# JunyiPeng00/wespeaker_hubert

Hardware: AMD Instinct MI355X
Metric: embeddings/sec on 5s 16kHz utts (higher is better)
Workload: dtype f32 (bf16x3 split MFMA, fp32 accumulate)

## Files before the change

include/wespeaker_amd.h:

```cpp
#ifndef WESPEAKER_AMD_H_
#define WESPEAKER_AMD_H_

#include <stddef.h>
#include <stdint.h>

#ifdef __cplusplus
extern "C" {
#endif

#define WSP_OK 0
#define WSP_E_INVALID (-1)
#define WSP_E_HIP (-2)
#define WSP_E_STATE (-3)
#define WSP_E_UNSUPPORTED (-4)

#define WSP_DTYPE_F32 0
#define WSP_DTYPE_S16 1

#define WSP_WINDOW_HAMMING 0
#define WSP_WINDOW_POVEY 1
#define WSP_WINDOW_HANNING 2
#define WSP_WINDOW_RECTANGULAR 3
#define WSP_WINDOW_BLACKMAN 4

typedef struct wsp_model wsp_model;

int wsp_abi_version(void);
const char* wsp_last_error(void);

int wsp_fbank_num_frames(int num_samples, int frame_len, int frame_shift);

typedef struct wsp_fbank_opts {
  int num_mel_bins;
  int sample_rate;
  double frame_length_ms;
  double frame_shift_ms;
  int window_type;
  double low_freq;
  double high_freq;
} wsp_fbank_opts;

int wsp_fbank_opts_default(wsp_fbank_opts* o);
int wsp_fbank_geometry(const wsp_fbank_opts* o, int* frame_len, int* frame_shift, int* padded);
int wsp_fbank_mel_banks(const wsp_fbank_opts* o, float* banks);

int wsp_fbank_ex(const void* wav, int wav_dtype, int B, int num_samples, int ld, float scale,
                 float* feats, const wsp_fbank_opts* opts, int cmn, void* stream);
int wsp_fbank(const void* wav, int wav_dtype, int B, int num_samples, int ld, float scale,
              float* feats, int num_bins, int sample_rate, int window_type, int cmn,
              void* stream);

int wsp_fbank_segments_ex(const void* wav, int wav_dtype, int B, const int32_t* sample_offsets,
                          const int32_t* frame_offsets, int max_frames, float scale, float* feats,
                          const wsp_fbank_opts* opts, int cmn, void* stream);
int wsp_fbank_segments(const void* wav, int wav_dtype, int B, const int32_t* sample_offsets,
                       const int32_t* frame_offsets, int max_frames, float scale, float* feats,
                       int num_bins, int sample_rate, int window_type, int cmn, void* stream);

int wsp_model_create(const char* arch, int feat_dim, int embed_dim, int emb_bn,
                     int two_emb_layer, wsp_model** out);
int wsp_model_destroy(wsp_model* m);
int wsp_model_num_params(const wsp_model* m);
int wsp_model_param_info(const wsp_model* m, int index, const char** name, int* ndim,
                         int64_t shape[4]);
int wsp_model_set_param(wsp_model* m, int index, const float* host_data, int64_t numel);
int wsp_model_finalize(wsp_model* m);
int wsp_model_embed_dim(const wsp_model* m);
int wsp_model_feat_dim(const wsp_model* m);
int wsp_model_workspace_bytes(const wsp_model* m, int B, int T, size_t* bytes);
int wsp_model_forward(wsp_model* m, const float* feats, int B, int T, float* embed,
                      void* workspace, size_t workspace_bytes, void* stream);

int wsp_model_workspace_bytes_segments(const wsp_model* m, int B, int total_frames, size_t* bytes);
int wsp_model_forward_segments(wsp_model* m, const float* feats, int B, const int32_t* frame_offsets,
                               int total_frames, float* embed, void* workspace, size_t workspace_bytes,
                               void* stream);

int wsp_model_set_option(wsp_model* m, const char* key, int value);
int wsp_model_get_option(const wsp_model* m, const char* key, int* value);

int wsp_model_profile(wsp_model* m, int enable);
int wsp_model_profile_query(wsp_model* m, const char* kernel_class, int* launches,
                            double* total_ms, double* flops_per_launch);

int wsp_frontend_out_frames(const wsp_model* m, int num_samples, int* frames);
int wsp_frontend_workspace_bytes(const wsp_model* m, int B, int num_samples, size_t* bytes);
int wsp_frontend_forward(wsp_model* m, const float* wav, int B, int num_samples, float* feats, int cmn,
                         void* workspace, size_t workspace_bytes, void* stream);

int wsp_frontend_workspace_bytes_segments(const wsp_model* m, int B, const int32_t* num_samples, size_t* bytes);
int wsp_frontend_forward_segments(wsp_model* m, const float* wav, int B, const int32_t* num_samples, float* feats,
                                  int32_t* frame_offsets, int cmn, void* workspace, size_t workspace_bytes,
                                  void* stream);

int wsp_cmn(float* x, int B, int T, int D, void* stream);
int wsp_cmvn(float* x, int B, int T, int D, const int32_t* frame_offsets, int norm_mean, int norm_var,
             void* stream);

typedef struct wsp_resampler wsp_resampler;
int wsp_resampler_create(int orig_freq, int new_freq, int lowpass_filter_width, float rolloff,
                         wsp_resampler** out);
int wsp_resampler_destroy(wsp_resampler* r);
int wsp_resampler_out_len(const wsp_resampler* r, int num_samples, int* out_len);
int wsp_resample(const wsp_resampler* r, const float* x, int B, int num_samples, int ld, float* y, int ldy,
                 void* stream);
int wsp_resampler_kernel(const wsp_resampler* r, int* reduced_orig, int* reduced_new, int* width, int* taps,
                         float* kernel);

int wsp_l2_normalize(const float* x, const float* sub, float* y, int R, int D, void* stream);
int wsp_cosine_pairs(const float* E, int D, const int32_t* idx_a, const int32_t* idx_b,
                     int P, double* score, void* stream);
int wsp_asnorm_stats(const float* E, int Ne, const float* C, int Nc, int D, int top_n,
                     double* mu, double* sd, void* workspace, size_t workspace_bytes,
                     void* stream);
int wsp_asnorm_workspace_bytes(int Ne, int Nc, int D, size_t* bytes);
int wsp_row_mean_accum(const float* x, const int32_t* group, int R, int D, double* acc,
                       double* cnt, void* stream);

#ifdef __cplusplus
}
#endif
#endif
```

wespeaker_hubert_amd/_lib.py:

```python
from __future__ import annotations

import ctypes
import os
from ctypes import POINTER, c_char_p, c_double, c_float, c_int, c_int64, c_size_t, c_void_p

_HERE = os.path.dirname(os.path.abspath(__file__))
LIB_PATH = os.path.join(_HERE, "libwsp_hip.so")

WSP_DTYPE_F32 = 0
WSP_DTYPE_S16 = 1
WSP_WINDOW_HAMMING = 0
WSP_WINDOW_POVEY = 1
WSP_WINDOW_HANNING = 2
WSP_WINDOW_RECTANGULAR = 3
WSP_WINDOW_BLACKMAN = 4
WINDOW_TYPES = {"hamming": WSP_WINDOW_HAMMING, "povey": WSP_WINDOW_POVEY, "hanning": WSP_WINDOW_HANNING,
                "rectangular": WSP_WINDOW_RECTANGULAR, "blackman": WSP_WINDOW_BLACKMAN}


class FbankOpts(ctypes.Structure):
    _fields_ = [("num_mel_bins", c_int), ("sample_rate", c_int), ("frame_length_ms", c_double),
                ("frame_shift_ms", c_double), ("window_type", c_int), ("low_freq", c_double),
                ("high_freq", c_double)]

SIGNATURES = {
    "wsp_abi_version": (c_int, []),
    "wsp_last_error": (c_char_p, []),
    "wsp_fbank_num_frames": (c_int, [c_int, c_int, c_int]),
    "wsp_fbank": (c_int, [c_void_p, c_int, c_int, c_int, c_int, c_float, c_void_p, c_int, c_int,
                          c_int, c_int, c_void_p]),
    "wsp_fbank_segments": (c_int, [c_void_p, c_int, c_int, c_void_p, c_void_p, c_int, c_float, c_void_p, c_int,
                                   c_int, c_int, c_int, c_void_p]),
    "wsp_fbank_opts_default": (c_int, [c_void_p]),
    "wsp_fbank_geometry": (c_int, [c_void_p, POINTER(c_int), POINTER(c_int), POINTER(c_int)]),
    "wsp_fbank_mel_banks": (c_int, [c_void_p, c_void_p]),
    "wsp_fbank_ex": (c_int, [c_void_p, c_int, c_int, c_int, c_int, c_float, c_void_p, c_void_p, c_int, c_void_p]),
    "wsp_fbank_segments_ex": (c_int, [c_void_p, c_int, c_int, c_void_p, c_void_p, c_int, c_float, c_void_p,
                                      c_void_p, c_int, c_void_p]),
    "wsp_model_create": (c_int, [c_char_p, c_int, c_int, c_int, c_int, POINTER(c_void_p)]),
    "wsp_model_destroy": (c_int, [c_void_p]),
    "wsp_model_num_params": (c_int, [c_void_p]),
    "wsp_model_param_info": (c_int, [c_void_p, c_int, POINTER(c_char_p), POINTER(c_int),
                                     POINTER(c_int64)]),
    "wsp_model_set_param": (c_int, [c_void_p, c_int, c_void_p, c_int64]),
    "wsp_model_finalize": (c_int, [c_void_p]),
    "wsp_model_embed_dim": (c_int, [c_void_p]),
    "wsp_model_feat_dim": (c_int, [c_void_p]),
    "wsp_model_workspace_bytes": (c_int, [c_void_p, c_int, c_int, POINTER(c_size_t)]),
    "wsp_model_forward": (c_int, [c_void_p, c_void_p, c_int, c_int, c_void_p, c_void_p, c_size_t,
                                  c_void_p]),
    "wsp_model_workspace_bytes_segments": (c_int, [c_void_p, c_int, c_int, POINTER(c_size_t)]),
    "wsp_model_forward_segments": (c_int, [c_void_p, c_void_p, c_int, c_void_p, c_int, c_void_p, c_void_p,
                                           c_size_t, c_void_p]),
    "wsp_model_set_option": (c_int, [c_void_p, c_char_p, c_int]),
    "wsp_model_get_option": (c_int, [c_void_p, c_char_p, POINTER(c_int)]),
    "wsp_frontend_out_frames": (c_int, [c_void_p, c_int, POINTER(c_int)]),
    "wsp_frontend_workspace_bytes": (c_int, [c_void_p, c_int, c_int, POINTER(c_size_t)]),
    "wsp_frontend_forward": (c_int, [c_void_p, c_void_p, c_int, c_int, c_void_p, c_int, c_void_p, c_size_t,
                                     c_void_p]),
    "wsp_frontend_workspace_bytes_segments": (c_int, [c_void_p, c_int, c_void_p, POINTER(c_size_t)]),
    "wsp_frontend_forward_segments": (c_int, [c_void_p, c_void_p, c_int, c_void_p, c_void_p, c_void_p, c_int,
                                              c_void_p, c_size_t, c_void_p]),
    "wsp_model_profile": (c_int, [c_void_p, c_int]),
    "wsp_model_profile_query": (c_int, [c_void_p, c_char_p, POINTER(c_int), POINTER(c_double),
                                        POINTER(c_double)]),
    "wsp_cmn": (c_int, [c_void_p, c_int, c_int, c_int, c_void_p]),
    "wsp_cmvn": (c_int, [c_void_p, c_int, c_int, c_int, c_void_p, c_int, c_int, c_void_p]),
    "wsp_resampler_create": (c_int, [c_int, c_int, c_int, c_float, c_void_p]),
    "wsp_resampler_destroy": (c_int, [c_void_p]),
    "wsp_resampler_out_len": (c_int, [c_void_p, c_int, c_void_p]),
    "wsp_resample": (c_int, [c_void_p, c_void_p, c_int, c_int, c_int, c_void_p, c_int, c_void_p]),
    "wsp_resampler_kernel": (c_int, [c_void_p, c_void_p, c_void_p, c_void_p, c_void_p, c_void_p]),
    "wsp_l2_normalize": (c_int, [c_void_p, c_void_p, c_void_p, c_int, c_int, c_void_p]),
    "wsp_cosine_pairs": (c_int, [c_void_p, c_int, c_void_p, c_void_p, c_int, c_void_p, c_void_p]),
    "wsp_asnorm_stats": (c_int, [c_void_p, c_int, c_void_p, c_int, c_int, c_int, c_void_p, c_void_p,
                                 c_void_p, c_size_t, c_void_p]),
    "wsp_asnorm_workspace_bytes": (c_int, [c_int, c_int, c_int, POINTER(c_size_t)]),
    "wsp_row_mean_accum": (c_int, [c_void_p, c_void_p, c_int, c_int, c_void_p, c_void_p, c_void_p]),
}

_lib = None


class WspError(RuntimeError):
    pass


def load() -> ctypes.CDLL:
    global _lib
    if _lib is not None:
        return _lib
    if not os.path.exists(LIB_PATH):
        raise WspError(f"HIP library not built: {LIB_PATH} is missing "
                       "(run `python -c 'import __graft_entry__ as g; g.build()'`)")
    lib = ctypes.CDLL(LIB_PATH)
    for name, (res, args) in SIGNATURES.items():
        fn = getattr(lib, name)
        fn.restype = res
        fn.argtypes = args
    _lib = lib
    return lib


def check(status: int, what: str = "") -> None:
    if status != 0:
        msg = load().wsp_last_error().decode("utf-8", "replace")
        raise WspError(f"{what} failed (status {status}): {msg}")


def call(name: str, *args) -> int:
    st = getattr(load(), name)(*args)
    check(st, name)
    return st
```

wespeaker_hubert_amd/csrc/capi.cpp:

```cpp
#include "../../include/wespeaker_amd.h"

#include <hip/hip_runtime.h>

#include <algorithm>
#include <memory>
#include <mutex>
#include <string>
#include <vector>

#include "kernels.h"
#include "model.h"

namespace wsp {
static thread_local std::string g_err;
void set_error(const std::string& m) { g_err = m; }
const std::string& get_error() { return g_err; }

static const FbankPlan& fbank_plan_dev(const FbankConfig& c) {
  static std::mutex mu;
  static std::vector<std::unique_ptr<FbankPlan>> plans;
  static std::vector<int> devs;
  int dev = 0;
  WSP_HIP(hipGetDevice(&dev));
  std::lock_guard<std::mutex> lk(mu);
  for (size_t i = 0; i < plans.size(); ++i) {
    const FbankConfig& q = plans[i]->cfg;
    if (devs[i] == dev && q.num_bins == c.num_bins && q.sample_rate == c.sample_rate && q.window == c.window &&
        q.frame_length_ms == c.frame_length_ms && q.frame_shift_ms == c.frame_shift_ms &&
        q.low_freq == c.low_freq && q.high_freq == c.high_freq)
      return *plans[i];
  }
  auto p = std::make_unique<FbankPlan>();
  fbank_plan(c, *p);
  double* d = nullptr;
  WSP_HIP(hipMalloc(&d, p->host_tab.size() * sizeof(double)));
  WSP_HIP(hipMemcpy(d, p->host_tab.data(), p->host_tab.size() * sizeof(double), hipMemcpyHostToDevice));
  p->tab = d;
  plans.push_back(std::move(p));
  devs.push_back(dev);
  return *plans.back();
}

static FbankConfig fbank_config(const wsp_fbank_opts* o) {
  WSP_CHECK(o != nullptr, "fbank: null options");
  FbankConfig c;
  c.num_bins = o->num_mel_bins;
  c.sample_rate = o->sample_rate;
  c.frame_length_ms = o->frame_length_ms;
  c.frame_shift_ms = o->frame_shift_ms;
  c.window = o->window_type;
  c.low_freq = o->low_freq;
  c.high_freq = o->high_freq;
  fbank_config_resolve(c);
  return c;
}
}

struct wsp_model {
  wsp::Model m;
};

#define WSP_GUARD(...)                                                           \
  try {                                                                          \
    __VA_ARGS__;                                                                      \
    return WSP_OK;                                                               \
  } catch (const wsp::InvalidArg& e) {                                           \
    wsp::set_error(e.msg);                                                       \
    return WSP_E_INVALID;                                                        \
  } catch (const wsp::HipError& e) {                                             \
    wsp::set_error(std::string("HIP error ") + hipGetErrorString(e.err) + " at " + e.where); \
    return WSP_E_HIP;                                                            \
  } catch (const std::exception& e) {                                            \
    wsp::set_error(e.what());                                                    \
    return WSP_E_STATE;                                                          \
  }

static hipStream_t S(void* s) { return reinterpret_cast<hipStream_t>(s); }

extern "C" {

int wsp_abi_version(void) { return 1; }
const char* wsp_last_error(void) { return wsp::get_error().c_str(); }

int wsp_fbank_num_frames(int num_samples, int frame_len, int frame_shift) {
  if (frame_len <= 0 || frame_shift <= 0 || num_samples < frame_len) return 0;
  return 1 + (num_samples - frame_len) / frame_shift;
}

int wsp_fbank_opts_default(wsp_fbank_opts* o) {
  if (!o) return WSP_E_INVALID;
  o->num_mel_bins = 80;
  o->sample_rate = 16000;
  o->frame_length_ms = 25.0;
  o->frame_shift_ms = 10.0;
  o->window_type = WSP_WINDOW_HAMMING;
  o->low_freq = 20.0;
  o->high_freq = 0.0;
  return WSP_OK;
}

int wsp_fbank_geometry(const wsp_fbank_opts* o, int* frame_len, int* frame_shift, int* padded) {
  WSP_GUARD({
    const wsp::FbankConfig c = wsp::fbank_config(o);
    wsp::FbankPlan p;
    wsp::fbank_plan(c, p);
    if (frame_len) *frame_len = c.frame_len;
    if (frame_shift) *frame_shift = c.frame_shift;
    if (padded) *padded = c.padded;
  });
}

int wsp_fbank_mel_banks(const wsp_fbank_opts* o, float* banks) {
  WSP_GUARD({
    WSP_CHECK(banks != nullptr, "fbank: null output");
    std::vector<float> w;
    wsp::fbank_mel_banks(wsp::fbank_config(o), w);
    std::copy(w.begin(), w.end(), banks);
  });
}

int wsp_fbank_ex(const void* wav, int wav_dtype, int B, int num_samples, int ld, float scale, float* feats,
                 const wsp_fbank_opts* opts, int cmn, void* stream) {
  WSP_GUARD({
    const wsp::FbankConfig c = wsp::fbank_config(opts);
    WSP_CHECK(wav_dtype == WSP_DTYPE_F32 || wav_dtype == WSP_DTYPE_S16, "fbank: bad dtype");
    WSP_CHECK(B >= 0 && num_samples >= 0 && ld >= num_samples, "fbank: bad shape");
    const int T = wsp_fbank_num_frames(num_samples, c.frame_len, c.frame_shift);
    if (B > 0 && T > 0) {
      WSP_CHECK(wav && feats, "fbank: null pointer");
      wsp::launch_fbank(wav, wav_dtype, B, num_samples, ld, scale, feats, T, cmn, wsp::fbank_plan_dev(c), S(stream));
    }
  });
}

int wsp_fbank(const void* wav, int wav_dtype, int B, int num_samples, int ld, float scale,
              float* feats, int num_bins, int sample_rate, int window_type, int cmn,
              void* stream) {
  wsp_fbank_opts o;
  wsp_fbank_opts_default(&o);
  o.num_mel_bins = num_bins;
  o.sample_rate = sample_rate;
  o.window_type = window_type;
  return wsp_fbank_ex(wav, wav_dtype, B, num_samples, ld, scale, feats, &o, cmn, stream);
}

int wsp_fbank_segments_ex(const void* wav, int wav_dtype, int B, const int32_t* sample_offsets,
                          const int32_t* frame_offsets, int max_frames, float scale, float* feats,
                          const wsp_fbank_opts* opts, int cmn, void* stream) {
  WSP_GUARD({
    const wsp::FbankConfig c = wsp::fbank_config(opts);
    WSP_CHECK(wav_dtype == WSP_DTYPE_F32 || wav_dtype == WSP_DTYPE_S16, "fbank: bad dtype");
    WSP_CHECK(B >= 0 && max_frames >= 0, "fbank: bad shape");
    if (B > 0 && max_frames > 0) {
      WSP_CHECK(wav && feats && sample_offsets && frame_offsets, "fbank: null pointer");
      wsp::launch_fbank(wav, wav_dtype, B, 0, 0, scale, feats, max_frames, cmn, wsp::fbank_plan_dev(c), S(stream),
                        sample_offsets, frame_offsets);
    }
  });
}

int wsp_fbank_segments(const void* wav, int wav_dtype, int B, const int32_t* sample_offsets,
                       const int32_t* frame_offsets, int max_frames, float scale, float* feats, int num_bins,
                       int sample_rate, int window_type, int cmn, void* stream) {
  wsp_fbank_opts o;
  wsp_fbank_opts_default(&o);
  o.num_mel_bins = num_bins;
  o.sample_rate = sample_rate;
  o.window_type = window_type;
  return wsp_fbank_segments_ex(wav, wav_dtype, B, sample_offsets, frame_offsets, max_frames, scale, feats, &o, cmn,
                               stream);
}

int wsp_model_create(const char* arch, int feat_dim, int embed_dim, int emb_bn, int two_emb_layer,
                     wsp_model** out) {
  WSP_GUARD({
    WSP_CHECK(arch && out, "null argument");
    auto* h = new wsp_model();
    try {
      h->m.create(arch, feat_dim, embed_dim, emb_bn != 0, two_emb_layer != 0);
    } catch (...) {
      delete h;
      throw;
    }
    *out = h;
  });
}

int wsp_model_destroy(wsp_model* m) {
  delete m;
  return WSP_OK;
}

int wsp_model_num_params(const wsp_model* m) { return m ? m->m.num_params() : WSP_E_INVALID; }

int wsp_model_param_info(const wsp_model* m, int index, const char** name, int* ndim,
                         int64_t shape[4]) {
  WSP_GUARD({
    WSP_CHECK(m && name && ndim && shape, "null argument");
    m->m.param_info(index, name, ndim, shape);
  });
}

int wsp_model_set_param(wsp_model* m, int index, const float* host_data, int64_t numel) {
  WSP_GUARD({
    WSP_CHECK(m && (host_data || numel == 0), "null argument");
    m->m.set_param(index, host_data, numel);
  });
}

int wsp_model_finalize(wsp_model* m) {
  WSP_GUARD({
    WSP_CHECK(m, "null model");
    m->m.finalize();
  });
}

int wsp_model_embed_dim(const wsp_model* m) { return m ? m->m.embed_dim() : WSP_E_INVALID; }
int wsp_model_feat_dim(const wsp_model* m) { return m ? m->m.feat_dim() : WSP_E_INVALID; }

int wsp_model_workspace_bytes(const wsp_model* m, int B, int T, size_t* bytes) {
  WSP_GUARD({
    WSP_CHECK(m && bytes && B >= 0 && T >= 0, "bad argument");
    *bytes = m->m.workspace_bytes(B, T);
  });
}

int wsp_model_forward(wsp_model* m, const float* feats, int B, int T, float* embed, void* workspace,
                      size_t workspace_bytes, void* stream) {
  WSP_GUARD({
    WSP_CHECK(m && feats && embed && workspace, "null argument");
    m->m.forward(feats, B, T, embed, workspace, workspace_bytes, S(stream));
  });
}

int wsp_frontend_out_frames(const wsp_model* m, int num_samples, int* frames) {
  WSP_GUARD({
    WSP_CHECK(m && frames, "null argument");
    *frames = m->m.out_frames(num_samples);
  });
}

int wsp_frontend_workspace_bytes(const wsp_model* m, int B, int num_samples, size_t* bytes) {
  WSP_GUARD({
    WSP_CHECK(m && bytes, "null argument");
    *bytes = m->m.frontend_workspace_bytes(B, num_samples);
  });
}

int wsp_frontend_forward(wsp_model* m, const float* wav, int B, int num_samples, float* feats, int cmn,
                         void* workspace, size_t workspace_bytes, void* stream) {
  WSP_GUARD({
    WSP_CHECK(m && wav && feats && workspace, "null argument");
    m->m.forward_frontend(wav, B, num_samples, feats, cmn, workspace, workspace_bytes, S(stream));
  });
}

int wsp_model_workspace_bytes_segments(const wsp_model* m, int B, int total_frames, size_t* bytes) {
  WSP_GUARD({
    WSP_CHECK(m && bytes, "null argument");
    *bytes = m->m.workspace_bytes_segments(B, total_frames);
  });
}

int wsp_model_forward_segments(wsp_model* m, const float* feats, int B, const int32_t* frame_offsets,
                               int total_frames, float* embed, void* workspace, size_t workspace_bytes,
                               void* stream) {
  WSP_GUARD({
    WSP_CHECK(m && feats && frame_offsets && embed && workspace, "null argument");
    m->m.forward_segments(feats, B, frame_offsets, total_frames, embed, workspace, workspace_bytes, S(stream));
  });
}

int wsp_frontend_workspace_bytes_segments(const wsp_model* m, int B, const int32_t* num_samples, size_t* bytes) {
  WSP_GUARD({
    WSP_CHECK(m && num_samples && bytes, "null argument");
    *bytes = m->m.frontend_workspace_bytes_segments(B, num_samples);
  });
}

int wsp_frontend_forward_segments(wsp_model* m, const float* wav, int B, const int32_t* num_samples, float* feats,
                                  int32_t* frame_offsets, int cmn, void* workspace, size_t workspace_bytes,
                                  void* stream) {
  WSP_GUARD({
    WSP_CHECK(m && wav && num_samples && feats && workspace, "null argument");
    m->m.forward_frontend_segments(wav, B, num_samples, feats, frame_offsets, cmn, workspace, workspace_bytes,
                                   S(stream));
  });
}

int wsp_model_set_option(wsp_model* m, const char* key, int value) {
  WSP_GUARD({
    WSP_CHECK(m && key, "null argument");
    m->m.set_option(key, value);
  });
}

int wsp_model_get_option(const wsp_model* m, const char* key, int* value) {
  WSP_GUARD({
    WSP_CHECK(m && key && value, "null argument");
    *value = m->m.get_option(key);
  });
}

int wsp_model_profile(wsp_model* m, int enable) {
  WSP_GUARD({
    WSP_CHECK(m, "null model");
    m->m.profile(enable != 0);
  });
}

int wsp_model_profile_query(wsp_model* m, const char* kernel_class, int* launches,
                            double* total_ms, double* flops_per_launch) {
  WSP_GUARD({
    WSP_CHECK(m && kernel_class && launches && total_ms && flops_per_launch, "null argument");
    m->m.profile_query(kernel_class, launches, total_ms, flops_per_launch);
  });
}

struct wsp_resampler {
  wsp::ResamplePlan plan;
  mutable std::mutex mu;
  mutable int device = -1;
  mutable float* kern = nullptr;
  mutable int* band = nullptr;
};

int wsp_resampler_create(int orig_freq, int new_freq, int lowpass_filter_width, float rolloff,
                         wsp_resampler** out) {
  WSP_GUARD({
    WSP_CHECK(out != nullptr, "bad argument");
    *out = nullptr;
    auto r = std::make_unique<wsp_resampler>();
    wsp::resample_plan(orig_freq, new_freq, lowpass_filter_width, rolloff, r->plan);
    *out = r.release();
  });
}

int wsp_resampler_destroy(wsp_resampler* r) {
  WSP_GUARD({
    if (r) {
      if (r->kern) (void)hipFree(r->kern);
      if (r->band) (void)hipFree(r->band);
      delete r;
    }
  });
}

int wsp_resampler_out_len(const wsp_resampler* r, int num_samples, int* out_len) {
  WSP_GUARD({
    WSP_CHECK(r && out_len && num_samples >= 0, "bad argument");
    const long long n = wsp::resample_out_len(r->plan, num_samples);
    WSP_CHECK(n < (1LL << 31), "output too long");
    *out_len = (int)n;
  });
}

int wsp_resampler_kernel(const wsp_resampler* r, int* reduced_orig, int* reduced_new, int* width, int* taps,
                         float* kernel) {
  WSP_GUARD({
    WSP_CHECK(r != nullptr, "bad argument");
    if (reduced_orig) *reduced_orig = r->plan.orig;
    if (reduced_new) *reduced_new = r->plan.nw;
    if (width) *width = r->plan.width;
    if (taps) *taps = r->plan.L;
    if (kernel && !r->plan.identity) std::copy(r->plan.kern.begin(), r->plan.kern.end(), kernel);
  });
}

int wsp_resample(const wsp_resampler* r, const float* x, int B, int num_samples, int ld, float* y, int ldy,
                 void* stream) {
  WSP_GUARD({
    WSP_CHECK(r && B >= 0 && num_samples >= 0 && (B == 0 || num_samples == 0 || (x && y)), "bad argument");
    int dev = -1;
    WSP_HIP(hipGetDevice(&dev));
    if (!r->plan.identity) {
      std::lock_guard<std::mutex> lk(r->mu);
      if (r->device < 0) {
        WSP_HIP(hipMalloc(&r->kern, r->plan.kern.size() * sizeof(float)));
        WSP_HIP(hipMalloc(&r->band, r->plan.band.size() * sizeof(int)));
        WSP_HIP(hipMemcpy(r->kern, r->plan.kern.data(), r->plan.kern.size() * sizeof(float),
                          hipMemcpyHostToDevice));
        WSP_HIP(hipMemcpy(r->band, r->plan.band.data(), r->plan.band.size() * sizeof(int), hipMemcpyHostToDevice));
        r->device = dev;
      }
      WSP_CHECK(dev == r->device, "resampler is bound to another device");
    }
    wsp::launch_resample(r->plan, r->kern, r->band, x, B, num_samples, ld, y, ldy, S(stream));
  });
}

int wsp_cmn(float* x, int B, int T, int D, void* stream) {
  WSP_GUARD({
    WSP_CHECK(B >= 0 && T > 0 && D > 0 && (B == 0 || x), "bad argument");
    if (B > 0) wsp::launch_cmn_rows(x, B, T, D, S(stream));
  });
}

int wsp_cmvn(float* x, int B, int T, int D, const int32_t* frame_offsets, int norm_mean, int norm_var,
             void* stream) {
  WSP_GUARD({
    WSP_CHECK(B >= 0 && D > 0 && (frame_offsets || T > 0) && (B == 0 || x), "bad argument");
    if (B > 0 && (norm_mean || norm_var))
      wsp::launch_cmvn_rows(x, B, T, D, norm_mean != 0, norm_var != 0, S(stream), frame_offsets);
  });
}

int wsp_l2_normalize(const float* x, const float* sub, float* y, int R, int D, void* stream) {
  WSP_GUARD({
    WSP_CHECK(R >= 0 && D > 0 && (R == 0 || (x && y)), "bad argument");
    wsp::launch_l2_normalize(x, sub, y, R, D, S(stream));
  });
}

int wsp_cosine_pairs(const float* E, int D, const int32_t* idx_a, const int32_t* idx_b, int P,
                     double* score, void* stream) {
  WSP_GUARD({
    WSP_CHECK(P >= 0 && D > 0 && (P == 0 || (E && idx_a && idx_b && score)), "bad argument");
    wsp::launch_cosine_pairs(E, D, idx_a, idx_b, P, score, S(stream));
  });
}

int wsp_asnorm_workspace_bytes(int Ne, int Nc, int D, size_t* bytes) {
  WSP_GUARD({
    WSP_CHECK(bytes && Ne >= 0 && Nc > 0 && D > 0, "bad argument");
    int a, b;
    wsp::asnorm_layout(Ne, Nc, D, &a, &b, bytes);
  });
}

int wsp_asnorm_stats(const float* E, int Ne, const float* C, int Nc, int D, int top_n, double* mu,
                     double* sd, void* workspace, size_t workspace_bytes, void* stream) {
  WSP_GUARD({
    WSP_CHECK(Ne >= 0 && Nc > 0 && D > 0, "bad argument");
    if (Ne == 0) return WSP_OK;
    int Ncp, Dp;
    size_t need;
    wsp::asnorm_layout(Ne, Nc, D, &Ncp, &Dp, &need);
    WSP_CHECK(workspace && workspace_bytes >= need, "asnorm: workspace too small");
    wsp::launch_asnorm_stats(E, Ne, C, Nc, D, top_n, mu, sd, static_cast<float*>(workspace),
                             S(stream));
  });
}

int wsp_row_mean_accum(const float* x, const int32_t* group, int R, int D, double* acc,
                       double* cnt, void* stream) {
  WSP_GUARD({
    WSP_CHECK(R >= 0 && D > 0 && (R == 0 || (x && group && acc && cnt)), "bad argument");
    wsp::launch_row_mean_accum(x, group, R, D, acc, cnt, S(stream));
  });
}

}
```

wespeaker_hubert_amd/csrc/conv_gemm.hip:

```cpp
#include "gemm_common.h"

namespace wsp {

namespace {

constexpr int BK = 32;
constexpr int LDK = BK + 4;

template <int WM, int WN, int TM, int TN, int AMODE, bool UNI>
__global__ __launch_bounds__(256, 2) void conv_gemm_f32(const ConvGemmArgs p) {
  constexpr int BM = WM * TM * 32;
  constexpr int BN = WN * TN * 32;
  constexpr int AR = BM / 32;
  constexpr int BR = BN / 32;
  static_assert(WM * WN == 4, "4 waves");

  extern __shared__ __attribute__((aligned(16))) float smem[];
  float* As = smem;
  float* Bs = smem + 2 * BM * LDK;

  const int tid = threadIdx.x;
  const int lane = tid & 63;
  const int wave = tid >> 6;
  const int ntiles = p.N / BN;
  const int mtiles = (p.M + BM - 1) / BM;
  const int wg = xcd_remap(blockIdx.x, ntiles * mtiles);
  const int mt = wg / ntiles;
  const int nt = wg - mt * ntiles;
  const int m0 = mt * BM;
  const int n0 = nt * BN;

  const int srow = tid >> 3;
  const int c4 = (tid & 7) * 4;
  ALoader<AR, AMODE, UNI> al;
  al.init(p, m0, srow, 32, c4);
  if (p.gcols) al.a0 += (n0 / p.gcols) * p.gcin;
  const __amdgpu_buffer_rsrc_t rw = make_rsrc(p.w);
  int woff[BR];
#pragma unroll
  for (int i = 0; i < BR; ++i) woff[i] = ((n0 + srow + 32 * i) * p.Kp + c4) * 4;

  f32x4 ra[AR], rb[BR];

  auto load_tile = [&](int k0) {
#pragma unroll
    for (int i = 0; i < BR; ++i) rb[i] = bload4(rw, woff[i] + k0 * 4);
    al.load(k0, ra);
  };

  auto store_tile = [&](int buf) {
    float* a = As + buf * BM * LDK;
    float* b = Bs + buf * BN * LDK;
#pragma unroll
    for (int i = 0; i < AR; ++i)
      *reinterpret_cast<f32x4*>(a + (srow + 32 * i) * LDK + c4) = ra[i];
#pragma unroll
    for (int i = 0; i < BR; ++i)
      *reinterpret_cast<f32x4*>(b + (srow + 32 * i) * LDK + c4) = rb[i];
  };

  const int wm = wave / WN;
  const int wn = wave - wm * WN;
  const int r32 = lane & 31;
  const int h = lane >> 5;

  f32x16 acc[TM][TN];
#pragma unroll
  for (int i = 0; i < TM; ++i)
#pragma unroll
    for (int j = 0; j < TN; ++j)
#pragma unroll
      for (int r = 0; r < 16; ++r) acc[i][j][r] = 0.f;

  const int nk = p.Kp / BK;
  load_tile(0);
  store_tile(0);
  __syncthreads();

  for (int kt = 0; kt < nk; ++kt) {
    const int cur = kt & 1;
    if (kt + 1 < nk) load_tile((kt + 1) * BK);
    const float* a = As + cur * BM * LDK + (wm * TM * 32 + r32) * LDK + h * 16;
    const float* b = Bs + cur * BN * LDK + (wn * TN * 32 + r32) * LDK + h * 16;
#pragma unroll
    for (int q = 0; q < 4; ++q) {
      f32x4 af[TM], bf[TN];
#pragma unroll
      for (int i = 0; i < TM; ++i) af[i] = *reinterpret_cast<const f32x4*>(a + i * 32 * LDK + q * 4);
#pragma unroll
      for (int j = 0; j < TN; ++j) bf[j] = *reinterpret_cast<const f32x4*>(b + j * 32 * LDK + q * 4);
#pragma unroll
      for (int s = 0; s < 4; ++s)
#pragma unroll
        for (int i = 0; i < TM; ++i)
#pragma unroll
          for (int j = 0; j < TN; ++j)
            acc[i][j] = __builtin_amdgcn_mfma_f32_32x32x2f32(af[i][s], bf[j][s], acc[i][j], 0, 0, 0);
    }
    if (kt + 1 < nk) store_tile(cur ^ 1);
    __syncthreads();
  }

  gemm_epilogue<TM, TN>(p, acc, m0, n0, wm, wn, lane);
}

template <int WM, int WN, int TM, int TN, int AMODE, bool UNI>
void launch_k(const ConvGemmArgs& p, hipStream_t s) {
  constexpr int BM = WM * TM * 32, BN = WN * TN * 32;
  const int nwg = ((p.M + BM - 1) / BM) * (p.N / BN);
  const size_t lds = (size_t)2 * (BM + BN) * LDK * sizeof(float);
  hipLaunchKernelGGL((conv_gemm_f32<WM, WN, TM, TN, AMODE, UNI>), dim3(nwg), dim3(256), lds, s, p);
  WSP_HIP(hipGetLastError());
}

template <int WM, int WN, int TM, int TN>
void launch_tile(const ConvGemmArgs& p, hipStream_t s) {
  const bool uni = uniform_ktiles(p);
  if (p.amode == kAAdd) {
    if (uni) launch_k<WM, WN, TM, TN, kAAdd, true>(p, s);
    else launch_k<WM, WN, TM, TN, kAAdd, false>(p, s);
  } else {
    if (uni) launch_k<WM, WN, TM, TN, kACat, true>(p, s);
    else launch_k<WM, WN, TM, TN, kACat, false>(p, s);
  }
}

}

int conv_gemm_tile_for(int N) { return (N % 128 == 0) ? 0 : 1; }

void launch_conv_gemm(const ConvGemmArgs& args, hipStream_t s) {
  const ConvGemmArgs p = normalized(args);
  check_conv_args(p, "conv_gemm");
  WSP_CHECK(!p.colsum, "conv_gemm: column sums are a bf16x3-kernel epilogue");
  WSP_CHECK(!p.conv2d && p.N % 64 == 0, "conv_gemm (f32): 1-D convs with N % 64 == 0 only");
  WSP_CHECK(!p.gcols || p.gcols % 64 == 0, "conv_gemm (f32): grouped columns must be a multiple of 64");
  if (conv_gemm_tile_for(p.N) == 0 && !p.gcols)
    launch_tile<2, 2, 2, 2>(p, s);
  else
    launch_tile<4, 1, 1, 2>(p, s);
}

}
```

wespeaker_hubert_amd/csrc/conv_gemm_x3.hip:

```cpp
#include "conv_gemm_x3_impl.h"

namespace wsp {

int conv_gemm_x3_block_rows(const ConvGemmArgs& p, int variant) {
  if (p.N % 64 != 0 || (p.gcols && p.gcols % 64 != 0)) return 128;
  if (p.gcols || p.N % 128 != 0) return 128;
  return variant == 3 ? 128 : 256;
}

namespace {
__global__ __launch_bounds__(256) void colsum_mean_kernel(const double* __restrict__ part, int bm, int T, int N,
                                                          float* __restrict__ out, int ldo) {
  const int b = blockIdx.y;
  const int n = blockIdx.x * 256 + threadIdx.x;
  if (n >= N) return;
  const long r0 = (long)b * T, r1 = r0 + T;
  double v = 0.0;
  for (long mt = r0 / bm; mt * bm < r1; ++mt) {
    const int slot = (mt * bm) / T == b ? 0 : 1;
    v += part[((size_t)mt * 2 + slot) * N + n];
  }
  out[(long)b * ldo + n] = (float)(v / (double)T);
}
}

void launch_colsum_mean(const double* part, int block_rows, int T, int B, int N, float* out, int ldo,
                        hipStream_t s) {
  WSP_CHECK(block_rows > 0 && T >= block_rows && B > 0 && N > 0, "colsum_mean: bad shape");
  hipLaunchKernelGGL(colsum_mean_kernel, dim3((N + 255) / 256, B), dim3(256), 0, s, part, block_rows, T, N, out,
                     ldo);
  WSP_HIP(hipGetLastError());
}

void launch_conv_gemm_x3(const ConvGemmArgs& args, const void* whi, const void* wlo, int variant,
                         hipStream_t s) {
  const ConvGemmArgs p = normalized(args);
  check_conv_args(p, "conv_gemm_x3");
  if (p.colsum) {
    const int bm = conv_gemm_x3_block_rows(p, variant);
    WSP_CHECK(!p.seg && !p.row_bias && !p.conv2d && p.T >= bm,
              "conv_gemm_x3: column sums need a uniform batch with T >= block rows and no row bias");
  }
  WSP_CHECK(p.Kp % 64 == 0, "conv_gemm_x3: packed K must be a multiple of 64");
  WSP_CHECK(variant >= 3 && variant <= 7, "conv_gemm_x3: tile family must be 3, 4, 5, 6 or 7");
  const __bf16* h = static_cast<const __bf16*>(whi);
  const __bf16* l = static_cast<const __bf16*>(wlo);
  x3::TileFn f;
  WSP_CHECK(!p.lnmode || (variant == 7 && x3::g256_supported(p)),
            "conv_gemm_x3: the LayerNorm fold runs on tile family 7 only");
  WSP_CHECK(!p.sc2d || (variant == 7 && x3::g256_supported(p)),
            "conv_gemm_x3: conv3 + shortcut runs on tile family 7 only (N % 256 == 0, 16-B aligned operands)");
  if (variant == 7 && x3::g256_supported(p)) {
    x3::t_g256(p, h, l, s);
    return;
  }
  if (variant == 7) variant = 6;
  if (p.N % 64 != 0 || (p.gcols && p.gcols % 64 != 0)) {
    f = x3::t_4x1_1x1;
  } else if (p.gcols) {
    f = variant >= 5 ? x3::t_8x1_1x2_sw : x3::t_4x1_1x2;
  } else if (p.N % 128 != 0) {
    f = x3::t_4x1_1x2;
  } else if (variant == 3) {
    f = x3::t_2x2_2x2_sw;
  } else if (variant == 4) {
    f = x3::t_4x2_2x2_sw;
  } else if (p.N % 256 == 0) {
    f = variant == 6 ? x3::t_4x2_2x4_mf16 : x3::t_4x2_2x4_sw1;
  } else {
    f = x3::t_4x2_2x2_sw;
  }
  f(p, h, l, s);
}

}
```

wespeaker_hubert_amd/csrc/conv_gemm_x3_impl.h:

```cpp
#pragma once

#include <type_traits>

#include "gemm_common.h"

namespace wsp {

namespace {

typedef __bf16 bf16x8 __attribute__((ext_vector_type(8)));
typedef __bf16 bf16x4 __attribute__((ext_vector_type(4)));

constexpr int BK = 32;

template <bool SWZ, int MF = 32>
struct Lds {
  static constexpr int ROWB = SWZ ? 64 : 80;
  static constexpr int SKEW = SWZ ? 0 : 64;
  __device__ __forceinline__ static int off(int row, int byte) {
    static_assert(MF == 32 || SWZ, "16x16 fragments need the swizzled rows");
    if constexpr (SWZ && MF == 16)
      return row * 64 + ((((byte >> 4) ^ (0x1320 >> (4 * ((row >> 2) & 3)))) & 3) << 4) + (byte & 15);
    else if constexpr (SWZ) return row * 64 + ((((byte >> 4) ^ (row >> 2)) & 3) << 4) + (byte & 15);
    else return row * 80 + byte;
  }
};

template <int WM, int WN, int TM, int TN, int AMODE, bool UNI, int ROLE, bool C2D = false, bool SWZ = false,
          int NSET = 2, int MF = 32>
__global__ __launch_bounds__(WM* WN * 64, 2) void conv_gemm_x3(const ConvGemmArgs p,
                                                               const __bf16* __restrict__ whi,
                                                               const __bf16* __restrict__ wlo) {
  using L = Lds<SWZ, MF>;
  static_assert(MF == 32 || NSET == 1, "16x16 MFMA: one-staging-set wide tiles only");
  constexpr int ROWB = L::ROWB;
  constexpr int NT = WM * WN * 64;
  constexpr int BM = WM * TM * 32;
  constexpr int BN = WN * TN * 32;
  constexpr int AR = BM * 8 / NT;
  constexpr int BR = BN * 8 / NT;
  constexpr int ROWS_A = NT / 8;
  constexpr int A_BYTES = BM * ROWB;
  constexpr int B_BYTES = BN * ROWB;
  constexpr int B_LO = B_BYTES + L::SKEW;
  constexpr int STAGE = 2 * A_BYTES + B_LO + B_BYTES;
  static_assert(AR >= 1 && BR >= 1, "tile too small for the thread count");
  static_assert(BN * 4 % 64 == 0, "a W image must be a whole number of wave loads");

  extern __shared__ __attribute__((aligned(16))) unsigned char smem[];

  const int tid = threadIdx.x;
  const int lane = tid & 63;
  const int wave = tid >> 6;
  const int ntiles = p.N / BN;
  const int mtiles = (p.M + BM - 1) / BM;
  const int wg = xcd_remap(blockIdx.x, ntiles * mtiles);
  const int mt = wg / ntiles;
  const int nt = wg - mt * ntiles;
  const int m0 = mt * BM;
  const int n0 = nt * BN;

  const int srow = tid >> 3;
  const int c4 = (tid & 7) * 4;
  std::conditional_t<C2D, ALoader2D<AR>, ALoader<AR, AMODE, UNI>> al;
  al.init(p, m0, srow, ROWS_A, c4);
  if (p.gcols) al.a0 += (n0 / p.gcols) * p.gcin;
  const __amdgpu_buffer_rsrc_t rwhi = make_rsrc(whi);
  const __amdgpu_buffer_rsrc_t rwlo = make_rsrc(wlo);
  int boff[BR], bls[BR];
  bool bimg[BR];
#pragma unroll
  for (int i = 0; i < BR; ++i) {
    const int q = tid + NT * i;
    const int img = __builtin_amdgcn_readfirstlane(q / (BN * 4));
    const int qq = q - img * BN * 4;
    const int row = qq >> 2, part = qq & 3;
    bimg[i] = img != 0;
    boff[i] = ((n0 + row) * p.Kp + part * 8) * 2;
    bls[i] = L::off(row, part * 16) + (img ? B_LO : 0);
  }

  f32x4 ra0[AR], ra1[AR];
  bf16x8 rb0[BR], rb1[BR];

  auto load_tile = [&](f32x4 (&ra)[AR], bf16x8 (&rb)[BR], int k0, bool live) {
#pragma unroll
    for (int i = 0; i < BR; ++i) {
      const int o = live ? boff[i] + k0 * 2 : kOOB;
      rb[i] = __builtin_bit_cast(bf16x8, __builtin_amdgcn_raw_buffer_load_b128(bimg[i] ? rwlo : rwhi, o, 0, 0));
    }
    al.load(k0, ra, live);
  };

  auto store_tile = [&](const f32x4 (&ra)[AR], const bf16x8 (&rb)[BR], int buf) {
    unsigned char* st = smem + buf * STAGE;
#pragma unroll
    for (int i = 0; i < AR; ++i) {
      bf16x4 hi, lo;
#pragma unroll
      for (int e = 0; e < 4; ++e) {
        const float x = ra[i][e];
        const __bf16 hh = (__bf16)x;
        hi[e] = hh;
        lo[e] = (__bf16)(x - (float)hh);
      }
      const int off = L::off(srow + ROWS_A * i, c4 * 2);
      *reinterpret_cast<bf16x4*>(st + off) = hi;
      *reinterpret_cast<bf16x4*>(st + A_BYTES + off) = lo;
    }
#pragma unroll
    for (int i = 0; i < BR; ++i) *reinterpret_cast<bf16x8*>(st + 2 * A_BYTES + bls[i]) = rb[i];
  };

  const int wm = wave / WN;
  const int wn = wave - wm * WN;
  const int r32 = lane & 31;
  const int h = lane >> 5;

  f32x16 acc[TM][TN];
#pragma unroll
  for (int i = 0; i < TM; ++i)
#pragma unroll
    for (int j = 0; j < TN; ++j)
#pragma unroll
      for (int r = 0; r < 16; ++r) acc[i][j][r] = 0.f;

  auto mma_step = [&](int buf, int s) {
    const unsigned char* st = smem + buf * STAGE;
    const unsigned char* a_hi = st + L::off(wm * TM * 32 + r32, h * 16 + s * 32);
    const unsigned char* a_lo = a_hi + A_BYTES;
    const unsigned char* b_hi = st + 2 * A_BYTES + L::off(wn * TN * 32 + r32, h * 16 + s * 32);
    const unsigned char* b_lo = b_hi + B_LO;
    bf16x8 ah[TM], al_[TM], bh[TN], bl[TN];
#pragma unroll
    for (int i = 0; i < TM; ++i) {
      ah[i] = *reinterpret_cast<const bf16x8*>(a_hi + i * 32 * ROWB);
      al_[i] = *reinterpret_cast<const bf16x8*>(a_lo + i * 32 * ROWB);
    }
#pragma unroll
    for (int j = 0; j < TN; ++j) {
      bh[j] = *reinterpret_cast<const bf16x8*>(b_hi + j * 32 * ROWB);
      bl[j] = *reinterpret_cast<const bf16x8*>(b_lo + j * 32 * ROWB);
    }
#pragma unroll
    for (int i = 0; i < TM; ++i)
#pragma unroll
      for (int j = 0; j < TN; ++j) {
        acc[i][j] = __builtin_amdgcn_mfma_f32_32x32x16_bf16(al_[i], bh[j], acc[i][j], 0, 0, 0);
        acc[i][j] = __builtin_amdgcn_mfma_f32_32x32x16_bf16(ah[i], bl[j], acc[i][j], 0, 0, 0);
        acc[i][j] = __builtin_amdgcn_mfma_f32_32x32x16_bf16(ah[i], bh[j], acc[i][j], 0, 0, 0);
      }
  };

  const int nk = p.Kp / BK;
  if constexpr (MF == 16) {
    const int r16 = lane & 15, qk = lane >> 4;
    f32x4 acc16[2 * TM][2 * TN];
#pragma unroll
    for (int i = 0; i < 2 * TM; ++i)
#pragma unroll
      for (int j = 0; j < 2 * TN; ++j) acc16[i][j] = f32x4{0.f, 0.f, 0.f, 0.f};
    bf16x8 fah[TM], fal[TM], fbh[TN], fbl[TN];
    auto rdA = [&](const unsigned char* st, int ih) {
#pragma unroll
      for (int i = 0; i < TM; ++i) {
        const int o = L::off(wm * TM * 32 + (ih * TM + i) * 16 + r16, qk * 16);
        fah[i] = *reinterpret_cast<const bf16x8*>(st + o);
        fal[i] = *reinterpret_cast<const bf16x8*>(st + A_BYTES + o);
      }
    };
    auto rdB = [&](const unsigned char* st, int jh) {
#pragma unroll
      for (int j = 0; j < TN; ++j) {
        const int o = L::off(wn * TN * 32 + (jh * TN + j) * 16 + r16, qk * 16);
        fbh[j] = *reinterpret_cast<const bf16x8*>(st + 2 * A_BYTES + o);
        fbl[j] = *reinterpret_cast<const bf16x8*>(st + 2 * A_BYTES + B_LO + o);
      }
    };
    auto mm = [&](int ih, int jh) {
#pragma unroll
      for (int i = 0; i < TM; ++i)
#pragma unroll
        for (int j = 0; j < TN; ++j) {
          f32x4& c = acc16[ih * TM + i][jh * TN + j];
          c = __builtin_amdgcn_mfma_f32_16x16x32_bf16(fal[i], fbh[j], c, 0, 0, 0);
          c = __builtin_amdgcn_mfma_f32_16x16x32_bf16(fah[i], fbl[j], c, 0, 0, 0);
          c = __builtin_amdgcn_mfma_f32_16x16x32_bf16(fah[i], fbh[j], c, 0, 0, 0);
        }
    };
    load_tile(ra0, rb0, 0, true);
    store_tile(ra0, rb0, 0);
    load_tile(ra0, rb0, BK, true);
    __syncthreads();
    for (int kt = 0; kt < nk; ++kt) {
      const int buf = kt & 1;
      const unsigned char* st = smem + buf * STAGE;
      rdA(st, 0);
      rdB(st, 0);
      mm(0, 0);
      rdB(st, 1);
      mm(0, 1);
      store_tile(ra0, rb0, buf ^ 1);
      load_tile(ra0, rb0, (kt + 2) * BK, kt + 2 < nk);
      rdA(st, 1);
      mm(1, 1);
      rdB(st, 0);
      mm(1, 0);
      __syncthreads();
    }
    gemm_epilogue16<2 * TM, 2 * TN, WM, WN>(p, acc16, m0, n0, wm, wn, lane, smem);
    return;
  } else if constexpr (NSET == 1) {
    load_tile(ra0, rb0, 0, true);
    store_tile(ra0, rb0, 0);
    load_tile(ra0, rb0, BK, true);
    __syncthreads();
    for (int kt = 0; kt < nk; ++kt) {
      const int buf = kt & 1;
      mma_step(buf, 0);
      store_tile(ra0, rb0, buf ^ 1);
      load_tile(ra0, rb0, (kt + 2) * BK, kt + 2 < nk);
      mma_step(buf, 1);
      __syncthreads();
    }
    gemm_epilogue<TM, TN, WM, WN>(p, acc, m0, n0, wm, wn, lane, smem);
    return;
  }
  load_tile(ra0, rb0, 0, true);
  load_tile(ra1, rb1, BK, true);
  store_tile(ra0, rb0, 0);
  __syncthreads();

  if constexpr (ROLE == 2) {
    for (int kt = 0; kt < nk - 2; kt += 2) {
      load_tile(ra0, rb0, (kt + 2) * BK, true);
      mma_step(0, 0);
      store_tile(ra1, rb1, 1);
      mma_step(0, 1);
      __syncthreads();
      load_tile(ra1, rb1, (kt + 3) * BK, true);
      mma_step(1, 0);
      store_tile(ra0, rb0, 0);
      mma_step(1, 1);
      __syncthreads();
    }
    float rv[TM][TN][16];
    load_residual_tiles<TM, TN>(p, rv, m0, n0, wm, wn, lane);
    mma_step(0, 0);
    store_tile(ra1, rb1, 1);
    mma_step(0, 1);
    __syncthreads();
    mma_step(1, 0);
    mma_step(1, 1);
    gemm_epilogue_res_pre<TM, TN>(p, acc, m0, n0, wm, wn, lane, rv);
    return;
  }

  for (int kt = 0; kt < nk; kt += 2) {
    load_tile(ra0, rb0, (kt + 2) * BK, kt + 2 < nk);
    mma_step(0, 0);
    store_tile(ra1, rb1, 1);
    mma_step(0, 1);
    __syncthreads();
    load_tile(ra1, rb1, (kt + 3) * BK, kt + 3 < nk);
    mma_step(1, 0);
    store_tile(ra0, rb0, 0);
    mma_step(1, 1);
    __syncthreads();
  }

  gemm_epilogue<TM, TN, WM, WN>(p, acc, m0, n0, wm, wn, lane, smem);
}

template <int WM, int WN, int TM, int TN, int AMODE, bool UNI, int ROLE, bool C2D, bool SWZ, int NSET, int MF = 32>
void launch_x3_k(const ConvGemmArgs& p, const __bf16* whi, const __bf16* wlo, hipStream_t s) {
  constexpr int BM = WM * TM * 32, BN = WN * TN * 32, NT = WM * WN * 64;
  constexpr int ROWB = Lds<SWZ>::ROWB;
  const int nwg = ((p.M + BM - 1) / BM) * (p.N / BN);
  const size_t lds = (size_t)2 * (2 * BM * ROWB + 2 * BN * ROWB + Lds<SWZ>::SKEW);
  hipLaunchKernelGGL((conv_gemm_x3<WM, WN, TM, TN, AMODE, UNI, ROLE, C2D, SWZ, NSET, MF>), dim3(nwg), dim3(NT), lds,
                     s, p, whi, wlo);
  WSP_HIP(hipGetLastError());
}

template <int WM, int WN, int TM, int TN, bool SWZ = false, int NSET = 2, int MF = 32>
void launch_x3_tile(const ConvGemmArgs& p, const __bf16* whi, const __bf16* wlo, hipStream_t s) {
  if constexpr (MF == 32) {
    if (p.conv2d) {
      launch_x3_k<WM, WN, TM, TN, kACat, true, 0, true, SWZ, NSET, MF>(p, whi, wlo, s);
      return;
    }
  }
  const bool uni = uniform_ktiles(p);
  if (MF == 32 && p.amode == kAAdd) {
    if constexpr (MF == 32) {
      if (uni)
        launch_x3_k<WM, WN, TM, TN, kAAdd, true, 0, false, SWZ, NSET, MF>(p, whi, wlo, s);
      else
        launch_x3_k<WM, WN, TM, TN, kAAdd, false, 0, false, SWZ, NSET, MF>(p, whi, wlo, s);
    }
  } else if (!uni) {
    launch_x3_k<WM, WN, TM, TN, kACat, false, 0, false, SWZ, NSET, MF>(p, whi, wlo, s);
  } else if (p.role == 1) {
    launch_x3_k<WM, WN, TM, TN, kACat, true, 1, false, SWZ, NSET, MF>(p, whi, wlo, s);
  } else if constexpr (NSET == 2 && TM * TN <= 4) {
    if (p.res && p.role == 2)
      launch_x3_k<WM, WN, TM, TN, kACat, true, 2, false, SWZ, NSET>(p, whi, wlo, s);
    else
      launch_x3_k<WM, WN, TM, TN, kACat, true, 0, false, SWZ, NSET>(p, whi, wlo, s);
  } else {
    launch_x3_k<WM, WN, TM, TN, kACat, true, 0, false, SWZ, NSET, MF>(p, whi, wlo, s);
  }
}

}

namespace x3 {
using TileFn = void (*)(const ConvGemmArgs&, const __bf16*, const __bf16*, hipStream_t);
void t_4x1_1x1(const ConvGemmArgs&, const __bf16*, const __bf16*, hipStream_t);
void t_4x1_1x2(const ConvGemmArgs&, const __bf16*, const __bf16*, hipStream_t);
void t_8x1_1x2_sw(const ConvGemmArgs&, const __bf16*, const __bf16*, hipStream_t);
void t_2x2_2x2_sw(const ConvGemmArgs&, const __bf16*, const __bf16*, hipStream_t);
void t_4x2_2x2_sw(const ConvGemmArgs&, const __bf16*, const __bf16*, hipStream_t);
void t_4x2_2x4_sw1(const ConvGemmArgs&, const __bf16*, const __bf16*, hipStream_t);
void t_4x2_2x4_mf16(const ConvGemmArgs&, const __bf16*, const __bf16*, hipStream_t);
bool g256_supported(const ConvGemmArgs&);
void t_g256(const ConvGemmArgs&, const __bf16*, const __bf16*, hipStream_t);
}

}
```

wespeaker_hubert_amd/csrc/conv_gemm_x3_t6.hip:

```cpp
#include "conv_gemm_x3_impl.h"

namespace wsp {
namespace {

typedef __attribute__((address_space(3))) void lds_void;
constexpr int kGA = 256 * 128, kGW = 256 * 64, kGStage = kGA + 2 * kGW;

__device__ __forceinline__ int g_aslot(int r, int c) { return r * 128 + ((c ^ ((r >> 1) & 5)) << 4); }

__device__ __forceinline__ void g_dma(__amdgpu_buffer_rsrc_t r, unsigned char* lds, int voff) {
  __builtin_amdgcn_raw_ptr_buffer_load_lds(r, (lds_void*)lds, 16, voff, 0, 0, 0);
}

constexpr int kGEpiLd = 132;
constexpr int kGEpiBytes = 8 * 32 * kGEpiLd * 4;
typedef unsigned u32x4 __attribute__((ext_vector_type(4)));

constexpr int kLnMaxParts = 8;
__device__ __forceinline__ void g_ln_row(const ConvGemmArgs& p, int row, float& mu, float& rstd) {
  const float* s = p.ln_in + (size_t)row * p.ln_parts * 2;
  float m = s[0], m2 = s[1];
#pragma unroll
  for (int k = 1; k < kLnMaxParts; ++k) {
    if (k < p.ln_parts) {
      const float d = s[2 * k] - m;
      m += d * (1.f / (float)(k + 1));
      m2 += s[2 * k + 1] + d * d * (128.f * (float)k / (float)(k + 1));
    }
  }
  mu = m;
  rstd = 1.f / sqrtf(m2 / (128.f * (float)p.ln_parts) + p.ln_eps);
}

template <int R>
__device__ __forceinline__ void g_ln_pieces(float (&m)[R], float (&m2)[R]) {
  float n = 4.f;
  auto merge = [&](int i, float mo, float m2o) {
    const float d = mo - m[i];
    m[i] = 0.5f * (m[i] + mo);
    m2[i] = (m2[i] + m2o) + d * d * (0.5f * n);
  };
#define WSP_DPP(v, ctrl) __builtin_bit_cast(float, __builtin_amdgcn_mov_dpp(__builtin_bit_cast(int, v), ctrl, 0xF, 0xF, false))
#pragma unroll
  for (int i = 0; i < R; ++i) merge(i, WSP_DPP(m[i], 0xB1), WSP_DPP(m2[i], 0xB1));
  n *= 2.f;
#pragma unroll
  for (int i = 0; i < R; ++i) merge(i, WSP_DPP(m[i], 0x4E), WSP_DPP(m2[i], 0x4E));
  n *= 2.f;
#pragma unroll
  for (int i = 0; i < R; ++i) merge(i, WSP_DPP(m[i], 0x141), WSP_DPP(m2[i], 0x141));
  n *= 2.f;
#pragma unroll
  for (int i = 0; i < R; ++i) merge(i, WSP_DPP(m[i], 0x140), WSP_DPP(m2[i], 0x140));
  n *= 2.f;
#undef WSP_DPP
#define WSP_BC15(v) \
  __builtin_bit_cast(float, __builtin_amdgcn_update_dpp(0, __builtin_bit_cast(int, v), 0x142, 0xA, 0xF, false))
#pragma unroll
  for (int i = 0; i < R; ++i) merge(i, WSP_BC15(m[i]), WSP_BC15(m2[i]));
#undef WSP_BC15
}

template <int ACT, bool RB, bool RES, int LNM = 0>
__device__ __forceinline__ void g_epilogue_rows(const ConvGemmArgs& p, f32x4 (&acc)[4][8], int m0, int n0, int wm,
                                                int wn, int wave, int lane, unsigned char* smem, float lmu = 0.f,
                                                float lrs = 1.f) {
  float* stg = reinterpret_cast<float*>(smem) + wave * 32 * kGEpiLd;
  const int c16 = lane & 15, q = lane >> 4;
  const int cl = 4 * (lane & 31);
  const int col = n0 + wn * 128 + cl;
  const f32x4 bv = p.bias ? *reinterpret_cast<const f32x4*>(p.bias + col) : f32x4{0.f, 0.f, 0.f, 0.f};
  const f32x4 sc = p.scale ? *reinterpret_cast<const f32x4*>(p.scale + col) : f32x4{1.f, 1.f, 1.f, 1.f};
  const f32x4 sh = p.scale ? *reinterpret_cast<const f32x4*>(p.shift + col) : f32x4{0.f, 0.f, 0.f, 0.f};
  f32x4 lcs{0.f, 0.f, 0.f, 0.f}, lg{1.f, 1.f, 1.f, 1.f}, lb{0.f, 0.f, 0.f, 0.f};
  if constexpr ((LNM & 2) != 0) lcs = *reinterpret_cast<const f32x4*>(p.ln_cs + col);
  if constexpr ((LNM & 4) != 0) {
    lg = *reinterpret_cast<const f32x4*>(p.ln_g + col);
    lb = *reinterpret_cast<const f32x4*>(p.ln_b + col);
  }
  const int lparts = p.N / 128, lpart = (n0 + wn * 128) / 128;
  const __amdgpu_buffer_rsrc_t ro = make_rsrc(p.out);
  const __amdgpu_buffer_rsrc_t rres = make_rsrc(RES ? p.res : p.out);
#pragma unroll
  for (int h = 0; h < 2; ++h) {
    float pm[(LNM & 1) ? 16 : 1], pm2[(LNM & 1) ? 16 : 1];
#pragma unroll
    for (int i2 = 0; i2 < 2; ++i2)
#pragma unroll
      for (int j = 0; j < 8; ++j)
#pragma unroll
        for (int r = 0; r < 4; ++r) stg[(i2 * 16 + 4 * q + r) * kGEpiLd + j * 16 + c16] = acc[2 * h + i2][j][r];
    asm volatile("s_waitcnt lgkmcnt(0)" ::: "memory");
#pragma unroll
    for (int u = 0; u < 16; ++u) {
      const int rl = 2 * u + (lane >> 5);
      const int row = m0 + wm * 64 + h * 32 + rl;
      const bool ok = row < p.M;
      const f32x4 x = *reinterpret_cast<const f32x4*>(stg + rl * kGEpiLd + cl);
      f32x4 rv{0.f, 0.f, 0.f, 0.f}, rb{0.f, 0.f, 0.f, 0.f};
      if constexpr (RES) rv = bload4(rres, ok ? (row * p.ldres + col) * 4 : kOOB);
      if constexpr (RB) {
        const int rowc = ok ? row : p.M - 1;
        const int ub = p.seg ? seg_of(p.seg, p.nseg, rowc) : rowc / p.T;
        rb = *reinterpret_cast<const f32x4*>(p.row_bias + (size_t)ub * p.N + col);
      }
      float mu = 0.f, rstd = 1.f;
      if constexpr ((LNM & 6) != 0) {
        auto rd = [](float v, int l) {
          return __builtin_bit_cast(float, __builtin_amdgcn_readlane(__builtin_bit_cast(int, v), l));
        };
        mu = lane < 32 ? rd(lmu, h * 32 + 2 * u) : rd(lmu, h * 32 + 2 * u + 1);
        rstd = lane < 32 ? rd(lrs, h * 32 + 2 * u) : rd(lrs, h * 32 + 2 * u + 1);
      }
      f32x4 y;
#pragma unroll
      for (int e = 0; e < 4; ++e) {
        float v;
        if constexpr ((LNM & 2) != 0) v = (x[e] - mu * lcs[e]) * rstd + bv[e];
        else v = x[e] + bv[e];
        if constexpr ((LNM & 4) != 0) v += (rv[e] - mu) * rstd * lg[e] + lb[e];
        else if constexpr (RES) v += rv[e];
        if constexpr (RB) v += rb[e];
        if constexpr (ACT == kActRelu) v = fmaxf(v, 0.f);
        else if constexpr (ACT == kActTanh) v = tanhf(v);
        else if constexpr (ACT == kActGelu) v = gelu_as(v);
        y[e] = v * sc[e] + sh[e];
      }
      __builtin_amdgcn_raw_buffer_store_b128(__builtin_bit_cast(u32x4, y), ro, ok ? (row * p.ldo + col) * 4 : kOOB, 0,
                                             0);
      if constexpr ((LNM & 1) != 0) {
        pm[u] = ((y[0] + y[1]) + (y[2] + y[3])) * 0.25f;
        float q2 = 0.f;
#pragma unroll
        for (int e = 0; e < 4; ++e) q2 += (y[e] - pm[u]) * (y[e] - pm[u]);
        pm2[u] = q2;
      }
    }
    if constexpr ((LNM & 1) != 0) {
      g_ln_pieces<16>(pm, pm2);
      if ((lane & 31) == 16) {
#pragma unroll
        for (int u = 0; u < 16; ++u) {
          const int row = m0 + wm * 64 + h * 32 + 2 * u + (lane >> 5);
          if (row < p.M) *reinterpret_cast<float2*>(p.ln_out + ((size_t)row * lparts + lpart) * 2) = float2{pm[u], pm2[u]};
        }
      }
    }
    asm volatile("s_waitcnt lgkmcnt(0)" ::: "memory");
  }
}

constexpr int kGCsLd = 68;
constexpr int kGCsBytes = 8 * 64 * kGCsLd * 4;
template <int ACT>
__device__ __forceinline__ void g_epilogue_cs(const ConvGemmArgs& p, f32x4 (&acc)[4][8], int m0, int n0, int wm,
                                              int wn, int wave, int lane, unsigned char* smem) {
  float* stg = reinterpret_cast<float*>(smem) + wave * 64 * kGCsLd;
  const int c16 = lane & 15, q = lane >> 4;
  const int cl = 4 * c16;
  const __amdgpu_buffer_rsrc_t ro = make_rsrc(p.out);
  const int nb = min((m0 / p.T + 1) * p.T, p.M) - m0, mb = p.M - m0;
  unsigned side0 = 0, side1 = 0;
#pragma unroll
  for (int k = 0; k < 16; ++k) {
    const int rr = wm * 64 + (k >> 2) * 16 + 4 * q + (k & 3);
    side0 |= (rr < nb ? 1u : 0u) << k;
    side1 |= (rr >= nb && rr < mb ? 1u : 0u) << k;
  }
  double rs[8][2];
#pragma unroll
  for (int pp = 0; pp < 2; ++pp) {
#pragma unroll
    for (int i = 0; i < 4; ++i)
#pragma unroll
      for (int jj = 0; jj < 4; ++jj)
#pragma unroll
        for (int r = 0; r < 4; ++r) stg[(16 * i + 4 * q + r) * kGCsLd + 16 * jj + c16] = acc[i][4 * pp + jj][r];
    asm volatile("s_waitcnt lgkmcnt(0)" ::: "memory");
    const int col = n0 + wn * 128 + 64 * pp + cl;
    const f32x4 bv = p.bias ? *reinterpret_cast<const f32x4*>(p.bias + col) : f32x4{0.f, 0.f, 0.f, 0.f};
    const f32x4 sc = p.scale ? *reinterpret_cast<const f32x4*>(p.scale + col) : f32x4{1.f, 1.f, 1.f, 1.f};
    const f32x4 sh = p.scale ? *reinterpret_cast<const f32x4*>(p.shift + col) : f32x4{0.f, 0.f, 0.f, 0.f};
#pragma unroll
    for (int u = 0; u < 16; ++u) {
      const int rl = 4 * u + q;
      const int row = m0 + wm * 64 + rl;
      float* sp = stg + rl * kGCsLd + cl;
      const f32x4 x = *reinterpret_cast<const f32x4*>(sp);
      f32x4 y;
#pragma unroll
      for (int e = 0; e < 4; ++e) {
        float v = x[e] + bv[e];
        if constexpr (ACT == kActRelu) v = fmaxf(v, 0.f);
        else if constexpr (ACT == kActTanh) v = tanhf(v);
        else if constexpr (ACT == kActGelu) v = gelu_as(v);
        y[e] = v * sc[e] + sh[e];
      }
      __builtin_amdgcn_raw_buffer_store_b128(__builtin_bit_cast(u32x4, y), ro,
                                             row < p.M ? (row * p.ldo + col) * 4 : kOOB, 0, 0);
      *reinterpret_cast<f32x4*>(sp) = y;
    }
    asm volatile("s_waitcnt lgkmcnt(0)" ::: "memory");
#pragma unroll
    for (int jj = 0; jj < 4; ++jj) {
      double c0 = 0.0, c1 = 0.0;
#pragma unroll
      for (int k = 0; k < 16; ++k) {
        const double yd = (double)stg[((k >> 2) * 16 + 4 * q + (k & 3)) * kGCsLd + 16 * jj + c16];
        c0 += (side0 >> k) & 1 ? yd : 0.0;
        c1 += (side1 >> k) & 1 ? yd : 0.0;
      }
      double v0 = c0 + __shfl_xor(c0, 16);
      v0 += __shfl_xor(v0, 32);
      double v1 = c1 + __shfl_xor(c1, 16);
      v1 += __shfl_xor(v1, 32);
      rs[4 * pp + jj][0] = v0;
      rs[4 * pp + jj][1] = v1;
      __builtin_amdgcn_sched_barrier(0);
    }
    asm volatile("s_waitcnt lgkmcnt(0)" ::: "memory");
  }
  __syncthreads();
  constexpr int BN = 256;
  double* red = reinterpret_cast<double*>(smem);
  if (lane < 16) {
#pragma unroll
    for (int j = 0; j < 8; ++j)
#pragma unroll
      for (int u = 0; u < 2; ++u) red[(wm * 2 + u) * BN + (wn * 8 + j) * 16 + lane] = rs[j][u];
  }
  __syncthreads();
  const int tid = threadIdx.x;
  if (tid < 2 * BN) {
    const int u = tid / BN, c = tid - u * BN;
    double v = 0.0;
#pragma unroll
    for (int w = 0; w < 4; ++w) v += red[(w * 2 + u) * BN + c];
    p.colsum[((size_t)(m0 / 256) * 2 + u) * p.N + n0 + c] = v;
  }
}

template <int AM, bool CSK, int LNM = 0, int XP = 0>
__global__ __launch_bounds__(512, 1) void conv_gemm_g(const ConvGemmArgs p, const __bf16* __restrict__ whi,
                                                      const __bf16* __restrict__ wlo) {
  using L = Lds<true, 16>;
  constexpr bool DENSE = AM == 1 || AM == 3;
  extern __shared__ __attribute__((aligned(16))) unsigned char smem[];
  const int tid = threadIdx.x;
  const int lane = tid & 63;
  const int wave = tid >> 6;
  const int ntiles = p.N / 256;
  const int mtiles = (p.M + 255) / 256;
  const int wg = xcd_remap(blockIdx.x, ntiles * mtiles);
  const int mt = wg / ntiles;
  const int nt = wg - mt * ntiles;
  const int m0 = mt * 256;
  const int n0 = nt * 256;

  const int ac0 = 4 * ((lane & 7) ^ ((lane >> 4) & 1)), ac1 = ac0 ^ 16;
  int a_r[4], a_t[DENSE ? 1 : 4], a_l[DENSE ? 1 : 4], a_s[AM == 3 ? 4 : 1];
#pragma unroll
  for (int i = 0; i < 4; ++i) {
    const int m = m0 + (4 * wave + i) * 8 + (lane >> 3);
    if constexpr (DENSE) {
      a_r[i] = m < p.M ? m : -1;
      if constexpr (AM == 3) {
        const int fto = p.Fo * p.To;
        const int b = m / fto, fo = (m - b * fto) / p.To, to = m - b * fto - fo * p.To;
        a_s[i] = m < p.M ? (b * p.Fi + fo * p.stride) * p.Ti + to * p.stride : -1;
      }
    } else if (p.seg) {
      const int mm = m < p.M ? m : p.M - 1;
      const int b = seg_of(p.seg, p.nseg, mm);
      const int t = (mm - p.seg[b]) * p.stride;
      const int* is = p.iseg ? p.iseg : p.seg;
      a_r[i] = is[b] + t;
      a_t[i] = (m < p.M) ? t : -0x40000000;
      a_l[i] = is[b + 1] - is[b];
    } else {
      const int b = m / p.T;
      const int t = (m - b * p.T) * p.stride;
      a_r[i] = b * p.Ti + t;
      a_t[i] = (m < p.M) ? t : -0x40000000;
      a_l[i] = p.Ti;
    }
  }
  int woff[2];
#pragma unroll
  for (int i = 0; i < 2; ++i) {
    const int row = (2 * wave + i) * 16 + (lane >> 2);
    const int c = (lane & 3) ^ ((0x1320 >> (4 * ((row >> 2) & 3))) & 3);
    woff[i] = ((n0 + row) * p.Kp + 8 * c) * 2;
  }
  const __amdgpu_buffer_rsrc_t rwh = make_rsrc(whi);
  const __amdgpu_buffer_rsrc_t rwl = make_rsrc(wlo);
  const int nk = p.Kp / BK;
  int jt = 0, ct = 0;
  auto dma = [&](int kt, int buf, int part = 3) {
    unsigned char* st = smem + buf * kGStage;
    const int off = jt * p.dil - p.pad;
    const float* base = p.a[0];
    int ld = p.lda[0], cl = ct;
    if (ct >= p.cseg[2]) {
      base = p.a[2];
      ld = p.lda[2];
      cl = ct - p.cseg[2];
    } else if (ct >= p.cseg[1]) {
      base = p.a[1];
      ld = p.lda[1];
      cl = ct - p.cseg[1];
    }
    const __amdgpu_buffer_rsrc_t ra = make_rsrc(base);
#pragma unroll
    for (int i = 0; i < 4; ++i) {
      if (!(part & 1)) break;
      if constexpr (DENSE) {
        const int ar = AM == 3 && ct >= p.cseg[1] ? a_s[i] : a_r[i];
        g_dma(ra, st + (4 * wave + i) * 1024, ar >= 0 ? (ar * ld + cl + (i & 1 ? ac1 : ac0)) * 4 : kOOB);
      } else if constexpr (AM == 2) {
        const int k = kt * BK + (i & 1 ? ac1 : ac0);
        const int tap = k / p.cin;
        const int offk = tap * p.dil - p.pad;
        const int tt = a_t[i] + offk;
        const bool ok = k < p.K && tt >= 0 && tt < a_l[i];
        g_dma(ra, st + (4 * wave + i) * 1024, ok ? ((a_r[i] + offk) * ld + k - tap * p.cin) * 4 : kOOB);
      } else {
        const int tt = a_t[i] + off;
        const bool ok = tt >= 0 && tt < a_l[i];
        g_dma(ra, st + (4 * wave + i) * 1024, ok ? ((a_r[i] + off) * ld + cl + (i & 1 ? ac1 : ac0)) * 4 : kOOB);
      }
    }
#pragma unroll
    for (int i = 0; i < 2; ++i) {
      if (!(part & 2)) break;
      const int o = woff[i] + kt * 64;
      g_dma(rwh, st + kGA + (2 * wave + i) * 1024, o);
      g_dma(rwl, st + kGA + kGW + (2 * wave + i) * 1024, o);
    }
    if (!(part & 2)) return;
    ct += 32;
    if (ct >= p.cin) {
      ct -= p.cin;
      ++jt;
    }
  };

  const int wm = wave >> 1, wn = wave & 1;
  const int r16 = lane & 15, qk = lane >> 4;
  f32x4 acc[4][8];
#pragma unroll
  for (int i = 0; i < 4; ++i)
#pragma unroll
    for (int j = 0; j < 8; ++j) acc[i][j] = f32x4{0.f, 0.f, 0.f, 0.f};
  bf16x8 ah[2], al[2], bh[4], bl[4];
  auto rdA = [&](const unsigned char* st, int ih) {
#pragma unroll
    for (int i = 0; i < 2; ++i) {
      const int r = wm * 64 + (ih * 2 + i) * 16 + r16;
      const f32x4 x0 = *reinterpret_cast<const f32x4*>(st + g_aslot(r, 2 * qk));
      const f32x4 x1 = *reinterpret_cast<const f32x4*>(st + g_aslot(r, 2 * qk + 1));
      if constexpr (XP == 1 || XP == 4) {
        ah[i] = __builtin_bit_cast(bf16x8, x0);
        al[i] = __builtin_bit_cast(bf16x8, x1);
        continue;
      }
#pragma unroll
      for (int e = 0; e < 4; ++e) {
        const __bf16 h0 = (__bf16)x0[e], h1 = (__bf16)x1[e];
        ah[i][e] = h0;
        ah[i][4 + e] = h1;
        al[i][e] = (__bf16)(x0[e] - (float)h0);
        al[i][4 + e] = (__bf16)(x1[e] - (float)h1);
      }
    }
  };
  auto rdB = [&](const unsigned char* st, int jh) {
#pragma unroll
    for (int j = 0; j < 4; ++j) {
      const int o = L::off(wn * 128 + (jh * 4 + j) * 16 + r16, qk * 16);
      bh[j] = *reinterpret_cast<const bf16x8*>(st + kGA + o);
      bl[j] = *reinterpret_cast<const bf16x8*>(st + kGA + kGW + o);
    }
  };
  auto mm = [&](int ih, int jh) {
#pragma unroll
    for (int i = 0; i < 2; ++i)
#pragma unroll
      for (int j = 0; j < 4; ++j) {
        f32x4& c = acc[ih * 2 + i][jh * 4 + j];
        c = __builtin_amdgcn_mfma_f32_16x16x32_bf16(al[i], bh[j], c, 0, 0, 0);
        c = __builtin_amdgcn_mfma_f32_16x16x32_bf16(ah[i], bl[j], c, 0, 0, 0);
        c = __builtin_amdgcn_mfma_f32_16x16x32_bf16(ah[i], bh[j], c, 0, 0, 0);
      }
  };

  float lmu = 0.f, lrs = 1.f;
  if constexpr ((LNM & 6) != 0) g_ln_row(p, min(m0 + wm * 64 + lane, p.M - 1), lmu, lrs);
  dma(0, 0);
  dma(1, 1);
  asm volatile("s_waitcnt vmcnt(8)" ::: "memory");
  __builtin_amdgcn_s_barrier();
  for (int kt = 0; kt < nk; ++kt) {
    const int buf = kt & 1;
    const unsigned char* st = smem + buf * kGStage;
    if constexpr (XP == 2) {
      rdA(st, 0);
      rdB(st, 0);
      mm(0, 0);
      __builtin_amdgcn_sched_barrier(0);
      if (kt >= 1 && kt + 1 < nk) dma(kt + 1, buf ^ 1, 1);
      __builtin_amdgcn_sched_barrier(0);
      rdB(st, 1);
      mm(0, 1);
      __builtin_amdgcn_sched_barrier(0);
      if (kt >= 1 && kt + 1 < nk) dma(kt + 1, buf ^ 1, 2);
      __builtin_amdgcn_sched_barrier(0);
      rdA(st, 1);
      mm(1, 1);
      rdB(st, 0);
      mm(1, 0);
      asm volatile("s_waitcnt vmcnt(0) lgkmcnt(0)" ::: "memory");
      __builtin_amdgcn_s_barrier();
      __builtin_amdgcn_sched_barrier(0);
      continue;
    }
    rdA(st, 0);
    rdB(st, 0);
    mm(0, 0);
    rdB(st, 1);
    mm(0, 1);
    rdA(st, 1);
    mm(1, 1);
    rdB(st, 0);
    mm(1, 0);
    if constexpr (XP >= 3) {
      asm volatile("s_waitcnt lgkmcnt(0)" ::: "memory");
      continue;
    }
    asm volatile("s_waitcnt vmcnt(0) lgkmcnt(0)" ::: "memory");
    __builtin_amdgcn_s_barrier();
    __builtin_amdgcn_sched_barrier(0);
    if (kt + 2 < nk) dma(kt + 2, buf);
  }
#define WSP_GEPI(RB, RES)                                                                                   \
  switch (p.act) {                                                                                         \
    case kActRelu: g_epilogue_rows<kActRelu, RB, RES>(p, acc, m0, n0, wm, wn, wave, lane, smem); break;    \
    case kActTanh: g_epilogue_rows<kActTanh, RB, RES>(p, acc, m0, n0, wm, wn, wave, lane, smem); break;    \
    case kActGelu: g_epilogue_rows<kActGelu, RB, RES>(p, acc, m0, n0, wm, wn, wave, lane, smem); break;    \
    default: g_epilogue_rows<kActNone, RB, RES>(p, acc, m0, n0, wm, wn, wave, lane, smem); break;          \
  }
  if constexpr (LNM != 0) {
    if constexpr ((LNM & 5) != 0)
      g_epilogue_rows<kActNone, false, true, LNM>(p, acc, m0, n0, wm, wn, wave, lane, smem, lmu, lrs);
    else if (p.act == kActGelu)
      g_epilogue_rows<kActGelu, false, false, LNM>(p, acc, m0, n0, wm, wn, wave, lane, smem, lmu, lrs);
    else
      g_epilogue_rows<kActNone, false, false, LNM>(p, acc, m0, n0, wm, wn, wave, lane, smem, lmu, lrs);
  } else if constexpr (CSK) {
    switch (p.act) {
      case kActRelu: g_epilogue_cs<kActRelu>(p, acc, m0, n0, wm, wn, wave, lane, smem); break;
      case kActTanh: g_epilogue_cs<kActTanh>(p, acc, m0, n0, wm, wn, wave, lane, smem); break;
      case kActGelu: g_epilogue_cs<kActGelu>(p, acc, m0, n0, wm, wn, wave, lane, smem); break;
      default: g_epilogue_cs<kActNone>(p, acc, m0, n0, wm, wn, wave, lane, smem); break;
    }
  } else if (p.res) {
    WSP_GEPI(false, true)
  } else if (p.row_bias) {
    WSP_GEPI(true, false)
  } else {
    WSP_GEPI(false, false)
  }
#undef WSP_GEPI
}

#ifdef WSP_G7_XP
constexpr int kBStages = 4;
template <int AM, bool CSK>
__global__ __launch_bounds__(512, 1) void conv_gemm_gb(const ConvGemmArgs p, const __bf16* __restrict__ whi,
                                                       const __bf16* __restrict__ wlo) {
  constexpr bool DENSE = AM == 1;
  static_assert(AM == 0 || AM == 1, "family 10: uniform k-tiles only");
  extern __shared__ __attribute__((aligned(16))) unsigned char smem[];
  const int tid = threadIdx.x;
  const int lane = tid & 63;
  const int wave = tid >> 6;
  const int ntiles = p.N / 256;
  const int mtiles = (p.M + 255) / 256;
  const int wg = xcd_remap(blockIdx.x, ntiles * mtiles);
  const int mt = wg / ntiles;
  const int nt = wg - mt * ntiles;
  const int m0 = mt * 256;
  const int n0 = nt * 256;

  const int ac0 = 4 * ((lane & 7) ^ ((lane >> 4) & 1)), ac1 = ac0 ^ 16;
  int a_r[4], a_t[DENSE ? 1 : 4], a_l[DENSE ? 1 : 4];
#pragma unroll
  for (int i = 0; i < 4; ++i) {
    const int m = m0 + (4 * wave + i) * 8 + (lane >> 3);
    if constexpr (DENSE) {
      a_r[i] = m < p.M ? m : -1;
    } else if (p.seg) {
      const int mm = m < p.M ? m : p.M - 1;
      const int b = seg_of(p.seg, p.nseg, mm);
      const int t = (mm - p.seg[b]) * p.stride;
      const int* is = p.iseg ? p.iseg : p.seg;
      a_r[i] = is[b] + t;
      a_t[i] = (m < p.M) ? t : -0x40000000;
      a_l[i] = is[b + 1] - is[b];
    } else {
      const int b = m / p.T;
      const int t = (m - b * p.T) * p.stride;
      a_r[i] = b * p.Ti + t;
      a_t[i] = (m < p.M) ? t : -0x40000000;
      a_l[i] = p.Ti;
    }
  }
  const int nk = p.Kp / BK;
  int jt = 0, ct = 0;
  auto dma_a = [&](int kt) {
    unsigned char* st = smem + (kt & (kBStages - 1)) * kGA;
    const bool live = kt < nk;
    const int off = jt * p.dil - p.pad;
    const float* base = p.a[0];
    int ld = p.lda[0], cl = ct;
    if (ct >= p.cseg[2]) {
      base = p.a[2];
      ld = p.lda[2];
      cl = ct - p.cseg[2];
    } else if (ct >= p.cseg[1]) {
      base = p.a[1];
      ld = p.lda[1];
      cl = ct - p.cseg[1];
    }
    const __amdgpu_buffer_rsrc_t ra = make_rsrc(base);
#pragma unroll
    for (int i = 0; i < 4; ++i) {
      if constexpr (DENSE) {
        g_dma(ra, st + (4 * wave + i) * 1024,
              live && a_r[i] >= 0 ? (a_r[i] * ld + cl + (i & 1 ? ac1 : ac0)) * 4 : kOOB);
      } else {
        const int tt = a_t[i] + off;
        const bool ok = live && tt >= 0 && tt < a_l[i];
        g_dma(ra, st + (4 * wave + i) * 1024, ok ? ((a_r[i] + off) * ld + cl + (i & 1 ? ac1 : ac0)) * 4 : kOOB);
      }
    }
    ct += 32;
    if (ct >= p.cin) {
      ct -= p.cin;
      ++jt;
    }
  };

  const int wm = wave >> 1, wn = wave & 1;
  const int r16 = lane & 15, qk = lane >> 4;
  const __amdgpu_buffer_rsrc_t rwh = make_rsrc(whi);
  const __amdgpu_buffer_rsrc_t rwl = make_rsrc(wlo);
  const int bcol0 = ((n0 + wn * 128 + r16) * p.Kp + 8 * qk) * 2;
  const int bjstep = 16 * p.Kp * 2;
  bf16x8 bh[2][4], bl[2][4];
  auto load_b = [&](int kt, int jh) {
    const bool live = kt < nk;
#pragma unroll
    for (int j = 0; j < 4; ++j) {
      const int o = live ? bcol0 + (4 * jh + j) * bjstep + kt * 64 : kOOB;
      bh[jh][j] = __builtin_bit_cast(bf16x8, __builtin_amdgcn_raw_buffer_load_b128(rwh, o, 0, 0));
      bl[jh][j] = __builtin_bit_cast(bf16x8, __builtin_amdgcn_raw_buffer_load_b128(rwl, o, 0, 0));
    }
  };

  f32x4 acc[4][8];
#pragma unroll
  for (int i = 0; i < 4; ++i)
#pragma unroll
    for (int j = 0; j < 8; ++j) acc[i][j] = f32x4{0.f, 0.f, 0.f, 0.f};
  bf16x8 ah[2][2], al[2][2];
  auto rdA = [&](const unsigned char* st, int ih) {
#pragma unroll
    for (int i = 0; i < 2; ++i) {
      const int r = wm * 64 + (ih * 2 + i) * 16 + r16;
      const f32x4 x0 = *reinterpret_cast<const f32x4*>(st + g_aslot(r, 2 * qk));
      const f32x4 x1 = *reinterpret_cast<const f32x4*>(st + g_aslot(r, 2 * qk + 1));
#pragma unroll
      for (int e = 0; e < 4; ++e) {
        const __bf16 h0 = (__bf16)x0[e], h1 = (__bf16)x1[e];
        ah[ih][i][e] = h0;
        ah[ih][i][4 + e] = h1;
        al[ih][i][e] = (__bf16)(x0[e] - (float)h0);
        al[ih][i][4 + e] = (__bf16)(x1[e] - (float)h1);
      }
    }
  };
  auto mm = [&](int ih, int jh) {
#pragma unroll
    for (int i = 0; i < 2; ++i)
#pragma unroll
      for (int j = 0; j < 4; ++j) {
        f32x4& c = acc[ih * 2 + i][jh * 4 + j];
        c = __builtin_amdgcn_mfma_f32_16x16x32_bf16(al[ih][i], bh[jh][j], c, 0, 0, 0);
        c = __builtin_amdgcn_mfma_f32_16x16x32_bf16(ah[ih][i], bl[jh][j], c, 0, 0, 0);
        c = __builtin_amdgcn_mfma_f32_16x16x32_bf16(ah[ih][i], bh[jh][j], c, 0, 0, 0);
      }
  };

  dma_a(0);
  dma_a(1);
  dma_a(2);
  dma_a(3);
  load_b(0, 0);
  load_b(0, 1);
  asm volatile("s_waitcnt vmcnt(0)" ::: "memory");
  __builtin_amdgcn_s_barrier();
  for (int kt = 0; kt < nk; ++kt) {
    const unsigned char* st = smem + (kt & (kBStages - 1)) * kGA;
    rdA(st, 0);
    mm(0, 0);
    rdA(st, 1);
    mm(1, 0);
    __builtin_amdgcn_sched_barrier(0);
    load_b(kt + 1, 0);
    __builtin_amdgcn_sched_barrier(0);
    mm(1, 1);
    mm(0, 1);
    __builtin_amdgcn_sched_barrier(0);
    load_b(kt + 1, 1);
    asm volatile("s_waitcnt vmcnt(56) lgkmcnt(0)" ::: "memory");
    __builtin_amdgcn_s_barrier();
    __builtin_amdgcn_sched_barrier(0);
    dma_a(kt + 4);
  }
  asm volatile("s_waitcnt vmcnt(0)" ::: "memory");
  __builtin_amdgcn_s_barrier();
#define WSP_GBEPI(RB, RES)                                                                                  \
  switch (p.act) {                                                                                         \
    case kActRelu: g_epilogue_rows<kActRelu, RB, RES>(p, acc, m0, n0, wm, wn, wave, lane, smem); break;    \
    case kActTanh: g_epilogue_rows<kActTanh, RB, RES>(p, acc, m0, n0, wm, wn, wave, lane, smem); break;    \
    case kActGelu: g_epilogue_rows<kActGelu, RB, RES>(p, acc, m0, n0, wm, wn, wave, lane, smem); break;    \
    default: g_epilogue_rows<kActNone, RB, RES>(p, acc, m0, n0, wm, wn, wave, lane, smem); break;          \
  }
  if constexpr (CSK) {
    switch (p.act) {
      case kActRelu: g_epilogue_cs<kActRelu>(p, acc, m0, n0, wm, wn, wave, lane, smem); break;
      case kActTanh: g_epilogue_cs<kActTanh>(p, acc, m0, n0, wm, wn, wave, lane, smem); break;
      case kActGelu: g_epilogue_cs<kActGelu>(p, acc, m0, n0, wm, wn, wave, lane, smem); break;
      default: g_epilogue_cs<kActNone>(p, acc, m0, n0, wm, wn, wave, lane, smem); break;
    }
  } else if (p.res) {
    WSP_GBEPI(false, true)
  } else if (p.row_bias) {
    WSP_GBEPI(true, false)
  } else {
    WSP_GBEPI(false, false)
  }
#undef WSP_GBEPI
}
#endif

}

namespace x3 {

bool g256_supported(const ConvGemmArgs& p) {
  auto a16 = [](const void* q) { return (reinterpret_cast<uintptr_t>(q) & 15) == 0; };
  const bool aligned = a16(p.out) && p.ldo % 4 == 0 && a16(p.bias) && a16(p.scale) && a16(p.shift) &&
                       a16(p.row_bias) && a16(p.res) && (!p.res || p.ldres % 4 == 0);
  return aligned && p.N % 256 == 0 && !p.conv2d && !p.gcols && p.amode == kACat &&
         (uniform_ktiles(p) || (p.cseg[1] >= p.cin && !p.colsum)) &&
         (!p.sc2d || (uniform_ktiles(p) && !p.colsum && !p.lnmode && !p.row_bias));
}

void t_g256(const ConvGemmArgs& p, const __bf16* h, const __bf16* l, hipStream_t s) {
  const int nwg = ((p.M + 255) / 256) * (p.N / 256);
  constexpr int lds0 = 2 * kGStage > kGEpiBytes ? 2 * kGStage : kGEpiBytes;
  constexpr int lds = lds0 > kGCsBytes ? lds0 : kGCsBytes;
  const bool dense = p.taps == 1 && p.pad == 0 && p.stride == 1 && !p.iseg && (p.seg || p.Ti == p.T);
  const int am = !uniform_ktiles(p) ? 2 : dense ? 1 : 0;
  if (p.sc2d) {
    hipLaunchKernelGGL((conv_gemm_g<3, false>), dim3(nwg), dim3(512), lds, s, p, h, l);
    WSP_HIP(hipGetLastError());
    return;
  }
  if (p.lnmode) {
    WSP_CHECK(am == 1 && !p.colsum && !p.row_bias && !p.scale && p.N % 128 == 0 &&
                  ((p.lnmode & 1) == 0 || (p.ln_out && p.res && p.act == kActNone)) &&
                  ((p.lnmode & 6) == 0 || (p.ln_in && p.ln_parts >= 1 && p.ln_parts <= kLnMaxParts)) && ((p.lnmode & 2) == 0 || (p.ln_cs && !p.res)) &&
                  ((p.lnmode & 4) == 0 || (p.ln_g && p.ln_b && p.res && p.act == kActNone)),
              "conv_gemm_x3: LayerNorm fold needs a dense 1x1 GEMM and its operands");
    switch (p.lnmode) {
      case 1: hipLaunchKernelGGL((conv_gemm_g<1, false, 1>), dim3(nwg), dim3(512), lds, s, p, h, l); break;
      case 2: hipLaunchKernelGGL((conv_gemm_g<1, false, 2>), dim3(nwg), dim3(512), lds, s, p, h, l); break;
      case 4: hipLaunchKernelGGL((conv_gemm_g<1, false, 4>), dim3(nwg), dim3(512), lds, s, p, h, l); break;
      case 5: hipLaunchKernelGGL((conv_gemm_g<1, false, 5>), dim3(nwg), dim3(512), lds, s, p, h, l); break;
      default: WSP_CHECK(false, "conv_gemm_x3: lnmode must be 1, 2, 4 or 5");
    }
    WSP_HIP(hipGetLastError());
    return;
  }
  if (p.colsum && am == 1)
    hipLaunchKernelGGL((conv_gemm_g<1, true>), dim3(nwg), dim3(512), lds, s, p, h, l);
  else if (p.colsum && am == 0)
    hipLaunchKernelGGL((conv_gemm_g<0, true>), dim3(nwg), dim3(512), lds, s, p, h, l);
  else if (am == 1)
    hipLaunchKernelGGL((conv_gemm_g<1, false>), dim3(nwg), dim3(512), lds, s, p, h, l);
  else if (am == 0)
    hipLaunchKernelGGL((conv_gemm_g<0, false>), dim3(nwg), dim3(512), lds, s, p, h, l);
  else
    hipLaunchKernelGGL((conv_gemm_g<2, false>), dim3(nwg), dim3(512), lds, s, p, h, l);
  WSP_HIP(hipGetLastError());
}

#ifdef WSP_G7_XP
bool gb256_supported(const ConvGemmArgs& p) {
  return g256_supported(p) && uniform_ktiles(p) && !p.lnmode && p.Kp % BK == 0;
}

void t_gb256(const ConvGemmArgs& p, const __bf16* h, const __bf16* l, hipStream_t s) {
  WSP_CHECK(gb256_supported(p), "conv_gemm_x3 family 10: unsupported operands");
  const int nwg = ((p.M + 255) / 256) * (p.N / 256);
  constexpr int lds0 = kBStages * kGA > kGEpiBytes ? kBStages * kGA : kGEpiBytes;
  constexpr int lds = lds0 > kGCsBytes ? lds0 : kGCsBytes;
  const bool dense = p.taps == 1 && p.pad == 0 && p.stride == 1 && !p.iseg && (p.seg || p.Ti == p.T);
  if (p.colsum && dense)
    hipLaunchKernelGGL((conv_gemm_gb<1, true>), dim3(nwg), dim3(512), lds, s, p, h, l);
  else if (p.colsum)
    hipLaunchKernelGGL((conv_gemm_gb<0, true>), dim3(nwg), dim3(512), lds, s, p, h, l);
  else if (dense)
    hipLaunchKernelGGL((conv_gemm_gb<1, false>), dim3(nwg), dim3(512), lds, s, p, h, l);
  else
    hipLaunchKernelGGL((conv_gemm_gb<0, false>), dim3(nwg), dim3(512), lds, s, p, h, l);
  WSP_HIP(hipGetLastError());
}

void t_g256_xp(const ConvGemmArgs& p, const __bf16* h, const __bf16* l, hipStream_t s, int xp) {
  const int nwg = ((p.M + 255) / 256) * (p.N / 256);
  constexpr int lds0 = 2 * kGStage > kGEpiBytes ? 2 * kGStage : kGEpiBytes;
  constexpr int lds = lds0 > kGCsBytes ? lds0 : kGCsBytes;
  const bool dense = p.taps == 1 && p.pad == 0 && p.stride == 1 && !p.iseg && (p.seg || p.Ti == p.T);
  const int am = !uniform_ktiles(p) ? 2 : dense ? 1 : 0;
  WSP_CHECK(am != 2 && !p.lnmode, "t_g256_xp: AM 0 / 1 only");
#define WSP_XPL(AMv, CS, XPv) hipLaunchKernelGGL((conv_gemm_g<AMv, CS, 0, XPv>), dim3(nwg), dim3(512), lds, s, p, h, l)
  if (xp == 1) {
    if (p.colsum) { if (am == 1) WSP_XPL(1, true, 1); else WSP_XPL(0, true, 1); }
    else { if (am == 1) WSP_XPL(1, false, 1); else WSP_XPL(0, false, 1); }
  } else if (xp == 3) {
    WSP_CHECK(am == 1 && !p.colsum, "t_g256_xp 3: dense, no column sums");
    WSP_XPL(1, false, 3);
  } else if (xp == 4) {
    WSP_CHECK(am == 1 && !p.colsum, "t_g256_xp 4: dense, no column sums");
    WSP_XPL(1, false, 4);
  } else {
    if (p.colsum) { if (am == 1) WSP_XPL(1, true, 2); else WSP_XPL(0, true, 2); }
    else { if (am == 1) WSP_XPL(1, false, 2); else WSP_XPL(0, false, 2); }
  }
#undef WSP_XPL
  WSP_HIP(hipGetLastError());
}
#endif

}
}
```

wespeaker_hubert_amd/csrc/ecapa_model.cpp:

```cpp
#include "model_impl.h"

namespace wsp {

void Model::Impl::build_ecapa_params() {
  const int64_t C = this->C, w = C / 8;
  add("layer1.conv.weight", {C, feat_dim, 5});
  add("layer1.conv.bias", {C});
  add_bn("layer1.bn", C);
  for (int li = 2; li <= 4; ++li) {
    const std::string p = "layer" + std::to_string(li) + ".se_res2block";
    add(p + ".0.conv.weight", {C, C, 1});
    add(p + ".0.conv.bias", {C});
    add_bn(p + ".0.bn", C);
    for (int i = 0; i < 7; ++i) {
      add(p + ".1.convs." + std::to_string(i) + ".weight", {w, w, 3});
      add(p + ".1.convs." + std::to_string(i) + ".bias", {w});
    }
    for (int i = 0; i < 7; ++i) add_bn(p + ".1.bns." + std::to_string(i), w);
    add(p + ".2.conv.weight", {C, C, 1});
    add(p + ".2.conv.bias", {C});
    add_bn(p + ".2.bn", C);
    add(p + ".3.linear1.weight", {128, C});
    add(p + ".3.linear1.bias", {128});
    add(p + ".3.linear2.weight", {C, 128});
    add(p + ".3.linear2.bias", {C});
  }
  add("conv.weight", {1536, 3 * C, 1});
  add("conv.bias", {1536});
  add("pool.linear1.weight", {128, glob ? 4608 : 1536, 1});
  add("pool.linear1.bias", {128});
  add("pool.linear2.weight", {1536, 128, 1});
  add("pool.linear2.bias", {1536});
  add_bn("bn", 3072);
  add("linear.weight", {embed_dim, 3072});
  add("linear.bias", {embed_dim});
  if (emb_bn) add_bn("bn2", embed_dim);
}

void Model::Impl::pack_res2(Block& b, const std::string& p, int w) {
  const std::vector<float>* W[7];
  std::vector<float> bias((size_t)7 * w), sc((size_t)7 * w), sh((size_t)7 * w);
  for (int i = 0; i < 7; ++i) {
    const std::string ci = p + ".1.convs." + std::to_string(i);
    W[i] = &P(ci + ".weight");
    const auto& bb = P(ci + ".bias");
    std::vector<double> s, t;
    bn_affine(p + ".1.bns." + std::to_string(i), s, t);
    for (int n = 0; n < w; ++n) {
      bias[(size_t)i * w + n] = bb[n];
      sc[(size_t)i * w + n] = (float)s[n];
      sh[(size_t)i * w + n] = (float)t[n];
    }
  }
  b.r2w = dev.upload_u16(pack::frag_res2(W, w));
  b.r2b = dev.upload(bias);
  b.r2s = dev.upload(sc);
  b.r2t = dev.upload(sh);
}

void Model::Impl::finalize_ecapa() {
  const int w = C / 8;
  layer1 = pack_conv(P("layer1.conv.weight"), C, feat_dim, 5, P("layer1.conv.bias").data(), "layer1.bn");
  for (int li = 0; li < 3; ++li) {
    const std::string p = "layer" + std::to_string(li + 2) + ".se_res2block";
    Block& b = blk[li];
    b.c1 = pack_conv(P(p + ".0.conv.weight"), C, C, 1, P(p + ".0.conv.bias").data(), p + ".0.bn");
    for (int i = 0; i < 7; ++i) {
      const std::string ci = p + ".1.convs." + std::to_string(i);
      b.res2[i] = pack_conv(P(ci + ".weight"), w, w, 3, P(ci + ".bias").data(), p + ".1.bns." + std::to_string(i));
    }
    if (res2_chain_supported(w, li + 2)) pack_res2(b, p, w);
    b.c3 = pack_conv(P(p + ".2.conv.weight"), C, C, 1, P(p + ".2.conv.bias").data(), p + ".2.bn");
    b.se1 = pack_lin(P(p + ".3.linear1.weight").data(), 128, C, C, P(p + ".3.linear1.bias").data());
    b.se2 = pack_lin(P(p + ".3.linear2.weight").data(), C, 128, 128, P(p + ".3.linear2.bias").data());
  }
  conv = pack_conv(P("conv.weight"), 1536, 3 * C, 1, P("conv.bias").data(), "");
  {
    std::vector<float> wg = P("conv.weight");
    for (int n = 0; n < 1536; ++n)
      for (int c = 0; c < C; ++c) {
        float* r = wg.data() + (size_t)n * 3 * C;
        r[C + c] = (float)((double)r[C + c] + (double)r[2 * C + c]);
      }
    conv_g = pack_conv(wg, 1536, 3 * C, 1, P("conv.bias").data(), "");
  }
  const auto& l1 = P("pool.linear1.weight");
  const int l1k = glob ? 4608 : 1536;
  {
    std::vector<float> wx((size_t)128 * 1536);
    for (int n = 0; n < 128; ++n)
      for (int k = 0; k < 1536; ++k) wx[(size_t)n * 1536 + k] = l1[(size_t)n * l1k + k];
    pool1 = pack_conv(wx, 128, 1536, 1, P("pool.linear1.bias").data(), "");
    if (glob) {
      pool1_ctx = pack_lin(l1.data() + 1536, 128, 3072, l1k, P("pool.linear1.bias").data());
    }
  }
  pool2 = pack_conv(P("pool.linear2.weight"), 1536, 128, 1, P("pool.linear2.bias").data(), "");
  pool2_frag = pack_frag(P("pool.linear2.weight"), 1536, 128);
  {
    std::vector<double> s, t;
    bn_affine("bn", s, t);
    const auto& W = P("linear.weight");
    const auto& bb = P("linear.bias");
    const int D = embed_dim;
    std::vector<double> s2(D, 1.0), t2(D, 0.0);
    if (emb_bn) bn_affine("bn2", s2, t2);
    std::vector<float> wf((size_t)D * 3072), bf(D);
    for (int n = 0; n < D; ++n) {
      double acc = bb[n];
      for (int k = 0; k < 3072; ++k) {
        const double wv = W[(size_t)n * 3072 + k];
        wf[(size_t)n * 3072 + k] = (float)(s2[n] * wv * s[k]);
        acc += wv * t[k];
      }
      bf[n] = (float)(s2[n] * acc + t2[n]);
    }
    head = pack_lin(wf.data(), D, 3072, 3072, bf.data());
  }
}

int Model::Impl::ecapa_chunk(int B, int T) const {
  return chunk_for(B, (size_t)T * std::max(C, 1536) * sizeof(float));
}

namespace {
struct EcapaWs {
  float *x[5], *h1, *h2, *h3, *gmean, *ghid, *gate, *xp, *att, *logit, *gstats, *rowb, *pooled;
  double* sesum;
  size_t floats;
};
EcapaWs ecapa_ws(size_t C, size_t B, size_t M, float* base) {
  WsCursor c{base};
  EcapaWs w;
  w.x[0] = nullptr;
  for (int i = 1; i <= 4; ++i) w.x[i] = c.take(M * C);
  w.h1 = c.take(M * C);
  w.h2 = c.take(M * C);
  w.h3 = c.take(M * C);
  w.gmean = c.take(B * C);
  w.ghid = c.take(B * 128);
  w.gate = c.take(B * C);
  w.xp = c.take(M * 1536);
  w.att = c.take(M * 128);
  w.logit = c.take(M * 1536);
  w.gstats = c.take(B * 3072);
  w.rowb = c.take(B * 128);
  w.pooled = c.take(B * 3072);
  w.sesum = reinterpret_cast<double*>(c.take(((M + 127) / 128) * 2 * C * 2));
  w.floats = c.off;
  return w;
}
}

size_t Model::Impl::ecapa_ws_floats(int B, size_t M) const { return ecapa_ws(C, B, M, nullptr).floats; }

void Model::Impl::forward_ecapa(const float* feats, int B, int T, float* embed, float* ws, hipStream_t s,
                                const int* seg, int M_seg) {
  const int M = seg ? M_seg : B * T, w = C / 8;
  const EcapaWs W = ecapa_ws(C, B, M, ws);
  float* const* x = W.x;
  float *h1 = W.h1, *h2 = W.h2, *h3 = W.h3, *xp = W.xp;
  const int se_bm = precision == 1 ? conv_gemm_x3_block_rows(ConvGemmArgs{.N = C}, x3_variant) : 0;
  const bool se_fused = precision == 1 && !seg && T >= se_bm;
  auto gemm3 = [&](const char* tag, ConvGemmArgs& g, const ConvW& cw, int dil, int pad, float* out, int ldo) {
    g.lda[0] = g.lda[1] = g.lda[2] = C;
    fill(g, cw, M, T, dil, pad, out, ldo, kActRelu, nullptr, true, seg, B);
    run(tag, 2.0 * M * cw.N * cw.K, s, [&] { launch(g, cw, s); });
  };

  gemm("layer1", layer1, feats, feat_dim, x[1], C, M, T, 1, 2, kActRelu, s, seg, B);
  for (int li = 0; li < 3; ++li) {
    const Block& b = blk[li];
    const int dil = li + 2;
    const float* xin = x[li + 1];
    gemm("conv1x1_CxC", b.c1, xin, C, h1, C, M, T, 1, 0, kActRelu, s, seg, B, nullptr, true, 1);
    if (precision == 1 && res2_fused && b.r2w) {
      Res2Args r{};
      r.x = h1;
      r.out = h2;
      r.ldx = r.ldo = C;
      r.M = M;
      r.T = T;
      r.dil = dil;
      r.variant = w == 128 ? res2_variant : std::min(res2_variant, 3);
      r.rout = res2_chain_rout(dil, r.variant, M);
      r.seg = seg;
      r.nseg = B;
      r.w = b.r2w;
      r.bias = b.r2b;
      r.scale = b.r2s;
      r.shift = b.r2t;
      run("res2_k3", 7 * 2.0 * M * w * 3 * w, s, [&] { launch_res2_chain(r, w, s); });
    } else {
      for (int i = 0; i < 7; ++i) {
        ConvGemmArgs g{};
        g.amode = i == 0 ? kACat : kAAdd;
        if (i == 0) {
          one_operand(g, h1, C, w);
        } else {
          g.a[0] = h1 + i * w;
          g.a[1] = h2 + (i - 1) * w;
          g.a[2] = h1;
        }
        gemm3("res2_k3", g, b.res2[i], dil, dil, h2 + i * w, C);
      }
    }
    {
      ConvGemmArgs g{};
      g.amode = kACat;
      g.a[0] = h2;
      g.a[1] = h1 + 7 * w;
      g.a[2] = h1;
      g.cseg[1] = 7 * w;
      g.cseg[2] = g.cseg[3] = C;
      g.role = 1;
      if (se_fused) g.colsum = W.sesum;
      gemm3("conv1x1_CxC", g, b.c3, 1, 0, h3, C);
    }
    run("se", 0, s, [&] {
      if (se_fused) launch_colsum_mean(W.sesum, se_bm, T, B, C, W.gmean, C, s);
      else launch_frame_stats(h3, C, B, T, C, W.gmean, C, 0, 0, s, seg);
      launch_small_linear({W.gmean, C, b.se1.wt, b.se1.bias, W.ghid, 128, B, C, 128, 1}, s);
      launch_small_linear({W.ghid, 128, b.se2.wt, b.se2.bias, W.gate, C, B, 128, C, 3}, s);
      launch_residual_scale(cat_gate && li == 2 ? nullptr : xin, h3, W.gate, x[li + 2], B, T, C, s, seg, M);
    });
  }
  {
    ConvGemmArgs g{};
    g.amode = kACat;
    g.a[0] = x[2];
    g.a[1] = x[3];
    g.a[2] = x[4];
    g.cseg[1] = C;
    g.cseg[2] = 2 * C;
    g.cseg[3] = 3 * C;
    gemm3("conv_cat", g, cat_gate ? conv_g : conv, 1, 0, xp, 1536);
  }
  if (glob) {
    run("glob_ctx", 0, s, [&] {
      launch_frame_stats(xp, 1536, B, T, 1536, W.gstats, 3072, 1, 1536, s, seg);
      launch_small_linear({W.gstats, 3072, pool1_ctx.wt, pool1_ctx.bias, W.rowb, 128, B, 3072, 128, 0}, s);
    });
  }
  gemm("pool_linear1", pool1, xp, 1536, W.att, 128, M, T, 1, 0, kActTanh, s, seg, B, glob ? W.rowb : nullptr, !glob);
  if (precision == 1 && astp_fused_on) {
    AstpArgs a{W.att, xp, 1536, B, T, 1536, seg, pool2_frag, pool2.bias, 1e-7f, W.pooled};
    run("astp", 2.0 * M * 1536 * 128, s, [&] { launch_astp_fused(a, s); });
  } else {
    gemm("pool_linear2", pool2, W.att, 128, W.logit, 1536, M, T, 1, 0, kActNone, s, seg, B);
    run("astp", 0, s, [&] { launch_astp_pool(W.logit, xp, B, T, 1536, W.pooled, s, seg); });
  }
  run("head", 0, s, [&] {
    launch_small_linear({W.pooled, 3072, head.wt, head.bias, embed, embed_dim, B, 3072, embed_dim, 0}, s);
  });
}

}
```

wespeaker_hubert_amd/csrc/gemm_common.h:

```cpp
#pragma once

#include <algorithm>

#include "kernels.h"

namespace wsp {

constexpr int kOOB = 0x7FFFFFF0;

__device__ __forceinline__ __amdgpu_buffer_rsrc_t make_rsrc(const void* base) {
  const unsigned long long a = reinterpret_cast<unsigned long long>(base);
  const unsigned lo = __builtin_amdgcn_readfirstlane((unsigned)a);
  const unsigned hi = __builtin_amdgcn_readfirstlane((unsigned)(a >> 32));
  void* p = reinterpret_cast<void*>(((unsigned long long)hi << 32) | lo);
  return __builtin_amdgcn_make_buffer_rsrc(p, (short)0, kOOB, 0x00020000);
}

__device__ __forceinline__ f32x4 bload4(__amdgpu_buffer_rsrc_t r, int voff) {
  return __builtin_bit_cast(f32x4, __builtin_amdgcn_raw_buffer_load_b128(r, voff, 0, 0));
}

template <int AR, int AMODE, bool UNI>
struct ALoader {
  const float* a0;
  const float* a1;
  const float* a2;
  int ld0, ld1, ld2, cs1, cs2;
  int cin, dil, pad, Ti, K;
  int c4;
  int a_r[AR], a_t[AR], a_l[AR];
  int j, c;

  __device__ __forceinline__ void init(const ConvGemmArgs& p, int m0, int srow, int rows_step,
                                       int c4_) {
    a0 = p.a[0];
    a1 = p.a[1];
    a2 = p.a[2];
    ld0 = p.lda[0];
    ld1 = p.lda[1];
    ld2 = p.lda[2];
    cs1 = p.cseg[1];
    cs2 = p.cseg[2];
    cin = p.cin;
    dil = p.dil;
    pad = p.pad;
    Ti = p.Ti;
    K = p.K;
    c4 = c4_;
    j = 0;
    c = 0;
#pragma unroll
    for (int i = 0; i < AR; ++i) {
      const int m = m0 + srow + rows_step * i;
      if (p.seg) {
        const int mm = m < p.M ? m : p.M - 1;
        const int b = seg_of(p.seg, p.nseg, mm);
        const int t = (mm - p.seg[b]) * p.stride;
        const int* is = p.iseg ? p.iseg : p.seg;
        a_r[i] = is[b] + t;
        a_t[i] = (m < p.M) ? t : -0x40000000;
        a_l[i] = is[b + 1] - is[b];
      } else {
        const int b = m / p.T;
        const int t = (m - b * p.T) * p.stride;
        a_r[i] = b * p.Ti + t;
        a_t[i] = (m < p.M) ? t : -0x40000000;
        a_l[i] = p.Ti;
      }
    }
  }

  __device__ __forceinline__ void load(int k0, f32x4 (&ra)[AR], bool live = true) {
    if constexpr (UNI) {
      const int off = j * dil - pad;
      const float* base = a0;
      int ld = ld0, cl = c;
      if (AMODE == kACat) {
        if (c >= cs2) {
          base = a2;
          ld = ld2;
          cl = c - cs2;
        } else if (c >= cs1) {
          base = a1;
          ld = ld1;
          cl = c - cs1;
        }
      }
      const __amdgpu_buffer_rsrc_t r0 = make_rsrc(base);
      const __amdgpu_buffer_rsrc_t r1 = make_rsrc(a1);
#pragma unroll
      for (int i = 0; i < AR; ++i) {
        const int tt = a_t[i] + off;
        const bool ok = live && tt >= 0 && tt < a_l[i];
        const int row = a_r[i] + off;
        ra[i] = bload4(r0, ok ? (row * ld + cl + c4) * 4 : kOOB);
        if (AMODE == kAAdd) ra[i] += bload4(r1, ok ? (row * ld1 + c + c4) * 4 : kOOB);
      }
      c += 32;
      if (c >= cin) {
        c -= cin;
        ++j;
      }
    } else {
      const int k = k0 + c4;
      const bool kin = k < K;
      const int jj = kin ? k / cin : 0;
      const int cc = k - jj * cin;
      const int off = jj * dil - pad;
      const __amdgpu_buffer_rsrc_t r0 = make_rsrc(a0);
      const __amdgpu_buffer_rsrc_t r1 = make_rsrc(a1);
#pragma unroll
      for (int i = 0; i < AR; ++i) {
        const int tt = a_t[i] + off;
        const bool ok = live && kin && tt >= 0 && tt < a_l[i];
        const int row = a_r[i] + off;
        ra[i] = bload4(r0, ok ? (row * ld0 + cc) * 4 : kOOB);
        if (AMODE == kAAdd) ra[i] += bload4(r1, ok ? (row * ld1 + cc) * 4 : kOOB);
      }
    }
  }
};

template <int AR>
struct ALoader2D {
  const float* a0;
  int ld, cin, Fi, Ti, kw, T0;
  int c4;
  int rb[AR], fi0[AR], ti0[AR];
  int j, c;

  __device__ __forceinline__ void init(const ConvGemmArgs& p, int m0, int srow, int rows_step,
                                       int c4_) {
    a0 = p.a[0];
    ld = p.lda[0];
    cin = p.cin;
    Fi = p.Fi;
    Ti = p.Ti;
    kw = p.kw;
    c4 = c4_;
    j = 0;
    c = 0;
    const int plane = p.Fo * p.To;
#pragma unroll
    for (int i = 0; i < AR; ++i) {
      const int m = m0 + srow + rows_step * i;
      const int b = m / plane;
      const int rem = m - b * plane;
      const int fo = rem / p.To;
      const int to = rem - fo * p.To;
      rb[i] = b * p.Fi * p.Ti;
      fi0[i] = (m < p.M) ? fo * p.stride - p.pad : -0x40000000;
      ti0[i] = to * p.stride - p.pad;
    }
  }

  __device__ __forceinline__ void load(int , f32x4 (&ra)[AR], bool live = true) {
    const int kf = j / kw;
    const int kt = j - kf * kw;
    const __amdgpu_buffer_rsrc_t r0 = make_rsrc(a0);
#pragma unroll
    for (int i = 0; i < AR; ++i) {
      const int fi = fi0[i] + kf;
      const int ti = ti0[i] + kt;
      const bool ok = live && fi >= 0 && fi < Fi && ti >= 0 && ti < Ti;
      const int row = rb[i] + fi * Ti + ti;
      ra[i] = bload4(r0, ok ? (row * ld + c + c4) * 4 : kOOB);
    }
    c += 32;
    if (c >= cin) {
      c -= cin;
      ++j;
    }
  }
};

template <int TM, int TN>
__device__ __forceinline__ void load_residual_tiles(const ConvGemmArgs& p, float (&rv)[TM][TN][16], int m0, int n0,
                                                    int wm, int wn, int lane) {
  const int r32 = lane & 31;
  const int h = lane >> 5;
  const __amdgpu_buffer_rsrc_t rres = make_rsrc(p.res);
  const int ldr4 = p.ldres * 4;
#pragma unroll
  for (int j = 0; j < TN; ++j)
#pragma unroll
    for (int i = 0; i < TM; ++i) {
      const int row0 = m0 + (wm * TM + i) * 32 + 4 * h;
      const int lim = p.M - row0;
      const int rbase = row0 * ldr4 + (n0 + (wn * TN + j) * 32 + r32) * 4;
#pragma unroll
      for (int r = 0; r < 16; ++r) {
        const int rr = (r & 3) + 8 * (r >> 2);
        rv[i][j][r] = __builtin_bit_cast(
            float, __builtin_amdgcn_raw_buffer_load_b32(rres, rr < lim ? rbase + rr * ldr4 : kOOB, 0, 0));
      }
    }
}

template <int TM, int TN, int ACT, bool RB, bool CS = false, bool RES = false, bool PRE = false>
__device__ __forceinline__ void gemm_epilogue_store(const ConvGemmArgs& p, f32x16 (&acc)[TM][TN], int m0, int n0,
                                                    int wm, int wn, int lane, double (*cs)[2] = nullptr,
                                                    const float (*rext)[TN][16] = nullptr) {
  const int r32 = lane & 31;
  const int h = lane >> 5;
  const __amdgpu_buffer_rsrc_t ro = make_rsrc(p.out);
  const int ldo4 = p.ldo * 4;
  const __amdgpu_buffer_rsrc_t rres = make_rsrc(RES ? p.res : p.out);
  const int ldr4 = p.ldres * 4;
  constexpr bool RPRE = RES && !PRE && TM * TN <= 4;
  float rpre[RPRE ? TM : 1][RPRE ? TN : 1][16];
  if constexpr (RPRE) {
#pragma unroll
    for (int j = 0; j < TN; ++j)
#pragma unroll
      for (int i = 0; i < TM; ++i) {
        const int row0 = m0 + (wm * TM + i) * 32 + 4 * h;
        const int lim = p.M - row0;
        const int rbase = row0 * ldr4 + (n0 + (wn * TN + j) * 32 + r32) * 4;
#pragma unroll
        for (int r = 0; r < 16; ++r) {
          const int rr = (r & 3) + 8 * (r >> 2);
          rpre[i][j][r] = __builtin_bit_cast(
              float, __builtin_amdgcn_raw_buffer_load_b32(rres, rr < lim ? rbase + rr * ldr4 : kOOB, 0, 0));
        }
      }
  }
#pragma unroll
  for (int j = 0; j < TN; ++j) {
    const int col = n0 + (wn * TN + j) * 32 + r32;
    const float bv = p.bias ? p.bias[col] : 0.f;
    const float sc = p.scale ? p.scale[col] : 1.f;
    const float sh = p.scale ? p.shift[col] : 0.f;
#pragma unroll
    for (int i = 0; i < TM; ++i) {
      const int row0 = m0 + (wm * TM + i) * 32 + 4 * h;
      const int lim = p.M - row0;
      const int base = row0 * ldo4 + col * 4;
      int mode = 2;
      if constexpr (CS) {
        const int t0 = m0 + (wm * TM + i) * 32;
        const int next = (m0 / p.T + 1) * p.T;
        if (t0 + 32 <= p.M) mode = t0 + 32 <= next ? 0 : (t0 >= next ? 1 : 2);
      }
      float rv[16];
      if constexpr (PRE) {
#pragma unroll
        for (int r = 0; r < 16; ++r) rv[r] = rext[i][j][r];
      } else if constexpr (RPRE) {
#pragma unroll
        for (int r = 0; r < 16; ++r) rv[r] = rpre[i][j][r];
      } else if constexpr (RES && !PRE) {
        const int rbase = row0 * ldr4 + col * 4;
#pragma unroll
        for (int r = 0; r < 16; ++r) {
          const int rr = (r & 3) + 8 * (r >> 2);
          rv[r] = __builtin_bit_cast(
              float, __builtin_amdgcn_raw_buffer_load_b32(rres, rr < lim ? rbase + rr * ldr4 : kOOB, 0, 0));
        }
      }
#pragma unroll
      for (int r = 0; r < 16; ++r) {
        const int rr = (r & 3) + 8 * (r >> 2);
        float y = acc[i][j][r] + bv;
        if constexpr (RES) y += rv[r];
        if constexpr (RB) {
          const int row = row0 + rr;
          const int rowc = row < p.M ? row : p.M - 1;
          const int ub = p.seg ? seg_of(p.seg, p.nseg, rowc) : rowc / p.T;
          y += p.row_bias[(size_t)ub * p.N + col];
        }
        if constexpr (ACT == kActRelu) y = fmaxf(y, 0.f);
        else if constexpr (ACT == kActTanh) y = tanhf(y);
        else if constexpr (ACT == kActGelu) y = gelu_as(y);
        y = y * sc + sh;
        const int off = rr < lim ? base + rr * ldo4 : kOOB;
        __builtin_amdgcn_raw_buffer_store_b32(__builtin_bit_cast(unsigned, y), ro, off, 0, 0);
        if constexpr (CS) {
          const double yd = (double)y;
          if (mode == 0) {
            cs[j][0] += yd;
          } else if (mode == 1) {
            cs[j][1] += yd;
          } else {
            const int row = row0 + rr;
            const int next = (m0 / p.T + 1) * p.T;
            cs[j][0] += (row < next && row < p.M) ? yd : 0.0;
            cs[j][1] += (row >= next && row < p.M) ? yd : 0.0;
          }
        }
      }
    }
  }
}

template <int TN, int WM, int WN, int BM>
__device__ __forceinline__ void gemm_colsum_reduce(const ConvGemmArgs& p, double (*cs)[2], int m0, int n0, int wm,
                                                   int wn, int lane, unsigned char* smem) {
  constexpr int BN = WN * TN * 32;
  double* red = reinterpret_cast<double*>(smem);
#pragma unroll
  for (int j = 0; j < TN; ++j)
#pragma unroll
    for (int u = 0; u < 2; ++u) {
      const double v = cs[j][u] + __shfl_xor(cs[j][u], 32);
      if (lane < 32) red[(wm * 2 + u) * BN + (wn * TN + j) * 32 + lane] = v;
    }
  __syncthreads();
  const int tid = threadIdx.x;
  if (tid < 2 * BN) {
    const int u = tid / BN, c = tid - u * BN;
    double v = 0.0;
#pragma unroll
    for (int w = 0; w < WM; ++w) v += red[(w * 2 + u) * BN + c];
    p.colsum[((size_t)(m0 / BM) * 2 + u) * p.N + n0 + c] = v;
  }
}

template <int TM, int TN, int WM = 0, int WN = 0>
__device__ __forceinline__ void gemm_epilogue(const ConvGemmArgs& p, f32x16 (&acc)[TM][TN], int m0, int n0,
                                              int wm, int wn, int lane, unsigned char* smem = nullptr) {
  if constexpr (WM > 0) {
    if (p.colsum) {
      double cs[TN][2];
#pragma unroll
      for (int j = 0; j < TN; ++j) cs[j][0] = cs[j][1] = 0.0;
      switch (p.act) {
        case kActRelu: gemm_epilogue_store<TM, TN, kActRelu, false, true>(p, acc, m0, n0, wm, wn, lane, cs); break;
        case kActTanh: gemm_epilogue_store<TM, TN, kActTanh, false, true>(p, acc, m0, n0, wm, wn, lane, cs); break;
        case kActGelu: gemm_epilogue_store<TM, TN, kActGelu, false, true>(p, acc, m0, n0, wm, wn, lane, cs); break;
        default: gemm_epilogue_store<TM, TN, kActNone, false, true>(p, acc, m0, n0, wm, wn, lane, cs); break;
      }
      gemm_colsum_reduce<TN, WM, WN, WM * TM * 32>(p, cs, m0, n0, wm, wn, lane, smem);
      return;
    }
  }
  if (p.res) {
    switch (p.act) {
      case kActRelu: gemm_epilogue_store<TM, TN, kActRelu, false, false, true>(p, acc, m0, n0, wm, wn, lane); break;
      case kActTanh: gemm_epilogue_store<TM, TN, kActTanh, false, false, true>(p, acc, m0, n0, wm, wn, lane); break;
      case kActGelu: gemm_epilogue_store<TM, TN, kActGelu, false, false, true>(p, acc, m0, n0, wm, wn, lane); break;
      default: gemm_epilogue_store<TM, TN, kActNone, false, false, true>(p, acc, m0, n0, wm, wn, lane); break;
    }
    return;
  }
  if (p.row_bias) {
    switch (p.act) {
      case kActRelu: gemm_epilogue_store<TM, TN, kActRelu, true>(p, acc, m0, n0, wm, wn, lane); break;
      case kActTanh: gemm_epilogue_store<TM, TN, kActTanh, true>(p, acc, m0, n0, wm, wn, lane); break;
      case kActGelu: gemm_epilogue_store<TM, TN, kActGelu, true>(p, acc, m0, n0, wm, wn, lane); break;
      default: gemm_epilogue_store<TM, TN, kActNone, true>(p, acc, m0, n0, wm, wn, lane); break;
    }
  } else {
    switch (p.act) {
      case kActRelu: gemm_epilogue_store<TM, TN, kActRelu, false>(p, acc, m0, n0, wm, wn, lane); break;
      case kActTanh: gemm_epilogue_store<TM, TN, kActTanh, false>(p, acc, m0, n0, wm, wn, lane); break;
      case kActGelu: gemm_epilogue_store<TM, TN, kActGelu, false>(p, acc, m0, n0, wm, wn, lane); break;
      default: gemm_epilogue_store<TM, TN, kActNone, false>(p, acc, m0, n0, wm, wn, lane); break;
    }
  }
}

template <int TM, int TN>
__device__ __forceinline__ void gemm_epilogue_res_pre(const ConvGemmArgs& p, f32x16 (&acc)[TM][TN], int m0, int n0,
                                                      int wm, int wn, int lane, const float (&rv)[TM][TN][16]) {
  switch (p.act) {
    case kActRelu: gemm_epilogue_store<TM, TN, kActRelu, false, false, true, true>(p, acc, m0, n0, wm, wn, lane, nullptr, rv); break;
    case kActTanh: gemm_epilogue_store<TM, TN, kActTanh, false, false, true, true>(p, acc, m0, n0, wm, wn, lane, nullptr, rv); break;
    case kActGelu: gemm_epilogue_store<TM, TN, kActGelu, false, false, true, true>(p, acc, m0, n0, wm, wn, lane, nullptr, rv); break;
    default: gemm_epilogue_store<TM, TN, kActNone, false, false, true, true>(p, acc, m0, n0, wm, wn, lane, nullptr, rv); break;
  }
}

template <int TM, int TN, int ACT, bool RB, bool CS = false, bool RES = false>
__device__ __forceinline__ void gemm_epilogue_store16(const ConvGemmArgs& p, f32x4 (&acc)[TM][TN], int m0, int n0,
                                                      int wm, int wn, int lane, double (*cs)[2] = nullptr) {
  const int c16 = lane & 15;
  const int q = lane >> 4;
  const __amdgpu_buffer_rsrc_t ro = make_rsrc(p.out);
  const int ldo4 = p.ldo * 4;
  const __amdgpu_buffer_rsrc_t rres = make_rsrc(RES ? p.res : p.out);
  const int ldr4 = p.ldres * 4;
#pragma unroll
  for (int j = 0; j < TN; ++j) {
    const int col = n0 + (wn * TN + j) * 16 + c16;
    const float bv = p.bias ? p.bias[col] : 0.f;
    const float sc = p.scale ? p.scale[col] : 1.f;
    const float sh = p.scale ? p.shift[col] : 0.f;
#pragma unroll
    for (int i = 0; i < TM; ++i) {
      const int t0 = m0 + (wm * TM + i) * 16;
      const int row0 = t0 + 4 * q;
      const int lim = p.M - row0;
      const int base = row0 * ldo4 + col * 4;
      int mode = 2;
      if constexpr (CS) {
        const int next = (m0 / p.T + 1) * p.T;
        if (t0 + 16 <= p.M) mode = t0 + 16 <= next ? 0 : (t0 >= next ? 1 : 2);
      }
      float rv[4];
      if constexpr (RES) {
        const int rbase = row0 * ldr4 + col * 4;
#pragma unroll
        for (int r = 0; r < 4; ++r)
          rv[r] = __builtin_bit_cast(float,
                                     __builtin_amdgcn_raw_buffer_load_b32(rres, r < lim ? rbase + r * ldr4 : kOOB, 0, 0));
      }
#pragma unroll
      for (int r = 0; r < 4; ++r) {
        float y = acc[i][j][r] + bv;
        if constexpr (RES) y += rv[r];
        if constexpr (RB) {
          const int row = row0 + r;
          const int rowc = row < p.M ? row : p.M - 1;
          const int ub = p.seg ? seg_of(p.seg, p.nseg, rowc) : rowc / p.T;
          y += p.row_bias[(size_t)ub * p.N + col];
        }
        if constexpr (ACT == kActRelu) y = fmaxf(y, 0.f);
        else if constexpr (ACT == kActTanh) y = tanhf(y);
        else if constexpr (ACT == kActGelu) y = gelu_as(y);
        y = y * sc + sh;
        __builtin_amdgcn_raw_buffer_store_b32(__builtin_bit_cast(unsigned, y), ro, r < lim ? base + r * ldo4 : kOOB, 0,
                                              0);
        if constexpr (CS) {
          const double yd = (double)y;
          if (mode == 0) {
            cs[j][0] += yd;
          } else if (mode == 1) {
            cs[j][1] += yd;
          } else {
            const int row = row0 + r;
            const int next = (m0 / p.T + 1) * p.T;
            cs[j][0] += (row < next && row < p.M) ? yd : 0.0;
            cs[j][1] += (row >= next && row < p.M) ? yd : 0.0;
          }
        }
      }
    }
  }
}

template <int TN, int WM, int WN, int BM>
__device__ __forceinline__ void gemm_colsum_reduce16(const ConvGemmArgs& p, double (*cs)[2], int m0, int n0, int wm,
                                                     int wn, int lane, unsigned char* smem) {
  constexpr int BN = WN * TN * 16;
  double* red = reinterpret_cast<double*>(smem);
#pragma unroll
  for (int j = 0; j < TN; ++j)
#pragma unroll
    for (int u = 0; u < 2; ++u) {
      double v = cs[j][u] + __shfl_xor(cs[j][u], 16);
      v += __shfl_xor(v, 32);
      if (lane < 16) red[(wm * 2 + u) * BN + (wn * TN + j) * 16 + lane] = v;
    }
  __syncthreads();
  const int tid = threadIdx.x;
  if (tid < 2 * BN) {
    const int u = tid / BN, c = tid - u * BN;
    double v = 0.0;
#pragma unroll
    for (int w = 0; w < WM; ++w) v += red[(w * 2 + u) * BN + c];
    p.colsum[((size_t)(m0 / BM) * 2 + u) * p.N + n0 + c] = v;
  }
}

template <int TM, int TN, int WM, int WN>
__device__ __forceinline__ void gemm_epilogue16(const ConvGemmArgs& p, f32x4 (&acc)[TM][TN], int m0, int n0, int wm,
                                                int wn, int lane, unsigned char* smem) {
  if (p.colsum) {
    double cs[TN][2];
#pragma unroll
    for (int j = 0; j < TN; ++j) cs[j][0] = cs[j][1] = 0.0;
    switch (p.act) {
      case kActRelu: gemm_epilogue_store16<TM, TN, kActRelu, false, true>(p, acc, m0, n0, wm, wn, lane, cs); break;
      case kActTanh: gemm_epilogue_store16<TM, TN, kActTanh, false, true>(p, acc, m0, n0, wm, wn, lane, cs); break;
      case kActGelu: gemm_epilogue_store16<TM, TN, kActGelu, false, true>(p, acc, m0, n0, wm, wn, lane, cs); break;
      default: gemm_epilogue_store16<TM, TN, kActNone, false, true>(p, acc, m0, n0, wm, wn, lane, cs); break;
    }
    gemm_colsum_reduce16<TN, WM, WN, WM * TM * 16>(p, cs, m0, n0, wm, wn, lane, smem);
    return;
  }
  if (p.res) {
    switch (p.act) {
      case kActRelu: gemm_epilogue_store16<TM, TN, kActRelu, false, false, true>(p, acc, m0, n0, wm, wn, lane); break;
      case kActTanh: gemm_epilogue_store16<TM, TN, kActTanh, false, false, true>(p, acc, m0, n0, wm, wn, lane); break;
      case kActGelu: gemm_epilogue_store16<TM, TN, kActGelu, false, false, true>(p, acc, m0, n0, wm, wn, lane); break;
      default: gemm_epilogue_store16<TM, TN, kActNone, false, false, true>(p, acc, m0, n0, wm, wn, lane); break;
    }
    return;
  }
  if (p.row_bias) {
    switch (p.act) {
      case kActRelu: gemm_epilogue_store16<TM, TN, kActRelu, true>(p, acc, m0, n0, wm, wn, lane); break;
      case kActTanh: gemm_epilogue_store16<TM, TN, kActTanh, true>(p, acc, m0, n0, wm, wn, lane); break;
      case kActGelu: gemm_epilogue_store16<TM, TN, kActGelu, true>(p, acc, m0, n0, wm, wn, lane); break;
      default: gemm_epilogue_store16<TM, TN, kActNone, true>(p, acc, m0, n0, wm, wn, lane); break;
    }
  } else {
    switch (p.act) {
      case kActRelu: gemm_epilogue_store16<TM, TN, kActRelu, false>(p, acc, m0, n0, wm, wn, lane); break;
      case kActTanh: gemm_epilogue_store16<TM, TN, kActTanh, false>(p, acc, m0, n0, wm, wn, lane); break;
      case kActGelu: gemm_epilogue_store16<TM, TN, kActGelu, false>(p, acc, m0, n0, wm, wn, lane); break;
      default: gemm_epilogue_store16<TM, TN, kActNone, false>(p, acc, m0, n0, wm, wn, lane); break;
    }
  }
}

inline bool uniform_ktiles(const ConvGemmArgs& p) {
  if (p.cin % 32 != 0) return false;
  if (p.amode == kACat && (p.cseg[1] % 32 != 0 || p.cseg[2] % 32 != 0)) return false;
  return true;
}

inline void check_conv_args(const ConvGemmArgs& p, const char* who) {
  const std::string w(who);
  const long long in_rows = (p.conv2d || p.sc2d) ? std::max<long long>(p.M, (long long)(p.M / (p.Fo * p.To)) * p.Fi * p.Ti)
                            : p.seg ? (long long)std::max(p.M, p.Ti)
                                     : std::max<long long>(p.M, (long long)((p.M + p.T - 1) / p.T) * p.Ti);
  for (int i = 0; i < 3; ++i)
    WSP_CHECK(in_rows * p.lda[i] * 4 < (long long)kOOB, w + ": operand exceeds 2 GiB (split the batch)");
  WSP_CHECK((long long)p.M * p.ldo * 4 < (long long)kOOB, w + ": output exceeds 2 GiB (split the batch)");
  if (p.res) WSP_CHECK((long long)p.M * p.ldres * 4 < (long long)kOOB, w + ": residual exceeds 2 GiB");
  WSP_CHECK((long long)p.N * p.Kp * 4 < (long long)kOOB, w + ": weights exceed 2 GiB");
  WSP_CHECK(p.M > 0 && p.N > 0 && p.K > 0 && p.T > 0, w + ": empty shape");
  WSP_CHECK(p.cin % 4 == 0, w + ": cin must be a multiple of 4");
  WSP_CHECK(p.K == p.cin * p.taps, w + ": K != cin * taps");
  WSP_CHECK(p.Kp % 32 == 0 && p.Kp >= p.K, w + ": bad packed K");
  WSP_CHECK(p.N % 32 == 0, w + ": N must be a multiple of 32");
  if (p.conv2d) {
    WSP_CHECK(p.amode == kACat && p.cseg[1] == p.cin && p.cin % 32 == 0,
              w + ": 2-D conv needs one segment with cin % 32 == 0");
    WSP_CHECK(p.M == p.T * p.Fo * p.To || p.T > 0, w + ": bad 2-D shape");
    WSP_CHECK(p.taps % p.kw == 0 && p.stride >= 1, w + ": bad 2-D taps/stride");
  }
  for (int i = 0; i < 3; ++i) WSP_CHECK(p.lda[i] % 4 == 0, w + ": lda must be a multiple of 4");
  if (p.sc2d)
    WSP_CHECK(!p.conv2d && !p.seg && p.taps == 1 && p.pad == 0 && p.amode == kACat && p.cseg[1] % 32 == 0 &&
                  p.cseg[2] == p.cin && p.stride >= 1 && p.Fo >= 1 && p.To >= 1 && p.M % (p.Fo * p.To) == 0 &&
                  (p.Fo - 1) * p.stride < p.Fi && (p.To - 1) * p.stride < p.Ti,
              w + ": conv3 + shortcut needs a dense 1x1 segment and a 2-D strided segment");
  if (!p.conv2d) WSP_CHECK(p.stride >= 1 && p.Ti >= 1, w + ": call normalized() first");
  if (p.seg) WSP_CHECK(!p.conv2d && p.nseg >= 1 && (p.iseg || p.stride == 1), w + ": segmented batch needs a 1-D conv (input offsets when strided)");
  WSP_CHECK(!p.res || (!p.row_bias && !p.colsum), w + ": a residual epilogue has no row bias / column sums");
  if (p.gcols) {
    WSP_CHECK(p.amode == kACat && p.cseg[1] == p.cin && !p.conv2d, w + ": grouped conv needs one 1-D segment");
    WSP_CHECK(p.N % p.gcols == 0 && p.gcols % 32 == 0 && p.gcin % 4 == 0, w + ": bad grouped-conv columns");
    WSP_CHECK(p.res == nullptr, w + ": grouped conv has no residual epilogue");
  }
  if (p.amode == kACat) {
    WSP_CHECK(p.cseg[0] == 0 && p.cseg[3] == p.cin && p.cseg[1] <= p.cseg[2] &&
                  p.cseg[2] <= p.cseg[3],
              w + ": bad channel segments");
    for (int i = 1; i < 3; ++i) WSP_CHECK(p.cseg[i] % 4 == 0, w + ": segment not float4 aligned");
    if (!uniform_ktiles(p))
      WSP_CHECK(p.cseg[1] == p.cin, w + ": multi-segment A needs 32-aligned segments");
  }
}

}
```

wespeaker_hubert_amd/csrc/kernels.h:

```cpp
#pragma once

#include <vector>

#include "common.h"

namespace wsp {

enum AMode { kACat = 0, kAAdd = 1 };
enum Act { kActNone = 0, kActRelu = 1, kActTanh = 2, kActGelu = 3 };

struct ConvGemmArgs {
  const float* a[3];
  int lda[3];
  int cseg[4];
  int cin, taps, dil, pad;
  int M, T, N;
  const float* w;
  int K, Kp;
  const float* bias;
  const float* row_bias;
  const float* res;
  int ldres;
  const float* scale;
  const float* shift;
  float* out;
  int ldo;
  int act;
  int amode;
  int role;
  int conv2d;
  int Fi, Ti, Fo, To, stride, kw;
  int sc2d;
  int gcols, gcin;
  const int* seg;
  const int* iseg;
  int nseg;
  double* colsum;
  int lnmode;
  float* ln_out;
  const float* ln_in;
  int ln_parts;
  const float* ln_cs;
  const float* ln_g;
  const float* ln_b;
  float ln_eps;
};

inline ConvGemmArgs normalized(ConvGemmArgs p) {
  if (!p.conv2d && !p.sc2d) {
    if (p.stride <= 0) p.stride = 1;
    if (p.Ti <= 0) p.Ti = p.T;
  }
  return p;
}

int conv_gemm_x3_block_rows(const ConvGemmArgs& p, int variant);
void launch_colsum_mean(const double* part, int block_rows, int T, int B, int N, float* out, int ldo,
                        hipStream_t s);
void launch_conv_gemm_x3(const ConvGemmArgs& p, const void* whi, const void* wlo, int variant,
                         hipStream_t s);


void launch_conv_gemm(const ConvGemmArgs& p, hipStream_t s);
int conv_gemm_tile_for(int N);

struct SmallLinearArgs {
  const float* in;
  int ldin;
  const float* wt;
  const float* bias;
  float* out;
  int ldo;
  int R, K, N;
  int act;
  float* scratch = nullptr;
  size_t scratch_floats = 0;
};
void launch_small_linear(const SmallLinearArgs& p, hipStream_t s);
size_t small_linear_scratch_floats(int R, int N, int K);


void launch_frame_stats(const float* x, int ldx, int B, int T, int C, float* out, int ldo,
                        int with_std, int std_off, hipStream_t s, const int* seg = nullptr);

void launch_residual_scale(const float* x, const float* h, const float* g, float* out, int B,
                           int T, int C, hipStream_t s, const int* seg = nullptr, int M = 0);

void launch_astp_pool(const float* e, const float* x, int B, int T, int C, float* out,
                      hipStream_t s, const int* seg = nullptr, float var_floor = 1e-7f);

int simam_chunks(int B, int rows);
void launch_simam(const float* z, const float* res, float* out, int B, int rows, int C, double* part, float* coef,
                  hipStream_t s);
void launch_nhwc_to_tfc(const float* in, float* out, int B, int F, int T, int C, hipStream_t s);

void launch_resnet_stem(const float* feats, int B, int T, int F, int C0, const float* w, const float* bias,
                        float* out, hipStream_t s);

struct FbankConfig {
  int num_bins = 80, sample_rate = 16000, window = 0;
  double frame_length_ms = 25.0, frame_shift_ms = 10.0, low_freq = 20.0, high_freq = 0.0;
  int frame_len = 0, frame_shift = 0, padded = 0;
};
void fbank_config_resolve(FbankConfig& c);
void fbank_mel_banks(const FbankConfig& c, std::vector<float>& w);
struct FbankPlan {
  FbankConfig cfg;
  bool fixed = false;
  int len0 = 0, len1 = 0;
  std::vector<double> host_tab;
  const double* tab = nullptr;
};
void fbank_plan(const FbankConfig& c, FbankPlan& p);
void launch_fbank(const void* wav, int dtype, int B, int N, int ld, float scale, float* feats,
                  int T, int cmn, const FbankPlan& plan, hipStream_t s, const int* wseg = nullptr,
                  const int* fseg = nullptr);

void launch_hubert_conv0(const float* wav, int B, int N, int ldw, int T0, const float* w, const float* gamma,
                         const float* beta, double* stats, float* out, hipStream_t s, const int* wseg = nullptr,
                         const int* oseg = nullptr);
size_t hubert_conv0_stats_doubles(int B, int T0);
void launch_hubert_pos_conv(const float* x, int ldx, const int* seg, int B, int maxT, int M, const void* whi,
                            const void* wlo, int ldw, int gout, const float* bias, float* out, int ldo,
                            hipStream_t s);
struct LayerNormArgs {
  const float* x;
  int ldx;
  const float* add;
  int ldadd, gin, gout;
  const float* gamma;
  const float* beta;
  float eps;
  float* out;
  int ldo;
  int M, D;
  float* feat;
  float feat_w;
  int feat_init, T, Tout;
  const int* seg;
  const int* fseg;
  int nseg;
};
void launch_layernorm(const LayerNormArgs& p, hipStream_t s);
void launch_cmn_rows(float* x, int B, int T, int D, hipStream_t s, const int* seg = nullptr);
void launch_cmvn_rows(float* x, int B, int T, int D, int norm_mean, int norm_var, hipStream_t s,
                      const int* seg = nullptr);

void launch_l2_normalize(const float* x, const float* sub, float* y, int R, int D, hipStream_t s);
void launch_cosine_pairs(const float* E, int D, const int32_t* ia, const int32_t* ib, int P,
                         double* score, hipStream_t s);
void asnorm_layout(int Ne, int Nc, int D, int* Ncp, int* Dp, size_t* bytes);
void launch_asnorm_stats(const float* E, int Ne, const float* C, int Nc, int D, int top_n,
                         double* mu, double* sd, float* ws, hipStream_t s);
void launch_row_mean_accum(const float* x, const int32_t* group, int R, int D, double* acc,
                           double* cnt, hipStream_t s);

struct ResamplePlan {
  int orig = 1, nw = 1, width = 0, L = 1;
  bool identity = true;
  std::vector<float> kern;
  std::vector<int> band;
};
void resample_plan(int orig_freq, int new_freq, int lowpass_filter_width, double rolloff, ResamplePlan& p);
long long resample_out_len(const ResamplePlan& p, long long n);
void launch_resample(const ResamplePlan& p, const float* d_kern, const int* d_band, const float* x, int B, int N,
                     long ldx, float* y, long ldy, hipStream_t s);

}
```

wespeaker_hubert_amd/csrc/model.cpp:

```cpp
#include "model_impl.h"

namespace wsp {

int detail::chunk_for(int B, size_t bytes) {
  const int bc = std::min((int)std::max<size_t>(1, kOperandCap / bytes), B);
  const int chunks = (B + bc - 1) / bc;
  return (B + chunks - 1) / chunks;
}

void Model::Impl::add(const std::string& n, std::vector<int64_t> shape) {
  idx[n] = (int)params.size();
  params.push_back(Param{n, std::move(shape), {}, false});
}
void Model::Impl::add_bn(const std::string& p, int64_t c) {
  add(p + ".weight", {c});
  add(p + ".bias", {c});
  add(p + ".running_mean", {c});
  add(p + ".running_var", {c});
  add(p + ".num_batches_tracked", {});
}
const std::vector<float>& Model::Impl::P(const std::string& n) const {
  auto it = idx.find(n);
  WSP_CHECK(it != idx.end(), "missing parameter " + n);
  const Param& p = params[it->second];
  WSP_CHECK(p.set || p.numel() == 0, "parameter not set: " + n);
  return p.host;
}

void Model::Impl::bn_affine(const std::string& p, std::vector<double>& sc, std::vector<double>& sh) const {
  const auto& w = P(p + ".weight");
  const auto& b = P(p + ".bias");
  const auto& rm = P(p + ".running_mean");
  const auto& rv = P(p + ".running_var");
  sc.resize(w.size());
  sh.resize(w.size());
  for (size_t i = 0; i < w.size(); ++i) {
    sc[i] = (double)w[i] / std::sqrt((double)rv[i] + kBnEps);
    sh[i] = (double)b[i] - (double)rm[i] * sc[i];
  }
}

ConvW Model::Impl::pack_conv(const std::vector<float>& w, int N, int cin, int taps, const float* bias,
                             const std::string& bn) {
  ConvW cw;
  cw.N = N;
  cw.cin = cin;
  cw.taps = taps;
  cw.K = cin * taps;
  cw.Kp = round_up(cw.K, 64);
  const std::vector<float> packed = pack::conv_kmajor(w, N, cin, taps, cw.Kp);
  std::vector<uint16_t> hi, lo;
  pack::split(packed, hi, lo);
  cw.w = dev.upload(packed);
  cw.whi = dev.upload_u16(hi);
  cw.wlo = dev.upload_u16(lo);
  if (bias) cw.bias = dev.upload(std::vector<float>(bias, bias + N));
  if (!bn.empty()) {
    std::vector<double> sc, sh;
    bn_affine(bn, sc, sh);
    cw.scale = dev.upload(std::vector<float>(sc.begin(), sc.end()));
    cw.shift = dev.upload(std::vector<float>(sh.begin(), sh.end()));
  }
  return cw;
}

LinW Model::Impl::pack_lin(const float* w, int N, int K, int ldk, const float* bias) {
  LinW lw;
  lw.N = N;
  lw.K = K;
  lw.wt = dev.upload(pack::transpose(w, N, K, ldk));
  if (bias) lw.bias = dev.upload(std::vector<float>(bias, bias + N));
  return lw;
}

void Model::Impl::one_operand(ConvGemmArgs& g, const float* a, int lda, int cin) {
  g.a[0] = g.a[1] = g.a[2] = a;
  g.lda[0] = g.lda[1] = g.lda[2] = lda;
  g.cseg[0] = 0;
  g.cseg[1] = g.cseg[2] = g.cseg[3] = cin;
}

void Model::Impl::fill(ConvGemmArgs& g, const ConvW& cw, int M, int T, int dil, int pad, float* out, int ldo, int act,
                       const float* row_bias, bool use_bias, const int* seg, int nseg) {
  g.cin = cw.cin;
  g.taps = cw.taps;
  g.dil = dil;
  g.pad = pad;
  g.M = M;
  g.T = T;
  g.N = cw.N;
  g.w = cw.w;
  g.K = cw.K;
  g.Kp = cw.Kp;
  g.bias = use_bias ? cw.bias : nullptr;
  g.row_bias = row_bias;
  g.scale = cw.scale;
  g.shift = cw.shift;
  g.out = out;
  g.ldo = ldo;
  g.act = act;
  g.seg = seg;
  g.nseg = nseg;
}

void Model::Impl::launch(const ConvGemmArgs& g, const ConvW& cw, hipStream_t s) {
  if (precision == 1)
    launch_conv_gemm_x3(g, cw.whi, cw.wlo, x3_variant, s);
  else
    launch_conv_gemm(g, s);
}

void Model::Impl::gemm(const char* tag, const ConvW& cw, const float* a0, int lda, float* out, int ldo, int M, int T,
                       int dil, int pad, int act, hipStream_t s, const int* seg, int nseg, const float* row_bias,
                       bool use_bias, int role) {
  ConvGemmArgs g{};
  one_operand(g, a0, lda, cw.cin);
  g.role = role;
  fill(g, cw, M, T, dil, pad, out, ldo, act, row_bias, use_bias, seg, nseg);
  run(tag, 2.0 * M * cw.N * cw.K, s, [&] { launch(g, cw, s); });
}

void Model::Impl::fork(hipStream_t s, int ns) {
  while ((int)sub_st.size() < ns - 1) {
    hipStream_t t;
    WSP_HIP(hipStreamCreateWithFlags(&t, hipStreamNonBlocking));
    sub_st.push_back(t);
  }
  while ((int)sub_ev.size() < ns) {
    hipEvent_t e;
    WSP_HIP(hipEventCreateWithFlags(&e, hipEventDisableTiming));
    sub_ev.push_back(e);
  }
  WSP_HIP(hipEventRecord(sub_ev[0], s));
  for (int i = 1; i < ns; ++i) WSP_HIP(hipStreamWaitEvent(sub_st[i - 1], sub_ev[0], 0));
}
void Model::Impl::join(hipStream_t s, int ns) {
  for (int i = 1; i < ns; ++i) {
    WSP_HIP(hipEventRecord(sub_ev[i], sub_st[i - 1]));
    WSP_HIP(hipStreamWaitEvent(s, sub_ev[i], 0));
  }
}

Model::Model() : impl(new Impl) {}
Model::~Model() {
  for (auto& kv : impl->prof_map)
    for (auto& e : kv.second.ev) {
      (void)hipEventDestroy(e.first);
      (void)hipEventDestroy(e.second);
    }
  for (auto t : impl->sub_st) (void)hipStreamDestroy(t);
  for (auto e : impl->sub_ev) (void)hipEventDestroy(e);
  delete impl;
}

void Model::create(const std::string& arch, int feat_dim, int embed_dim, bool emb_bn, bool two_emb) {
  Impl& m = *impl;
  m.arch = arch;
  m.feat_dim = feat_dim;
  m.embed_dim = embed_dim;
  m.emb_bn = emb_bn;
  m.two_emb = two_emb;
  if (hipGetDevice(&m.device) != hipSuccess) {
    (void)hipGetLastError();
    m.device = -1;
  }
  if (arch == "ECAPA_TDNN_c512" || arch == "ECAPA_TDNN_GLOB_c512" || arch == "ECAPA_TDNN_c1024" ||
      arch == "ECAPA_TDNN_GLOB_c1024") {
    m.ecapa = true;
    m.x3_variant = 7;
    m.C = (arch.find("c1024") != std::string::npos) ? 1024 : 512;
    m.glob = arch.find("GLOB") != std::string::npos;
    WSP_CHECK(feat_dim > 0 && feat_dim % 4 == 0, "ECAPA feat_dim must be a positive multiple of 4");
    WSP_CHECK(embed_dim > 0, "embed_dim must be positive");
    m.build_ecapa_params();
  } else if (arch.rfind("ResNet", 0) == 0) {
    static const std::map<std::string, std::pair<bool, std::vector<int>>> kRes = {
        {"ResNet18", {false, {2, 2, 2, 2}}},     {"ResNet34", {false, {3, 4, 6, 3}}},
        {"ResNet50", {true, {3, 4, 6, 3}}},      {"ResNet101", {true, {3, 4, 23, 3}}},
        {"ResNet152", {true, {3, 8, 36, 3}}},    {"ResNet221", {true, {6, 16, 48, 3}}},
        {"ResNet293", {true, {10, 20, 64, 3}}}};
    auto it = kRes.find(arch);
    WSP_CHECK(it != kRes.end(), "unsupported arch " + arch);
    WSP_CHECK(feat_dim >= 8 && feat_dim % 8 == 0, "ResNet feat_dim must be a positive multiple of 8");
    m.ecapa = false;
    m.x3_variant = it->second.first ? 7 : 4;
    m.streams = 2;
    m.bottleneck = it->second.first;
    for (int i = 0; i < 4; ++i) m.nblocks[i] = it->second.second[i];
    m.build_resnet_params();
  } else if (arch == "SimAM_ResNet34_ASP" || arch == "SimAM_ResNet100_ASP") {
    WSP_CHECK(!two_emb && !emb_bn, "SimAM-ResNet has no emb_bn / two_emb_layer");
    WSP_CHECK(feat_dim >= 8 && feat_dim % 8 == 0, "SimAM-ResNet acoustic_dim must be a multiple of 8");
    WSP_CHECK(embed_dim > 0, "embed_dim must be positive");
    m.ecapa = false;
    m.simam = true;
    m.bottleneck = false;
    m.x3_variant = 5;
    m.streams = 2;
    m.m_ch = 64;
    const int nb34[4] = {3, 4, 6, 3}, nb100[4] = {6, 16, 24, 3};
    for (int i = 0; i < 4; ++i) m.nblocks[i] = arch == "SimAM_ResNet34_ASP" ? nb34[i] : nb100[i];
    m.build_simam_params();
  } else if (arch == "HuBERT_base" || arch == "WavLM_base") {
    WSP_CHECK(embed_dim == 768, arch + " output size is 768");
    m.ecapa = false;
    m.hubert = true;
    m.wavlm = arch == "WavLM_base";
    m.feat_dim = 1;
    m.x3_variant = 7;
    m.streams = 2;
    m.build_hubert_params();
  } else {
    throw InvalidArg{"unsupported arch " + arch};
  }
}

int Model::num_params() const { return (int)impl->params.size(); }

void Model::param_info(int i, const char** name, int* ndim, int64_t* shape) const {
  WSP_CHECK(i >= 0 && i < num_params(), "param index out of range");
  const Param& p = impl->params[i];
  *name = p.name.c_str();
  *ndim = (int)p.shape.size();
  for (size_t d = 0; d < p.shape.size() && d < 4; ++d) shape[d] = p.shape[d];
}

void Model::set_param(int i, const float* data, int64_t numel) {
  WSP_CHECK(i >= 0 && i < num_params(), "param index out of range");
  Param& p = impl->params[i];
  WSP_CHECK(numel == p.numel(), "numel mismatch for " + p.name);
  p.host.assign(data, data + numel);
  p.set = true;
}

void Model::finalize() {
  Impl& m = *impl;
  WSP_CHECK(!m.finalized, "model already finalized");
  int dev = 0;
  WSP_HIP(hipGetDevice(&dev));
  WSP_CHECK(m.device < 0 || dev == m.device, "finalize on a different device than create");
  m.device = dev;
  for (auto& p : m.params)
    WSP_CHECK(p.set || p.name.find("num_batches_tracked") != std::string::npos,
              "parameter not set: " + p.name);
  if (m.ecapa)
    m.finalize_ecapa();
  else if (m.simam)
    m.finalize_simam();
  else if (m.hubert)
    m.finalize_hubert();
  else
    m.finalize_resnet();
  for (auto& p : m.params) std::vector<float>().swap(p.host);
  m.finalized = true;
}

int Model::embed_dim() const { return impl->embed_dim; }
int Model::feat_dim() const { return impl->feat_dim; }

size_t Model::Impl::ws_bytes_one(int B, int T) const {
  const int bc = ecapa ? ecapa_chunk(B, T) : B;
  const size_t f = ecapa ? ecapa_ws_floats(bc, (size_t)bc * T) : resnet_ws_floats(B, T);
  return (f * sizeof(float) + 255) & ~size_t(255);
}

size_t Model::workspace_bytes(int B, int T) const {
  WSP_CHECK(!impl->hubert, "HuBERT handle: use the front-end workspace query");
  const int ns = impl->nsub(B);
  size_t bytes = 256;
  for (int i = 0; i < ns; ++i) bytes += impl->ws_bytes_one(B * (i + 1) / ns - B * i / ns, T);
  return bytes;
}

void Model::forward(const float* feats, int B, int T, float* embed, void* ws, size_t ws_bytes,
                    hipStream_t s) {
  Impl& m = *impl;
  WSP_CHECK(!m.hubert, "HuBERT handle: use the front-end forward");
  WSP_CHECK(m.finalized, "forward before finalize");
  WSP_CHECK(B > 0 && T > 1, "forward needs B >= 1 and T >= 2 frames");
  WSP_CHECK((size_t)B * T < (1u << 31), "B*T too large");
  WSP_CHECK(ws_bytes >= workspace_bytes(B, T), "workspace too small");
  WSP_CHECK(m.ecapa || m.precision == 1, "ResNet runs on the bf16x3 kernels only (precision=1)");
  WSP_CHECK(!m.simam || (T + 7) / 8 >= 2, "SimAM-ResNet needs >= 2 frames after the three stride-2 stages");
  char* wsb = reinterpret_cast<char*>((reinterpret_cast<uintptr_t>(ws) + 255) & ~uintptr_t(255));
  const int ns = m.nsub(B);
  if (ns > 1) m.fork(s, ns);
  for (int i = 0; i < ns; ++i) {
    const int b0 = B * i / ns, nb = B * (i + 1) / ns - b0;
    const float* f = feats + (size_t)b0 * T * m.feat_dim;
    float* e = embed + (size_t)b0 * m.embed_dim;
    float* wsf = reinterpret_cast<float*>(wsb);
    const hipStream_t si = m.sub(s, i);
    if (m.ecapa) {
      const int bc = m.ecapa_chunk(nb, T);
      for (int c0 = 0; c0 < nb; c0 += bc)
        m.forward_ecapa(f + (size_t)c0 * T * m.feat_dim, std::min(bc, nb - c0), T, e + (size_t)c0 * m.embed_dim, wsf,
                        si);
    } else if (m.simam)
      m.forward_simam(f, nb, T, e, wsf, si);
    else
      m.forward_resnet(f, nb, T, e, wsf, si);
    wsb += m.ws_bytes_one(nb, T);
  }
  if (ns > 1) m.join(s, ns);
}

size_t Model::workspace_bytes_segments(int B, int M) const {
  WSP_CHECK(impl->ecapa, "segmented batches are implemented for ECAPA-TDNN handles");
  WSP_CHECK(B > 0 && M >= B, "segmented batch needs B >= 1 and M >= B rows");
  return impl->ecapa_ws_floats(B, (size_t)M) * sizeof(float) + 256;
}

void Model::forward_segments(const float* feats, int B, const int* seg, int M, float* embed, void* ws,
                             size_t ws_bytes, hipStream_t s) {
  Impl& m = *impl;
  WSP_CHECK(m.ecapa, "segmented batches are implemented for ECAPA-TDNN handles");
  WSP_CHECK(m.finalized, "forward before finalize");
  WSP_CHECK(seg != nullptr && B > 0 && M >= B, "segmented batch needs offsets, B >= 1 and M >= B rows");
  WSP_CHECK((size_t)M * 1536 < (1u << 31) / 4, "segmented batch too large");
  WSP_CHECK(ws_bytes >= workspace_bytes_segments(B, M), "workspace too small");
  float* wsf = reinterpret_cast<float*>((reinterpret_cast<uintptr_t>(ws) + 255) & ~uintptr_t(255));
  m.forward_ecapa(feats, B, 1, embed, wsf, s, seg, M);
}

void Model::profile(bool on) {
  if (on && !impl->prof)
    for (auto& kv : impl->prof_map) {
      kv.second.used = 0;
      kv.second.flops = 0;
    }
  impl->prof = on;
}

namespace {
struct Opt {
  const char* key;
  int Model::Impl::*field;
  int lo, hi, hole;
  const char* err;
};
using I = Model::Impl;
constexpr int kNoHole = -1000;
const Opt kOpts[] = {
    {"precision", &I::precision, 0, 1, kNoHole, "precision must be 0 (f32) or 1 (bf16x3)"},
    {"streams", &I::streams, 1, 8, kNoHole, "streams must be 1..8"},
    {"layer", &I::h_layer_sel, -1, 12, kNoHole, "layer must be -1 (weighted sum) or 0..12"},
    {"in_planes", &I::m_ch, 32, 64, kNoHole, "in_planes must be 32 or 64"},
    {"res2_fused", &I::res2_fused, 0, 1, kNoHole, "res2_fused must be 0 or 1"},
    {"cat_gate", &I::cat_gate, 0, 1, kNoHole, "cat_gate must be 0 or 1"},
    {"res_prefetch", &I::res_prefetch, 0, 1, kNoHole, "res_prefetch must be 0 or 1"},
    {"res_tail", &I::res_tail, 0, 2, kNoHole, "res_tail must be 0 (off), 1 (tail + next conv1) or 2 (tail alone)"},
    {"sc_fuse", &I::sc_fuse, 0, 3, kNoHole, "sc_fuse must be 0 .. 3 (bit 0: one GEMM, bit 1: in the tail)"},
    {"c1_stage_fuse", &I::c1_stage_fuse, 0, 1, kNoHole, "c1_stage_fuse must be 0 or 1"},
    {"astp_fused", &I::astp_fused_on, 0, 3, kNoHole,
     "astp_fused must be 0 (linear2 GEMM + pooling kernel) or 1 (fused)"},
    {"attn_pipe", &I::attn_pipe, 0, 1, kNoHole, "attn_pipe must be 0 or 1"},
    {"pos_conv", &I::pos_conv, 0, 1, kNoHole,
     "pos_conv must be 0 (grouped implicit GEMM) or 1 (direct grouped conv)"},
    {"ln_fold", &I::ln_fold, 0, 1, kNoHole, "ln_fold must be 0 (LayerNorm kernels) or 1 (folded into the GEMMs)"},
    {"tail_batch", &I::tail_batch, 0, 1, kNoHole,
     "tail_batch must be 0 (CNN layers 4-6 per chunk) or 1 (batch-wide)"},
    {"res2_variant", &I::res2_variant, 0, 4, 1,
     "res2_variant must be 0 (4 waves, 2 x 2), 2 (4 waves on N, 4 W k-steps in flight), 3 (8 waves) "
     "or 4 (halo-free strips, c1024 widths; else as 3)"},
    {"x3_variant", &I::x3_variant, 0, 9, kNoHole,
     "x3_variant must be 3, 4, 5, 6 (5 on 16x16x32 MFMAs) or 7 (6 staged by LDS-DMA)"},
    {"conv3x3_img", &I::conv3x3_img_on, 0, 3, kNoHole,
     "conv3x3_img must be 0 (off), 1 (32 / 64 channels) or 2 / 3 (also 128)"},
};
const Opt& find_opt(const std::string& key) {
  for (const Opt& o : kOpts)
    if (key == o.key) return o;
  throw InvalidArg{"unknown option " + key};
}
}

void Model::set_option(const std::string& key, int value) {
  Impl& m = *impl;
  if (key == "attn_lds" || key == "conv1x1_rows") return;
  const Opt& o = find_opt(key);
  if (key == "layer") {
    WSP_CHECK(m.hubert, "option 'layer' applies to the HuBERT front end");
    WSP_CHECK(!m.finalized, "option 'layer' must be set before finalize");
  } else if (key == "in_planes") {
    WSP_CHECK(m.simam, "option 'in_planes' applies to SimAM-ResNet handles");
    WSP_CHECK(!m.finalized, "option 'in_planes' must be set before finalize");
    WSP_CHECK(value == 32 || value == 64, o.err);
    for (const auto& p : m.params) WSP_CHECK(!p.set, "option 'in_planes' must be set before the weights");
  }
  WSP_CHECK(value >= o.lo && value <= o.hi && value != o.hole, o.err);
  if (key == "x3_variant") {
    value = value >= 3 && value <= 7 ? value : value == 8 ? 7 : 5;
  } else if (key == "astp_fused") {
    value = value ? 1 : 0;
  }
  m.*o.field = value;
  if (key == "in_planes") m.build_simam_params();
}

int Model::get_option(const std::string& key) const { return impl->*find_opt(key).field; }

void Model::profile_query(const std::string& tag, int* launches, double* total_ms, double* flops) {
  *launches = 0;
  *total_ms = 0;
  *flops = 0;
  double fl = 0;
  for (auto& kv : impl->prof_map) {
    const std::string& k = kv.first;
    if (k != tag && k.compare(0, tag.size() + 1, tag + ".") != 0) continue;
    ProfEntry& e = kv.second;
    for (size_t i = 0; i < e.used; ++i) {
      WSP_HIP(hipEventSynchronize(e.ev[i].second));
      float ms = 0;
      WSP_HIP(hipEventElapsedTime(&ms, e.ev[i].first, e.ev[i].second));
      *total_ms += ms;
    }
    *launches += (int)e.used;
    fl += e.flops;
  }
  *flops = *launches ? fl / (double)*launches : 0.0;
}

}
```

wespeaker_hubert_amd/csrc/model_impl.h:

```cpp
#pragma once

#include <hip/hip_runtime.h>

#include <cmath>
#include <cstdint>
#include <algorithm>
#include <map>
#include <string>
#include <vector>

#include "kernels.h"
#include "model.h"
#include "pack.h"
#include "res2_chain.h"
#include "astp_fused.h"
#include "conv3x3_img.h"

namespace wsp {

namespace detail {

constexpr double kBnEps = 1e-5;

struct DevBuf {
  std::vector<void*> ptrs;
  ~DevBuf() {
    for (void* p : ptrs) (void)hipFree(p);
  }
  void* upload_u16(const std::vector<uint16_t>& v) {
    void* p = nullptr;
    WSP_HIP(hipMalloc(&p, std::max<size_t>(v.size(), 1) * sizeof(uint16_t)));
    ptrs.push_back(p);
    if (!v.empty()) WSP_HIP(hipMemcpy(p, v.data(), v.size() * sizeof(uint16_t), hipMemcpyHostToDevice));
    return p;
  }
  float* upload(const std::vector<float>& v) {
    void* p = nullptr;
    WSP_HIP(hipMalloc(&p, std::max<size_t>(v.size(), 1) * sizeof(float)));
    ptrs.push_back(p);
    if (!v.empty()) WSP_HIP(hipMemcpy(p, v.data(), v.size() * sizeof(float), hipMemcpyHostToDevice));
    return static_cast<float*>(p);
  }
};

struct ConvW {
  float* w = nullptr;
  void* whi = nullptr;
  void* wlo = nullptr;
  float* bias = nullptr;
  float* scale = nullptr;
  float* shift = nullptr;
  int N = 0, cin = 0, taps = 1, K = 0, Kp = 0;
  void* frag = nullptr;
};

struct LinW {
  float* wt = nullptr;
  float* bias = nullptr;
  int K = 0, N = 0;
};

inline int round_up(int a, int b) { return (a + b - 1) / b * b; }

constexpr size_t kOperandCap = ((size_t)1 << 31) / 8 * 7;
int chunk_for(int B, size_t bytes);

struct WsCursor {
  float* base = nullptr;
  size_t off = 0;
  static size_t padded(size_t n) { return (n + 63) / 64 * 64; }
  float* take(size_t n) {
    float* p = base ? base + off : nullptr;
    off += padded(n);
    return p;
  }
};

}

using namespace detail;

struct HubertChunk {
  int b0 = 0, b1 = 0;
  size_t off = 0;
  size_t rows[7] = {};
  size_t samples = 0, sample0 = 0, row6 = 0;
  size_t row3 = 0;
  int maxT0 = 0;
};
struct HubertPlan {
  int B = 0;
  size_t M = 0, Mout = 0, maxA = 0, maxB = 0;
  size_t M3 = 0, M4 = 0, M5 = 0;
  bool tail_batch = false;
  int maxChunk = 0, maxT6 = 0;
  size_t maxStats = 0;
  std::vector<HubertChunk> chunks;
  std::vector<int> offs;
};

struct Param {
  std::string name;
  std::vector<int64_t> shape;
  std::vector<float> host;
  bool set = false;
  int64_t numel() const {
    int64_t n = 1;
    for (auto s : shape) n *= s;
    return n;
  }
};

struct ProfEntry {
  std::vector<std::pair<hipEvent_t, hipEvent_t>> ev;
  size_t used = 0;
  double flops = 0;
};

struct Model::Impl {
  std::string arch;
  bool ecapa = true;
  int C = 512;
  bool glob = false;
  int feat_dim = 80, embed_dim = 192;
  bool emb_bn = false, two_emb = false;
  std::vector<Param> params;
  std::map<std::string, int> idx;
  bool finalized = false;
  int device = 0;
  DevBuf dev;

  ConvW layer1;
  struct Block {
    ConvW c1, c3, res2[7];
    LinW se1, se2;
    void* r2w = nullptr;
    float *r2b = nullptr, *r2s = nullptr, *r2t = nullptr;
  } blk[3];
  int res2_fused = 1;
  int res2_variant = 4;
  ConvW conv, pool1, pool2;
  ConvW conv_g;
  int cat_gate = 1;
  void* pool2_frag = nullptr;
  int astp_fused_on = 1;
  LinW pool1_ctx;
  LinW head;
  void build_ecapa_params();
  void pack_res2(Block& b, const std::string& p, int w);
  void finalize_ecapa();
  int ecapa_chunk(int B, int T) const;
  size_t ecapa_ws_floats(int B, size_t M) const;
  void forward_ecapa(const float* feats, int B, int T, float* embed, float* ws, hipStream_t s,
                     const int* seg = nullptr, int M_seg = 0);

  bool bottleneck = true;
  int nblocks[4] = {0, 0, 0, 0};
  int m_ch = 32;
  float* stem_w = nullptr;
  float* stem_b = nullptr;
  int conv3x3_img_on = 2;
  int res_prefetch = 1;
  int res_tail = 1;
  int sc_fuse = 3;
  int c1_stage_fuse = 1;
  bool img_ok(const ConvW& cw, int C) const { return cw.frag && conv3x3_img_on && (C <= 64 || conv3x3_img_on >= 2); }
  struct RBlock {
    ConvW c1, c2, c3, sc;
    ConvW c3sc;
    void* w3acc = nullptr;
    void* w3scx = nullptr;
    float* b3scx = nullptr;
    void* w1frag = nullptr;
    bool has_sc = false;
    int stride = 1, in_planes = 0, planes = 0, out_planes = 0;
    std::string name;
    int li = 0, bi = 0;
  };
  std::vector<RBlock> rblocks;
  LinW seg1, seg2;
  bool simam = false;
  ConvW asp1, asp2;
  LinW simam_head;
  struct RShapes {
    size_t big = 0, y1 = 0, y2 = 0, sc = 0;
    int F4 = 0, T4 = 0, C4 = 0;
  };
  void build_res_blocks(const std::string& pre, const char* sc_conv, const char* sc_bn);
  void build_resnet_params();
  void build_simam_params();
  ConvW pack_conv_bn(const std::string& wname, const std::string& bn, int N, int cin, int taps,
                     void** acc_frag = nullptr, void** b_frag = nullptr);
  void finalize_res_blocks(const std::string& pre, const char* sc_conv, const char* sc_bn);
  void finalize_resnet();
  void finalize_simam();
  RShapes resnet_shapes(int T) const;
  int resnet_chunk(int B, int T) const;
  size_t resnet_ws_floats(int B, int T) const;
  void gemm2d(const char* tag, const ConvW& cw, const float* a0, int lda, float* out, int ldo, int B, int Fi, int Ti,
              int kw, int stride, int pad, int act, const float* res, int ldres, hipStream_t s);
  void gemm1x1(const char* tag, const ConvW& cw, const float* a0, float* out, int M, int act, const float* res,
               hipStream_t s);
  void gemm_c3sc(const char* tag, const RBlock& rb, const float* y2, const float* x, int Ci, float* out, int B, int Fi,
                 int Ti, int Fo, int To, hipStream_t s);
  void conv3x3(const char* tag, const ConvW& cw, const float* in, int ldin, float* out, int B, int Fi, int Ti,
               int stride, bool relu, const float* res, hipStream_t s);
  void forward_resnet(const float* feats, int B, int T, float* embed, float* ws, hipStream_t s);
  void forward_simam(const float* feats, int B, int T, float* embed, float* ws, hipStream_t s);

  bool hubert = false;
  float* h_conv0_w = nullptr;
  float* h_gn_g = nullptr;
  float* h_gn_b = nullptr;
  ConvW h_conv[7];
  float* h_ln0_g = nullptr;
  float* h_ln0_b = nullptr;
  ConvW h_proj, h_pos;
  float* h_enc_g = nullptr;
  float* h_enc_b = nullptr;
  struct HLayer {
    ConvW qkv, out, fc1, fc2;
    float *ln1_g = nullptr, *ln1_b = nullptr, *ln2_g = nullptr, *ln2_b = nullptr;
    ConvW fc1f;
    float* fc1_cs = nullptr;
    float* gate_w = nullptr;
  };
  bool wavlm = false;
  float* h_rel_tab = nullptr;
  std::vector<HLayer> h_layers;
  std::vector<float> h_fw;
  int h_layer_sel = -1;
  int attn_pipe = 1;
  int pos_conv = 1;
  int ln_fold = 0;
  int tail_batch = 1;
  void build_hubert_params();
  void finalize_hubert();
  int hubert_cnn_frames(int N, int upto) const;
  HubertPlan hubert_plan(int B, const int* lens) const;
  size_t hubert_ws_floats(const HubertPlan& pl) const;
  void forward_hubert(const float* wav, const HubertPlan& pl, float* feats, int cmn, float* ws, hipStream_t s);

  int precision = 1;
  int x3_variant = 5;

  int streams = 1;
  std::vector<hipStream_t> sub_st;
  std::vector<hipEvent_t> sub_ev;
  int nsub(int B) const { return std::max(1, std::min(streams, B)); }
  size_t ws_bytes_one(int B, int T) const;
  hipStream_t sub(hipStream_t s, int i) const { return i == 0 ? s : sub_st[i - 1]; }
  void fork(hipStream_t s, int ns);
  void join(hipStream_t s, int ns);

  void add(const std::string& n, std::vector<int64_t> shape);
  void add_bn(const std::string& p, int64_t c);
  const std::vector<float>& P(const std::string& n) const;
  void bn_affine(const std::string& p, std::vector<double>& sc, std::vector<double>& sh) const;

  ConvW pack_conv(const std::vector<float>& w, int N, int cin, int taps, const float* bias, const std::string& bn);
  void* pack_frag(const std::vector<float>& w, int N, int K, pack::FragOrder order = pack::kPlain, int kacc = -1) {
    return dev.upload_u16(pack::frag(w, N, K, order, kacc));
  }
  void* pack_frag_acc(const std::vector<float>& w, int N, int K, int kacc = -1) { return pack_frag(w, N, K, pack::kAcc, kacc); }
  LinW pack_lin(const float* w, int N, int K, int ldk, const float* bias);

  static void one_operand(ConvGemmArgs& g, const float* a, int lda, int cin);
  void fill(ConvGemmArgs& g, const ConvW& cw, int M, int T, int dil, int pad, float* out, int ldo, int act,
            const float* row_bias, bool use_bias, const int* seg, int nseg);
  void launch(const ConvGemmArgs& g, const ConvW& cw, hipStream_t s);
  void gemm(const char* tag, const ConvW& cw, const float* a0, int lda, float* out, int ldo, int M, int T, int dil,
            int pad, int act, hipStream_t s, const int* seg, int nseg, const float* row_bias = nullptr,
            bool use_bias = true, int role = 0);

  bool prof = false;
  std::map<std::string, ProfEntry> prof_map;
  template <typename F>
  void run(const char* tag, double flops, hipStream_t s, F&& f) {
    if (!prof) {
      f();
      return;
    }
    ProfEntry& e = prof_map[tag];
    if (e.used == e.ev.size()) {
      hipEvent_t a, b;
      WSP_HIP(hipEventCreate(&a));
      WSP_HIP(hipEventCreate(&b));
      e.ev.emplace_back(a, b);
    }
    auto& pr = e.ev[e.used++];
    e.flops += flops;
    WSP_HIP(hipEventRecord(pr.first, s));
    f();
    WSP_HIP(hipEventRecord(pr.second, s));
  }
};

}
```

wespeaker_hubert_amd/csrc/ops.hip:

```cpp
#include "kernels.h"

namespace wsp {

namespace {
constexpr int kRB = 4;
constexpr int kSW = 16;

__global__ __launch_bounds__(64 * kSW) void small_linear_kernel(const SmallLinearArgs p) {
  __shared__ float part[kSW][kRB][64];
  const int lane = threadIdx.x & 63;
  const int wave = threadIdx.x >> 6;
  const int n = blockIdx.y * 64 + lane;
  const int r0 = blockIdx.x * kRB;
  const int kq = (p.K + kSW - 1) / kSW;
  const int k0 = wave * kq, k1 = min(p.K, k0 + kq);
  float acc[kRB];
#pragma unroll
  for (int r = 0; r < kRB; ++r) acc[r] = 0.f;
  const float* in[kRB];
#pragma unroll
  for (int r = 0; r < kRB; ++r) in[r] = p.in + (long)min(r0 + r, p.R - 1) * p.ldin;
  if (n < p.N) {
    const float* w = p.wt + n;
    int k = k0;
    for (; k + 4 <= k1; k += 4) {
      const float w0 = w[(long)k * p.N], w1 = w[(long)(k + 1) * p.N];
      const float w2 = w[(long)(k + 2) * p.N], w3 = w[(long)(k + 3) * p.N];
#pragma unroll
      for (int r = 0; r < kRB; ++r) {
        float a = acc[r];
        a = fmaf(in[r][k], w0, a);
        a = fmaf(in[r][k + 1], w1, a);
        a = fmaf(in[r][k + 2], w2, a);
        a = fmaf(in[r][k + 3], w3, a);
        acc[r] = a;
      }
    }
    for (; k < k1; ++k) {
      const float w0 = w[(long)k * p.N];
#pragma unroll
      for (int r = 0; r < kRB; ++r) acc[r] = fmaf(in[r][k], w0, acc[r]);
    }
  }
#pragma unroll
  for (int r = 0; r < kRB; ++r) part[wave][r][lane] = acc[r];
  __syncthreads();
  if (wave < kRB && n < p.N) {
    const int r = wave;
    if (r0 + r >= p.R) return;
    float y = 0.f;
#pragma unroll
    for (int w = 0; w < kSW; ++w) y += part[w][r][lane];
    y += p.bias ? p.bias[n] : 0.f;
    if (p.act == 1) y = fmaxf(y, 0.f);
    else if (p.act == 2) y = tanhf(y);
    else if (p.act == 3) y = 1.f / (1.f + expf(-y));
    p.out[(long)(r0 + r) * p.ldo + n] = y;
  }
}

constexpr int kSKR = 16;
__global__ __launch_bounds__(64 * kSW) void small_linear_splitk_kernel(const SmallLinearArgs p, int kslice) {
  __shared__ float part[kSW][kSKR][64];
  const int lane = threadIdx.x & 63;
  const int wave = threadIdx.x >> 6;
  const int n = blockIdx.y * 64 + lane;
  const int r0 = blockIdx.x * kSKR;
  const int ks = blockIdx.z;
  const int kb = ks * kslice, ke = min(p.K, kb + kslice);
  const int kq = (ke - kb + kSW - 1) / kSW;
  const int k0 = kb + wave * kq, k1 = min(ke, k0 + kq);
  float acc[kSKR];
#pragma unroll
  for (int r = 0; r < kSKR; ++r) acc[r] = 0.f;
  if (n < p.N) {
    const float* w = p.wt + n;
    for (int k = k0; k < k1; ++k) {
      const float wk = w[(long)k * p.N];
#pragma unroll
      for (int r = 0; r < kSKR; ++r) acc[r] = fmaf(p.in[(long)min(r0 + r, p.R - 1) * p.ldin + k], wk, acc[r]);
    }
  }
#pragma unroll
  for (int r = 0; r < kSKR; ++r) part[wave][r][lane] = acc[r];
  __syncthreads();
  if (wave < kSKR && n < p.N && r0 + wave < p.R) {
    float y = 0.f;
#pragma unroll
    for (int w = 0; w < kSW; ++w) y += part[w][wave][lane];
    p.scratch[((size_t)ks * p.R + r0 + wave) * p.N + n] = y;
  }
}

__global__ __launch_bounds__(256) void small_linear_reduce_kernel(const SmallLinearArgs p, int nks) {
  const int i = blockIdx.x * 256 + threadIdx.x;
  if (i >= p.R * p.N) return;
  const int r = i / p.N, n = i - r * p.N;
  float y = 0.f;
  for (int ks = 0; ks < nks; ++ks) y += p.scratch[(size_t)ks * p.R * p.N + i];
  y += p.bias ? p.bias[n] : 0.f;
  if (p.act == 1) y = fmaxf(y, 0.f);
  else if (p.act == 2) y = tanhf(y);
  else if (p.act == 3) y = 1.f / (1.f + expf(-y));
  p.out[(long)r * p.ldo + n] = y;
}
}

size_t small_linear_scratch_floats(int R, int N, int K) {
  if (K < 4096) return 0;
  const int kslice = std::max(256, (ceil_div(K, 32) + 63) / 64 * 64);
  return (size_t)ceil_div(K, kslice) * R * N;
}

void launch_small_linear(const SmallLinearArgs& p, hipStream_t s) {
  if (p.R == 0) return;
  const int rb = ceil_div(p.R, kSKR), nb = ceil_div(p.N, 64);
  if (p.scratch && p.K >= 4096) {
    const int kslice = std::max(256, (ceil_div(p.K, 32) + 63) / 64 * 64);
    const int nks = ceil_div(p.K, kslice);
    WSP_CHECK((size_t)nks * p.R * p.N <= p.scratch_floats, "small_linear: split-K scratch too small");
    hipLaunchKernelGGL(small_linear_splitk_kernel, dim3(rb, nb, nks), dim3(64 * kSW), 0, s, p, kslice);
    WSP_HIP(hipGetLastError());
    hipLaunchKernelGGL(small_linear_reduce_kernel, dim3(ceil_div(p.R * p.N, 256)), dim3(256), 0, s, p, nks);
    WSP_HIP(hipGetLastError());
    return;
  }
  dim3 grid(ceil_div(p.R, kRB), ceil_div(p.N, 64));
  hipLaunchKernelGGL(small_linear_kernel, grid, dim3(64 * kSW), 0, s, p);
  WSP_HIP(hipGetLastError());
}

namespace {
__global__ __launch_bounds__(256) void frame_stats_kernel(const float* __restrict__ x, int ldx,
                                                          int T_, int C, float* __restrict__ out,
                                                          int ldo, int with_std, int std_off,
                                                          const int* __restrict__ seg) {
  __shared__ float part[4][64];
  __shared__ float s_mean[64];
  const int b = blockIdx.x;
  const int tid = threadIdx.x, lane = tid & 63, wave = tid >> 6;
  const int c = blockIdx.y * 64 + lane;
  const bool ok = c < C;
  const int T = seg ? seg[b + 1] - seg[b] : T_;
  const float* xb = x + (seg ? (long)seg[b] : (long)b * T_) * ldx + c;
  float s = 0.f;
  if (ok)
    for (int t = wave; t < T; t += 4) s += xb[(long)t * ldx];
  part[wave][lane] = s;
  __syncthreads();
  if (wave == 0) {
    const float m = (part[0][lane] + part[1][lane] + part[2][lane] + part[3][lane]) / (float)T;
    s_mean[lane] = m;
    if (ok) out[(long)b * ldo + c] = m;
  }
  __syncthreads();
  if (!with_std) return;
  const float m = s_mean[lane];
  float q = 0.f;
  if (ok)
    for (int t = wave; t < T; t += 4) {
      const float d = xb[(long)t * ldx] - m;
      q = fmaf(d, d, q);
    }
  __syncthreads();
  part[wave][lane] = q;
  __syncthreads();
  if (wave == 0 && ok) {
    const float v = (part[0][lane] + part[1][lane] + part[2][lane] + part[3][lane]) / (float)(T - 1);
    out[(long)b * ldo + std_off + c] = sqrtf(v + 1e-7f);
  }
}

__global__ __launch_bounds__(256) void frame_stats4_kernel(const float* __restrict__ x, int ldx, int T_,
                                                           int C, float* __restrict__ out, int ldo,
                                                           int with_std, int std_off,
                                                           const int* __restrict__ seg) {
  __shared__ double part[4][4][64];
  __shared__ float s_mean[4][64];
  const int b = blockIdx.x;
  const int tid = threadIdx.x, lane = tid & 63, wave = tid >> 6;
  const int c = (blockIdx.y * 64 + lane) * 4;
  const bool ok = c < C;
  const int T = seg ? seg[b + 1] - seg[b] : T_;
  const float* xb = x + (seg ? (long)seg[b] : (long)b * T_) * ldx + (ok ? c : 0);
  auto row = [&](int t) { return *reinterpret_cast<const f32x4*>(xb + (long)t * ldx); };
  double a[4] = {0.0, 0.0, 0.0, 0.0};
  int t = wave;
  if (ok) {
    for (; t + 12 < T; t += 16) {
      const f32x4 r0 = row(t), r1 = row(t + 4), r2 = row(t + 8), r3 = row(t + 12);
#pragma unroll
      for (int e = 0; e < 4; ++e) a[e] += ((double)r0[e] + (double)r1[e]) + ((double)r2[e] + (double)r3[e]);
    }
    for (; t < T; t += 4) {
      const f32x4 r0 = row(t);
#pragma unroll
      for (int e = 0; e < 4; ++e) a[e] += (double)r0[e];
    }
  }
#pragma unroll
  for (int e = 0; e < 4; ++e) part[wave][e][lane] = a[e];
  __syncthreads();
  if (wave == 0) {
    f32x4 m;
#pragma unroll
    for (int e = 0; e < 4; ++e) {
      m[e] = (float)((part[0][e][lane] + part[1][e][lane] + part[2][e][lane] + part[3][e][lane]) / (double)T);
      s_mean[e][lane] = m[e];
    }
    if (ok) *reinterpret_cast<f32x4*>(out + (long)b * ldo + c) = m;
  }
  __syncthreads();
  if (!with_std) return;
  double q[4] = {0.0, 0.0, 0.0, 0.0};
  float m[4];
#pragma unroll
  for (int e = 0; e < 4; ++e) m[e] = s_mean[e][lane];
  if (ok)
    for (t = wave; t < T; t += 4) {
      const f32x4 r0 = row(t);
#pragma unroll
      for (int e = 0; e < 4; ++e) {
        const double d = (double)(r0[e] - m[e]);
        q[e] += d * d;
      }
    }
  __syncthreads();
#pragma unroll
  for (int e = 0; e < 4; ++e) part[wave][e][lane] = q[e];
  __syncthreads();
  if (wave == 0 && ok) {
    f32x4 r;
#pragma unroll
    for (int e = 0; e < 4; ++e) {
      const double v = (part[0][e][lane] + part[1][e][lane] + part[2][e][lane] + part[3][e][lane]) / (double)(T - 1);
      r[e] = sqrtf((float)v + 1e-7f);
    }
    float* o = out + (long)b * ldo + std_off + c;
    if (((ldo | std_off) & 3) == 0) *reinterpret_cast<f32x4*>(o) = r;
    else for (int e = 0; e < 4; ++e) o[e] = r[e];
  }
}
}

void launch_frame_stats(const float* x, int ldx, int B, int T, int C, float* out, int ldo,
                        int with_std, int std_off, hipStream_t s, const int* seg) {
  if (B == 0) return;
  const bool vec = C % 4 == 0 && ldx % 4 == 0 && ldo % 4 == 0 &&
                   (reinterpret_cast<uintptr_t>(x) & 15) == 0 && (reinterpret_cast<uintptr_t>(out) & 15) == 0;
  if (vec) {
    dim3 grid(B, ceil_div(C, 256));
    hipLaunchKernelGGL(frame_stats4_kernel, grid, dim3(256), 0, s, x, ldx, T, C, out, ldo, with_std, std_off,
                       seg);
  } else {
    dim3 grid(B, ceil_div(C, 64));
    hipLaunchKernelGGL(frame_stats_kernel, grid, dim3(256), 0, s, x, ldx, T, C, out, ldo, with_std,
                       std_off, seg);
  }
  WSP_HIP(hipGetLastError());
}

namespace {
constexpr int kRSRows = 64;

template <bool HX>
__global__ __launch_bounds__(256) void residual_scale_kernel(const f32x4* __restrict__ x,
                                                             const f32x4* __restrict__ h,
                                                             const float* __restrict__ g,
                                                             f32x4* __restrict__ out, int M, int T, int C4,
                                                             const int* __restrict__ seg, int nseg) {
  const int tpr = min(C4, 256);
  const int rpp = 256 / tpr;
  const int sub = threadIdx.x / tpr;
  const int r0 = blockIdx.x * kRSRows;
  const int r1 = min(M, r0 + kRSRows);
  for (int c4 = threadIdx.x % tpr; c4 < C4; c4 += tpr) {
    int r = r0 + sub;
    for (; r + 7 * rpp < r1; r += 8 * rpp) {
      f32x4 xv[8], hv[8], gv[8];
#pragma unroll
      for (int u = 0; u < 8; ++u) {
        const long i = (long)(r + u * rpp) * C4 + c4;
        xv[u] = HX ? __builtin_nontemporal_load(x + i) : f32x4{0.f, 0.f, 0.f, 0.f};
        hv[u] = __builtin_nontemporal_load(h + i);
      }
#pragma unroll
      for (int u = 0; u < 8; ++u) {
        const int row = r + u * rpp;
        const int b = seg ? seg_of(seg, nseg, row) : row / T;
        gv[u] = *reinterpret_cast<const f32x4*>(g + ((long)b * C4 + c4) * 4);
      }
#pragma unroll
      for (int u = 0; u < 8; ++u) out[(long)(r + u * rpp) * C4 + c4] = HX ? xv[u] + hv[u] * gv[u] : hv[u] * gv[u];
    }
    for (; r < r1; r += rpp) {
      const int b = seg ? seg_of(seg, nseg, r) : r / T;
      const long i = (long)r * C4 + c4;
      const f32x4 gv = *reinterpret_cast<const f32x4*>(g + ((long)b * C4 + c4) * 4);
      out[i] = HX ? x[i] + h[i] * gv : h[i] * gv;
    }
  }
}
}

void launch_residual_scale(const float* x, const float* h, const float* g, float* out, int B,
                           int T, int C, hipStream_t s, const int* seg, int M) {
  WSP_CHECK(C % 4 == 0, "residual_scale: C % 4");
  const int C4 = C / 4;
  WSP_CHECK(C4 % 256 == 0 || 256 % C4 == 0, "residual_scale: C/4 must divide or be a multiple of 256");
  const int rows = seg ? M : B * T;
  if (rows == 0) return;
  const dim3 grid(ceil_div(rows, kRSRows));
  const f32x4* x4 = reinterpret_cast<const f32x4*>(x);
  const f32x4* h4 = reinterpret_cast<const f32x4*>(h);
  f32x4* o4 = reinterpret_cast<f32x4*>(out);
  if (x)
    hipLaunchKernelGGL(residual_scale_kernel<true>, grid, dim3(256), 0, s, x4, h4, g, o4, rows, T, C4, seg, B);
  else
    hipLaunchKernelGGL(residual_scale_kernel<false>, grid, dim3(256), 0, s, x4, h4, g, o4, rows, T, C4, seg, B);
  WSP_HIP(hipGetLastError());
}

namespace {
__global__ __launch_bounds__(256) void astp_pool_kernel(const float* __restrict__ e,
                                                        const float* __restrict__ x, int T_, int C,
                                                        float* __restrict__ out, const int* __restrict__ seg,
                                                        float floor_) {
  __shared__ float sm[4][4][64];
  const int b = blockIdx.x;
  const int tid = threadIdx.x, lane = tid & 63, wave = tid >> 6;
  const int c = blockIdx.y * 64 + lane;
  const bool ok = c < C;
  float mx = -INFINITY, se = 0.f, a1 = 0.f, a2 = 0.f;
  const int T = seg ? seg[b + 1] - seg[b] : T_;
  if (ok) {
    const long base = (seg ? (long)seg[b] : (long)b * T_) * C + c;
    for (int t = wave; t < T; t += 4) {
      const float ev = e[base + (long)t * C];
      const float xv = x[base + (long)t * C];
      if (ev > mx) {
        const float sc = expf(mx - ev);
        se = se * sc + 1.f;
        a1 = a1 * sc + xv;
        a2 = a2 * sc + xv * xv;
        mx = ev;
      } else {
        const float pe = expf(ev - mx);
        se += pe;
        a1 = fmaf(pe, xv, a1);
        a2 = fmaf(pe * xv, xv, a2);
      }
    }
  }
  sm[wave][0][lane] = mx;
  sm[wave][1][lane] = se;
  sm[wave][2][lane] = a1;
  sm[wave][3][lane] = a2;
  __syncthreads();
  if (wave == 0 && ok) {
    float M = sm[0][0][lane];
    for (int w = 1; w < 4; ++w) M = fmaxf(M, sm[w][0][lane]);
    float S = 0.f, A1 = 0.f, A2 = 0.f;
    for (int w = 0; w < 4; ++w) {
      const float m = sm[w][0][lane];
      const float f = (m == -INFINITY) ? 0.f : expf(m - M);
      S += sm[w][1][lane] * f;
      A1 += sm[w][2][lane] * f;
      A2 += sm[w][3][lane] * f;
    }
    const float mean = A1 / S;
    const float var = A2 / S - mean * mean;
    out[(long)b * 2 * C + c] = mean;
    out[(long)b * 2 * C + C + c] = sqrtf(fmaxf(var, floor_));
  }
}

__global__ __launch_bounds__(256) void astp_pool4_kernel(const float* __restrict__ e,
                                                         const float* __restrict__ x, int T_, int C,
                                                         float* __restrict__ out, const int* __restrict__ seg,
                                                         float floor_) {
  __shared__ f32x4 sm[4][4][64];
  const int b = blockIdx.x;
  const int tid = threadIdx.x, lane = tid & 63, wave = tid >> 6;
  const int c = (blockIdx.y * 64 + lane) * 4;
  const bool ok = c < C;
  const f32x4 z = {0.f, 0.f, 0.f, 0.f};
  f32x4 mx = {-INFINITY, -INFINITY, -INFINITY, -INFINITY}, se = z, a1 = z, a2 = z;
  const int T = seg ? seg[b + 1] - seg[b] : T_;
  auto step = [&](const f32x4& ev, const f32x4& xv) {
#pragma unroll
    for (int k = 0; k < 4; ++k) {
      const float m1 = fmaxf(mx[k], ev[k]);
      const float sc = __expf(mx[k] - m1);
      const float pe = __expf(ev[k] - m1);
      se[k] = fmaf(se[k], sc, pe);
      a1[k] = fmaf(a1[k], sc, pe * xv[k]);
      a2[k] = fmaf(a2[k], sc, pe * xv[k] * xv[k]);
      mx[k] = m1;
    }
  };
  if (ok) {
    const long base = (seg ? (long)seg[b] : (long)b * T_) * C + c;
    auto ld = [&](const float* p, int t) { return *reinterpret_cast<const f32x4*>(p + base + (long)t * C); };
    int t = wave;
    for (; t + 4 < T; t += 8) {
      const f32x4 e0 = ld(e, t), x0 = ld(x, t), e1 = ld(e, t + 4), x1 = ld(x, t + 4);
      step(e0, x0);
      step(e1, x1);
    }
    if (t < T) step(ld(e, t), ld(x, t));
  }
  sm[wave][0][lane] = mx;
  sm[wave][1][lane] = se;
  sm[wave][2][lane] = a1;
  sm[wave][3][lane] = a2;
  __syncthreads();
  if (wave == 0 && ok) {
    f32x4 mean, sd;
#pragma unroll
    for (int k = 0; k < 4; ++k) {
      float M = sm[0][0][lane][k];
      for (int w = 1; w < 4; ++w) M = fmaxf(M, sm[w][0][lane][k]);
      float S = 0.f, A1 = 0.f, A2 = 0.f;
      for (int w = 0; w < 4; ++w) {
        const float m = sm[w][0][lane][k];
        const float f = (m == -INFINITY) ? 0.f : __expf(m - M);
        S += sm[w][1][lane][k] * f;
        A1 += sm[w][2][lane][k] * f;
        A2 += sm[w][3][lane][k] * f;
      }
      mean[k] = A1 / S;
      sd[k] = sqrtf(fmaxf(A2 / S - mean[k] * mean[k], floor_));
    }
    *reinterpret_cast<f32x4*>(out + (long)b * 2 * C + c) = mean;
    *reinterpret_cast<f32x4*>(out + (long)b * 2 * C + C + c) = sd;
  }
}
}

void launch_astp_pool(const float* e, const float* x, int B, int T, int C, float* out,
                      hipStream_t s, const int* seg, float var_floor) {
  if (B == 0) return;
  const bool vec = C % 4 == 0 && ((reinterpret_cast<uintptr_t>(e) | reinterpret_cast<uintptr_t>(x) |
                                   reinterpret_cast<uintptr_t>(out)) & 15) == 0;
  if (vec) {
    dim3 grid(B, ceil_div(C, 256));
    hipLaunchKernelGGL(astp_pool4_kernel, grid, dim3(256), 0, s, e, x, T, C, out, seg, var_floor);
  } else {
    dim3 grid(B, ceil_div(C, 64));
    hipLaunchKernelGGL(astp_pool_kernel, grid, dim3(256), 0, s, e, x, T, C, out, seg, var_floor);
  }
  WSP_HIP(hipGetLastError());
}

}

namespace wsp {

namespace {
template <int C0>
__global__ __launch_bounds__(256) void resnet_stem_kernel(const float* __restrict__ feats, int T, int F,
                                                          const float* __restrict__ w,
                                                          const float* __restrict__ bias,
                                                          float* __restrict__ out, long total) {
  __shared__ float s_w[C0 * 9];
  __shared__ float s_b[C0];
  for (int i = threadIdx.x; i < C0 * 9; i += 256) s_w[i] = w[i];
  for (int i = threadIdx.x; i < C0; i += 256) s_b[i] = bias[i];
  __syncthreads();
  const long idx = blockIdx.x * 256L + threadIdx.x;
  if (idx >= total) return;
  const int t = (int)(idx % T);
  const long bf = idx / T;
  const int f = (int)(bf % F);
  const int b = (int)(bf / F);
  float x[9];
#pragma unroll
  for (int kf = 0; kf < 3; ++kf)
#pragma unroll
    for (int kt = 0; kt < 3; ++kt) {
      const int ff = f + kf - 1, tt = t + kt - 1;
      x[kf * 3 + kt] = (ff >= 0 && ff < F && tt >= 0 && tt < T) ? feats[((long)b * T + tt) * F + ff] : 0.f;
    }
  f32x4* o = reinterpret_cast<f32x4*>(out + idx * C0);
#pragma unroll
  for (int c4 = 0; c4 < C0 / 4; ++c4) {
    f32x4 v;
#pragma unroll
    for (int e = 0; e < 4; ++e) {
      const int c = c4 * 4 + e;
      float a = s_b[c];
#pragma unroll
      for (int q = 0; q < 9; ++q) a = fmaf(x[q], s_w[c * 9 + q], a);
      v[e] = fmaxf(a, 0.f);
    }
    o[c4] = v;
  }
}
}

void launch_resnet_stem(const float* feats, int B, int T, int F, int C0, const float* w, const float* bias,
                        float* out, hipStream_t s) {
  WSP_CHECK(C0 == 32 || C0 == 64, "resnet stem: m_channels must be 32 or 64");
  const long total = (long)B * F * T;
  if (total == 0) return;
  const unsigned grid = (unsigned)((total + 255) / 256);
  if (C0 == 32)
    hipLaunchKernelGGL(resnet_stem_kernel<32>, dim3(grid), dim3(256), 0, s, feats, T, F, w, bias, out, total);
  else
    hipLaunchKernelGGL(resnet_stem_kernel<64>, dim3(grid), dim3(256), 0, s, feats, T, F, w, bias, out, total);
  WSP_HIP(hipGetLastError());
}

}
```

Measured before the change: 25480.

## Pre-split GEMM-only ECAPA activations into bf16 hi/lo in residual-scale producer

The residual-scale kernel can now write its output directly as interleaved bf16 hi/lo pairs (split8 format), using a DPP lane swap to pack 8-value groups. The bf16x3 tile-family-7 GEMM reads such A segments raw instead of converting fp32 to hi/lo per k-tile, avoiding repeated split work and keeping the same byte footprint. It is enabled by default for the block-3 conv1 input and the concatenated conv_cat segments when the GEMM path supports it. It adds a per-k-tile segment-format branch in the mixed case and restricts those buffers to GEMM-only consumers.

```diff
diff --git a/include/wespeaker_amd.h b/include/wespeaker_amd.h
--- a/include/wespeaker_amd.h
+++ b/include/wespeaker_amd.h
@@ -78,6 +78,7 @@
 
 int wsp_model_set_option(wsp_model* m, const char* key, int value);
 int wsp_model_get_option(const wsp_model* m, const char* key, int* value);
+int wsp_gemm_reads_split8(int precision, int x3_variant, int n, int cin, int cseg1, int cseg2);
 
 int wsp_model_profile(wsp_model* m, int enable);
 int wsp_model_profile_query(wsp_model* m, const char* kernel_class, int* launches,
diff --git a/wespeaker_hubert_amd/_lib.py b/wespeaker_hubert_amd/_lib.py
--- a/wespeaker_hubert_amd/_lib.py
+++ b/wespeaker_hubert_amd/_lib.py
@@ -54,6 +54,7 @@
                                            c_size_t, c_void_p]),
     "wsp_model_set_option": (c_int, [c_void_p, c_char_p, c_int]),
     "wsp_model_get_option": (c_int, [c_void_p, c_char_p, POINTER(c_int)]),
+    "wsp_gemm_reads_split8": (c_int, [c_int, c_int, c_int, c_int, c_int, c_int]),
     "wsp_frontend_out_frames": (c_int, [c_void_p, c_int, POINTER(c_int)]),
     "wsp_frontend_workspace_bytes": (c_int, [c_void_p, c_int, c_int, POINTER(c_size_t)]),
     "wsp_frontend_forward": (c_int, [c_void_p, c_void_p, c_int, c_int, c_void_p, c_int, c_void_p, c_size_t,
diff --git a/wespeaker_hubert_amd/csrc/capi.cpp b/wespeaker_hubert_amd/csrc/capi.cpp
--- a/wespeaker_hubert_amd/csrc/capi.cpp
+++ b/wespeaker_hubert_amd/csrc/capi.cpp
@@ -302,6 +302,17 @@
   });
 }
 
+int wsp_gemm_reads_split8(int precision, int x3_variant, int n, int cin, int cseg1, int cseg2) {
+  wsp::ConvGemmArgs g{};
+  g.amode = wsp::kACat;
+  g.cseg[1] = cseg1;
+  g.cseg[2] = cseg2;
+  g.cseg[3] = g.cin = g.K = g.Kp = cin;
+  g.taps = 1;
+  g.N = n;
+  return wsp::conv_gemm_reads_split8(g, precision, x3_variant) ? 1 : 0;
+}
+
 int wsp_model_profile(wsp_model* m, int enable) {
   WSP_GUARD({
     WSP_CHECK(m, "null model");
diff --git a/wespeaker_hubert_amd/csrc/conv_gemm.hip b/wespeaker_hubert_amd/csrc/conv_gemm.hip
--- a/wespeaker_hubert_amd/csrc/conv_gemm.hip
+++ b/wespeaker_hubert_amd/csrc/conv_gemm.hip
@@ -133,6 +133,7 @@
   const ConvGemmArgs p = normalized(args);
   check_conv_args(p, "conv_gemm");
   WSP_CHECK(!p.colsum, "conv_gemm: column sums are a bf16x3-kernel epilogue");
+  WSP_CHECK(!has_split8(p), "conv_gemm (f32): split8 A segments are read by bf16x3 tile family 7 only");
   WSP_CHECK(!p.conv2d && p.N % 64 == 0, "conv_gemm (f32): 1-D convs with N % 64 == 0 only");
   WSP_CHECK(!p.gcols || p.gcols % 64 == 0, "conv_gemm (f32): grouped columns must be a multiple of 64");
   if (conv_gemm_tile_for(p.N) == 0 && !p.gcols)
diff --git a/wespeaker_hubert_amd/csrc/conv_gemm_x3.hip b/wespeaker_hubert_amd/csrc/conv_gemm_x3.hip
--- a/wespeaker_hubert_amd/csrc/conv_gemm_x3.hip
+++ b/wespeaker_hubert_amd/csrc/conv_gemm_x3.hip
@@ -32,6 +32,11 @@
   WSP_HIP(hipGetLastError());
 }
 
+bool conv_gemm_reads_split8(const ConvGemmArgs& args, int precision, int variant) {
+  const ConvGemmArgs p = normalized(args);
+  return precision == 1 && variant == 7 && x3::g256_supported(p) && x3::g256_takes_split8(p);
+}
+
 void launch_conv_gemm_x3(const ConvGemmArgs& args, const void* whi, const void* wlo, int variant,
                          hipStream_t s) {
   const ConvGemmArgs p = normalized(args);
@@ -50,6 +55,9 @@
             "conv_gemm_x3: the LayerNorm fold runs on tile family 7 only");
   WSP_CHECK(!p.sc2d || (variant == 7 && x3::g256_supported(p)),
             "conv_gemm_x3: conv3 + shortcut runs on tile family 7 only (N % 256 == 0, 16-B aligned operands)");
+  WSP_CHECK(!has_split8(p) || (variant == 7 && x3::g256_supported(p) && x3::g256_takes_split8(p)),
+            "conv_gemm_x3: split8 A segments are read by tile family 7's dense 1x1 kernels only (x3_variant 7, "
+            "N % 256 == 0, 16-B aligned epilogue operands, no column sums, LayerNorm fold or 2-D segment)");
   if (variant == 7 && x3::g256_supported(p)) {
     x3::t_g256(p, h, l, s);
     return;
diff --git a/wespeaker_hubert_amd/csrc/conv_gemm_x3_impl.h b/wespeaker_hubert_amd/csrc/conv_gemm_x3_impl.h
--- a/wespeaker_hubert_amd/csrc/conv_gemm_x3_impl.h
+++ b/wespeaker_hubert_amd/csrc/conv_gemm_x3_impl.h
@@ -325,6 +325,7 @@
 void t_4x2_2x4_sw1(const ConvGemmArgs&, const __bf16*, const __bf16*, hipStream_t);
 void t_4x2_2x4_mf16(const ConvGemmArgs&, const __bf16*, const __bf16*, hipStream_t);
 bool g256_supported(const ConvGemmArgs&);
+bool g256_takes_split8(const ConvGemmArgs&);
 void t_g256(const ConvGemmArgs&, const __bf16*, const __bf16*, hipStream_t);
 }
 
diff --git a/wespeaker_hubert_amd/csrc/conv_gemm_x3_t6.hip b/wespeaker_hubert_amd/csrc/conv_gemm_x3_t6.hip
--- a/wespeaker_hubert_amd/csrc/conv_gemm_x3_t6.hip
+++ b/wespeaker_hubert_amd/csrc/conv_gemm_x3_t6.hip
@@ -240,7 +240,7 @@
   }
 }
 
-template <int AM, bool CSK, int LNM = 0, int XP = 0>
+template <int AM, bool CSK, int LNM = 0, int XP = 0, int SPL = 0>
 __global__ __launch_bounds__(512, 1) void conv_gemm_g(const ConvGemmArgs p, const __bf16* __restrict__ whi,
                                                       const __bf16* __restrict__ wlo) {
   using L = Lds<true, 16>;
@@ -353,13 +353,16 @@
 #pragma unroll
     for (int j = 0; j < 8; ++j) acc[i][j] = f32x4{0.f, 0.f, 0.f, 0.f};
   bf16x8 ah[2], al[2], bh[4], bl[4];
-  auto rdA = [&](const unsigned char* st, int ih) {
+  auto rdA = [&](const unsigned char* st, int ih, auto s8) {
 #pragma unroll
     for (int i = 0; i < 2; ++i) {
       const int r = wm * 64 + (ih * 2 + i) * 16 + r16;
       const f32x4 x0 = *reinterpret_cast<const f32x4*>(st + g_aslot(r, 2 * qk));
       const f32x4 x1 = *reinterpret_cast<const f32x4*>(st + g_aslot(r, 2 * qk + 1));
-      if constexpr (XP == 1 || XP == 4) {
+      bool raw = XP == 1 || XP == 4;
+      if constexpr (std::is_same_v<decltype(s8), bool>) raw = s8;
+      else raw = raw || decltype(s8)::value;
+      if (raw) {
         ah[i] = __builtin_bit_cast(bf16x8, x0);
         al[i] = __builtin_bit_cast(bf16x8, x1);
         continue;
@@ -400,11 +403,32 @@
   dma(1, 1);
   asm volatile("s_waitcnt vmcnt(8)" ::: "memory");
   __builtin_amdgcn_s_barrier();
-  for (int kt = 0; kt < nk; ++kt) {
+  auto ktile = [&](int kt, auto s8) {
     const int buf = kt & 1;
     const unsigned char* st = smem + buf * kGStage;
-    if constexpr (XP == 2) {
-      rdA(st, 0);
+    rdA(st, 0, s8);
+    rdB(st, 0);
+    mm(0, 0);
+    rdB(st, 1);
+    mm(0, 1);
+    rdA(st, 1, s8);
+    mm(1, 1);
+    rdB(st, 0);
+    mm(1, 0);
+    if constexpr (XP >= 3) {
+      asm volatile("s_waitcnt lgkmcnt(0)" ::: "memory");
+      return;
+    }
+    asm volatile("s_waitcnt vmcnt(0) lgkmcnt(0)" ::: "memory");
+    __builtin_amdgcn_s_barrier();
+    __builtin_amdgcn_sched_barrier(0);
+    if (kt + 2 < nk) dma(kt + 2, buf);
+  };
+  if constexpr (XP == 2) {
+    for (int kt = 0; kt < nk; ++kt) {
+      const int buf = kt & 1;
+      const unsigned char* st = smem + buf * kGStage;
+      rdA(st, 0, std::false_type{});
       rdB(st, 0);
       mm(0, 0);
       __builtin_amdgcn_sched_barrier(0);
@@ -415,32 +439,24 @@
       __builtin_amdgcn_sched_barrier(0);
       if (kt >= 1 && kt + 1 < nk) dma(kt + 1, buf ^ 1, 2);
       __builtin_amdgcn_sched_barrier(0);
-      rdA(st, 1);
+      rdA(st, 1, std::false_type{});
       mm(1, 1);
       rdB(st, 0);
       mm(1, 0);
       asm volatile("s_waitcnt vmcnt(0) lgkmcnt(0)" ::: "memory");
       __builtin_amdgcn_s_barrier();
       __builtin_amdgcn_sched_barrier(0);
-      continue;
-    }
-    rdA(st, 0);
-    rdB(st, 0);
-    mm(0, 0);
-    rdB(st, 1);
-    mm(0, 1);
-    rdA(st, 1);
-    mm(1, 1);
-    rdB(st, 0);
-    mm(1, 0);
-    if constexpr (XP >= 3) {
-      asm volatile("s_waitcnt lgkmcnt(0)" ::: "memory");
-      continue;
-    }
-    asm volatile("s_waitcnt vmcnt(0) lgkmcnt(0)" ::: "memory");
-    __builtin_amdgcn_s_barrier();
-    __builtin_amdgcn_sched_barrier(0);
-    if (kt + 2 < nk) dma(kt + 2, buf);
+    }
+  } else if constexpr (SPL == 1) {
+    int rc = 0;
+    for (int kt = 0; kt < nk; ++kt) {
+      const int sg = rc >= p.cseg[2] ? 2 : rc >= p.cseg[1] ? 1 : 0;
+      ktile(kt, p.afmt[sg] == kASplit8);
+      rc += 32;
+      if (rc >= p.cin) rc -= p.cin;
+    }
+  } else {
+    for (int kt = 0; kt < nk; ++kt) ktile(kt, std::bool_constant<SPL == 2>{});
   }
 #define WSP_GEPI(RB, RES)                                                                                   \
   switch (p.act) {                                                                                         \
@@ -668,6 +684,11 @@
          (!p.sc2d || (uniform_ktiles(p) && !p.colsum && !p.lnmode && !p.row_bias));
 }
 
+bool g256_takes_split8(const ConvGemmArgs& p) {
+  const bool dense = p.taps == 1 && p.pad == 0 && p.stride == 1 && !p.iseg && (p.seg || p.Ti == p.T);
+  return uniform_ktiles(p) && dense && !p.colsum && !p.lnmode && !p.sc2d;
+}
+
 void t_g256(const ConvGemmArgs& p, const __bf16* h, const __bf16* l, hipStream_t s) {
   const int nwg = ((p.M + 255) / 256) * (p.N / 256);
   constexpr int lds0 = 2 * kGStage > kGEpiBytes ? 2 * kGStage : kGEpiBytes;
@@ -692,6 +713,17 @@
       case 5: hipLaunchKernelGGL((conv_gemm_g<1, false, 5>), dim3(nwg), dim3(512), lds, s, p, h, l); break;
       default: WSP_CHECK(false, "conv_gemm_x3: lnmode must be 1, 2, 4 or 5");
     }
+    WSP_HIP(hipGetLastError());
+    return;
+  }
+  if (has_split8(p)) {
+    WSP_CHECK(g256_takes_split8(p), "conv_gemm_x3: split8 A segments need a dense 1x1 GEMM on uniform k-tiles");
+    bool all = true;
+    for (int i = 0; i < 3; ++i) all = all && (p.cseg[i + 1] == p.cseg[i] || p.afmt[i] == kASplit8);
+    if (all)
+      hipLaunchKernelGGL((conv_gemm_g<1, false, 0, 0, 2>), dim3(nwg), dim3(512), lds, s, p, h, l);
+    else
+      hipLaunchKernelGGL((conv_gemm_g<1, false, 0, 0, 1>), dim3(nwg), dim3(512), lds, s, p, h, l);
     WSP_HIP(hipGetLastError());
     return;
   }
diff --git a/wespeaker_hubert_amd/csrc/ecapa_model.cpp b/wespeaker_hubert_amd/csrc/ecapa_model.cpp
--- a/wespeaker_hubert_amd/csrc/ecapa_model.cpp
+++ b/wespeaker_hubert_amd/csrc/ecapa_model.cpp
@@ -154,6 +154,26 @@
 
 size_t Model::Impl::ecapa_ws_floats(int B, size_t M) const { return ecapa_ws(C, B, M, nullptr).floats; }
 
+int Model::Impl::ecapa_presplit_plan() const {
+  if (!a_presplit || !cat_gate) return 0;
+  auto reads = [&](int N, int cin, int c1, int c2) {
+    ConvGemmArgs g{};
+    g.amode = kACat;
+    g.cseg[1] = c1;
+    g.cseg[2] = c2;
+    g.cseg[3] = g.cin = g.K = g.Kp = cin;
+    g.taps = 1;
+    g.N = g.T = g.M = N;
+    return conv_gemm_reads_split8(g, precision, x3_variant);
+  };
+  int plan = 0;
+  if (reads(1536, 3 * C, C, 2 * C)) {
+    plan |= kSplitD4;
+    if (reads(C, C, C, C)) plan |= kSplitX3;
+  }
+  return plan;
+}
+
 void Model::Impl::forward_ecapa(const float* feats, int B, int T, float* embed, float* ws, hipStream_t s,
                                 const int* seg, int M_seg) {
   const int M = seg ? M_seg : B * T, w = C / 8;
@@ -162,6 +182,7 @@
   float *h1 = W.h1, *h2 = W.h2, *h3 = W.h3, *xp = W.xp;
   const int se_bm = precision == 1 ? conv_gemm_x3_block_rows(ConvGemmArgs{.N = C}, x3_variant) : 0;
   const bool se_fused = precision == 1 && !seg && T >= se_bm;
+  const int split = ecapa_presplit_plan();
   auto gemm3 = [&](const char* tag, ConvGemmArgs& g, const ConvW& cw, int dil, int pad, float* out, int ldo) {
     g.lda[0] = g.lda[1] = g.lda[2] = C;
     fill(g, cw, M, T, dil, pad, out, ldo, kActRelu, nullptr, true, seg, B);
@@ -173,7 +194,8 @@
     const Block& b = blk[li];
     const int dil = li + 2;
     const float* xin = x[li + 1];
-    gemm("conv1x1_CxC", b.c1, xin, C, h1, C, M, T, 1, 0, kActRelu, s, seg, B, nullptr, true, 1);
+    gemm("conv1x1_CxC", b.c1, xin, C, h1, C, M, T, 1, 0, kActRelu, s, seg, B, nullptr, true, 1,
+         li == 2 && (split & kSplitX3) ? kASplit8 : kAF32);
     if (precision == 1 && res2_fused && b.r2w) {
       Res2Args r{};
       r.x = h1;
@@ -222,7 +244,8 @@
       else launch_frame_stats(h3, C, B, T, C, W.gmean, C, 0, 0, s, seg);
       launch_small_linear({W.gmean, C, b.se1.wt, b.se1.bias, W.ghid, 128, B, C, 128, 1}, s);
       launch_small_linear({W.ghid, 128, b.se2.wt, b.se2.bias, W.gate, C, B, 128, C, 3}, s);
-      launch_residual_scale(cat_gate && li == 2 ? nullptr : xin, h3, W.gate, x[li + 2], B, T, C, s, seg, M);
+      const bool s8 = (li == 1 && (split & kSplitX3)) || (li == 2 && (split & kSplitD4));
+      launch_residual_scale(cat_gate && li == 2 ? nullptr : xin, h3, W.gate, x[li + 2], B, T, C, s, seg, M, s8);
     });
   }
   {
@@ -234,6 +257,8 @@
     g.cseg[1] = C;
     g.cseg[2] = 2 * C;
     g.cseg[3] = 3 * C;
+    g.afmt[1] = split & kSplitX3 ? kASplit8 : kAF32;
+    g.afmt[2] = split & kSplitD4 ? kASplit8 : kAF32;
     gemm3("conv_cat", g, cat_gate ? conv_g : conv, 1, 0, xp, 1536);
   }
   if (glob) {
diff --git a/wespeaker_hubert_amd/csrc/gemm_common.h b/wespeaker_hubert_amd/csrc/gemm_common.h
--- a/wespeaker_hubert_amd/csrc/gemm_common.h
+++ b/wespeaker_hubert_amd/csrc/gemm_common.h
@@ -554,6 +554,13 @@
     if (!uniform_ktiles(p))
       WSP_CHECK(p.cseg[1] == p.cin, w + ": multi-segment A needs 32-aligned segments");
   }
-}
-
-}
+  for (int i = 0; i < 3; ++i) {
+    WSP_CHECK(p.afmt[i] == kAF32 || p.afmt[i] == kASplit8, w + ": A segment format must be fp32 or split8");
+    if (p.afmt[i] == kASplit8)
+      WSP_CHECK(p.amode == kACat && !p.conv2d && !p.sc2d && !p.gcols && uniform_ktiles(p) && p.lda[i] % 8 == 0 &&
+                    (reinterpret_cast<uintptr_t>(p.a[i]) & 31) == 0,
+                w + ": a split8 A segment needs a 1-D concatenated operand on uniform k-tiles, 32-B aligned rows");
+  }
+}
+
+}
diff --git a/wespeaker_hubert_amd/csrc/kernels.h b/wespeaker_hubert_amd/csrc/kernels.h
--- a/wespeaker_hubert_amd/csrc/kernels.h
+++ b/wespeaker_hubert_amd/csrc/kernels.h
@@ -44,7 +44,12 @@
   const float* ln_g;
   const float* ln_b;
   float ln_eps;
+  int afmt[3];
 };
+enum AFmt { kAF32 = 0, kASplit8 = 1 };
+inline bool has_split8(const ConvGemmArgs& p) {
+  return p.afmt[0] == kASplit8 || p.afmt[1] == kASplit8 || p.afmt[2] == kASplit8;
+}
 
 inline ConvGemmArgs normalized(ConvGemmArgs p) {
   if (!p.conv2d && !p.sc2d) {
@@ -59,6 +64,7 @@
                         hipStream_t s);
 void launch_conv_gemm_x3(const ConvGemmArgs& p, const void* whi, const void* wlo, int variant,
                          hipStream_t s);
+bool conv_gemm_reads_split8(const ConvGemmArgs& p, int precision, int variant);
 
 
 void launch_conv_gemm(const ConvGemmArgs& p, hipStream_t s);
@@ -84,7 +90,8 @@
                         int with_std, int std_off, hipStream_t s, const int* seg = nullptr);
 
 void launch_residual_scale(const float* x, const float* h, const float* g, float* out, int B,
-                           int T, int C, hipStream_t s, const int* seg = nullptr, int M = 0);
+                           int T, int C, hipStream_t s, const int* seg = nullptr, int M = 0,
+                           bool split8 = false);
 
 void launch_astp_pool(const float* e, const float* x, int B, int T, int C, float* out,
                       hipStream_t s, const int* seg = nullptr, float var_floor = 1e-7f);
diff --git a/wespeaker_hubert_amd/csrc/model.cpp b/wespeaker_hubert_amd/csrc/model.cpp
--- a/wespeaker_hubert_amd/csrc/model.cpp
+++ b/wespeaker_hubert_amd/csrc/model.cpp
@@ -112,9 +112,10 @@
 
 void Model::Impl::gemm(const char* tag, const ConvW& cw, const float* a0, int lda, float* out, int ldo, int M, int T,
                        int dil, int pad, int act, hipStream_t s, const int* seg, int nseg, const float* row_bias,
-                       bool use_bias, int role) {
+                       bool use_bias, int role, int afmt) {
   ConvGemmArgs g{};
   one_operand(g, a0, lda, cw.cin);
+  g.afmt[0] = g.afmt[1] = g.afmt[2] = afmt;
   g.role = role;
   fill(g, cw, M, T, dil, pad, out, ldo, act, row_bias, use_bias, seg, nseg);
   run(tag, 2.0 * M * cw.N * cw.K, s, [&] { launch(g, cw, s); });
@@ -348,6 +349,7 @@
     {"in_planes", &I::m_ch, 32, 64, kNoHole, "in_planes must be 32 or 64"},
     {"res2_fused", &I::res2_fused, 0, 1, kNoHole, "res2_fused must be 0 or 1"},
     {"cat_gate", &I::cat_gate, 0, 1, kNoHole, "cat_gate must be 0 or 1"},
+    {"a_presplit", &I::a_presplit, 0, 1, kNoHole, "a_presplit must be 0 (fp32 activations) or 1 (GEMM-only ones pre-split)"},
     {"res_prefetch", &I::res_prefetch, 0, 1, kNoHole, "res_prefetch must be 0 or 1"},
     {"res_tail", &I::res_tail, 0, 2, kNoHole, "res_tail must be 0 (off), 1 (tail + next conv1) or 2 (tail alone)"},
     {"sc_fuse", &I::sc_fuse, 0, 3, kNoHole, "sc_fuse must be 0 .. 3 (bit 0: one GEMM, bit 1: in the tail)"},
@@ -398,7 +400,10 @@
   if (key == "in_planes") m.build_simam_params();
 }
 
-int Model::get_option(const std::string& key) const { return impl->*find_opt(key).field; }
+int Model::get_option(const std::string& key) const {
+  if (key == "presplit_plan") return impl->ecapa ? impl->ecapa_presplit_plan() : 0;
+  return impl->*find_opt(key).field;
+}
 
 void Model::profile_query(const std::string& tag, int* launches, double* total_ms, double* flops) {
   *launches = 0;
diff --git a/wespeaker_hubert_amd/csrc/model_impl.h b/wespeaker_hubert_amd/csrc/model_impl.h
--- a/wespeaker_hubert_amd/csrc/model_impl.h
+++ b/wespeaker_hubert_amd/csrc/model_impl.h
@@ -142,6 +142,9 @@
   ConvW conv, pool1, pool2;
   ConvW conv_g;
   int cat_gate = 1;
+  int a_presplit = 1;
+  enum { kSplitX3 = 2, kSplitD4 = 4 };
+  int ecapa_presplit_plan() const;
   void* pool2_frag = nullptr;
   int astp_fused_on = 1;
   LinW pool1_ctx;
@@ -271,7 +274,7 @@
   void launch(const ConvGemmArgs& g, const ConvW& cw, hipStream_t s);
   void gemm(const char* tag, const ConvW& cw, const float* a0, int lda, float* out, int ldo, int M, int T, int dil,
             int pad, int act, hipStream_t s, const int* seg, int nseg, const float* row_bias = nullptr,
-            bool use_bias = true, int role = 0);
+            bool use_bias = true, int role = 0, int afmt = kAF32);
 
   bool prof = false;
   std::map<std::string, ProfEntry> prof_map;
diff --git a/wespeaker_hubert_amd/csrc/ops.hip b/wespeaker_hubert_amd/csrc/ops.hip
--- a/wespeaker_hubert_amd/csrc/ops.hip
+++ b/wespeaker_hubert_amd/csrc/ops.hip
@@ -262,8 +262,9 @@
 
 namespace {
 constexpr int kRSRows = 64;
-
-template <bool HX>
+typedef unsigned u32x4 __attribute__((ext_vector_type(4)));
+
+template <bool HX, bool SPL>
 __global__ __launch_bounds__(256) void residual_scale_kernel(const f32x4* __restrict__ x,
                                                              const f32x4* __restrict__ h,
                                                              const float* __restrict__ g,
@@ -274,6 +275,34 @@
   const int sub = threadIdx.x / tpr;
   const int r0 = blockIdx.x * kRSRows;
   const int r1 = min(M, r0 + kRSRows);
+  const bool odd = threadIdx.x & 1;
+  auto put = [&](long i, f32x4 v) {
+    if constexpr (SPL) {
+      unsigned hi[2], lo[2];
+#pragma unroll
+      for (int k = 0; k < 2; ++k) {
+        unsigned hb[2], lb[2];
+#pragma unroll
+        for (int e = 0; e < 2; ++e) {
+          float ve = v[2 * k + e];
+          asm("" : "+v"(ve));
+          const __bf16 hh = (__bf16)ve;
+          hb[e] = __builtin_bit_cast(unsigned short, hh);
+          lb[e] = __builtin_bit_cast(unsigned short, (__bf16)(ve - (float)hh));
+        }
+        hi[k] = hb[0] | (hb[1] << 16);
+        lo[k] = lb[0] | (lb[1] << 16);
+      }
+      unsigned got[2];
+#pragma unroll
+      for (int k = 0; k < 2; ++k)
+        got[k] = (unsigned)__builtin_amdgcn_mov_dpp((int)(odd ? hi[k] : lo[k]), 0xB1, 0xF, 0xF, false);
+      const u32x4 o = odd ? u32x4{got[0], got[1], lo[0], lo[1]} : u32x4{hi[0], hi[1], got[0], got[1]};
+      out[i] = __builtin_bit_cast(f32x4, o);
+    } else {
+      out[i] = v;
+    }
+  };
   for (int c4 = threadIdx.x % tpr; c4 < C4; c4 += tpr) {
     int r = r0 + sub;
     for (; r + 7 * rpp < r1; r += 8 * rpp) {
@@ -291,21 +320,23 @@
         gv[u] = *reinterpret_cast<const f32x4*>(g + ((long)b * C4 + c4) * 4);
       }
 #pragma unroll
-      for (int u = 0; u < 8; ++u) out[(long)(r + u * rpp) * C4 + c4] = HX ? xv[u] + hv[u] * gv[u] : hv[u] * gv[u];
+      for (int u = 0; u < 8; ++u) put((long)(r + u * rpp) * C4 + c4, HX ? xv[u] + hv[u] * gv[u] : hv[u] * gv[u]);
     }
     for (; r < r1; r += rpp) {
       const int b = seg ? seg_of(seg, nseg, r) : r / T;
       const long i = (long)r * C4 + c4;
       const f32x4 gv = *reinterpret_cast<const f32x4*>(g + ((long)b * C4 + c4) * 4);
-      out[i] = HX ? x[i] + h[i] * gv : h[i] * gv;
+      put(i, HX ? x[i] + h[i] * gv : h[i] * gv);
     }
   }
 }
 }
 
 void launch_residual_scale(const float* x, const float* h, const float* g, float* out, int B,
-                           int T, int C, hipStream_t s, const int* seg, int M) {
+                           int T, int C, hipStream_t s, const int* seg, int M, bool split8) {
   WSP_CHECK(C % 4 == 0, "residual_scale: C % 4");
+  WSP_CHECK(!split8 || (C % 8 == 0 && (reinterpret_cast<uintptr_t>(out) & 31) == 0),
+            "residual_scale: split8 output needs C % 8 == 0 and 32-B aligned rows");
   const int C4 = C / 4;
   WSP_CHECK(C4 % 256 == 0 || 256 % C4 == 0, "residual_scale: C/4 must divide or be a multiple of 256");
   const int rows = seg ? M : B * T;
@@ -314,10 +345,13 @@
   const f32x4* x4 = reinterpret_cast<const f32x4*>(x);
   const f32x4* h4 = reinterpret_cast<const f32x4*>(h);
   f32x4* o4 = reinterpret_cast<f32x4*>(out);
-  if (x)
-    hipLaunchKernelGGL(residual_scale_kernel<true>, grid, dim3(256), 0, s, x4, h4, g, o4, rows, T, C4, seg, B);
-  else
-    hipLaunchKernelGGL(residual_scale_kernel<false>, grid, dim3(256), 0, s, x4, h4, g, o4, rows, T, C4, seg, B);
+#define WSP_RS(HX, SPL) \
+  hipLaunchKernelGGL((residual_scale_kernel<HX, SPL>), grid, dim3(256), 0, s, x4, h4, g, o4, rows, T, C4, seg, B)
+  if (x && split8) WSP_RS(true, true);
+  else if (x) WSP_RS(true, false);
+  else if (split8) WSP_RS(false, true);
+  else WSP_RS(false, false);
+#undef WSP_RS
   WSP_HIP(hipGetLastError());
 }
 
```

After: 25550 (median of 6 runs). No clear change (+0.3%).
